# TomClabault/RayTracerCPP

Measured on AMD Instinct MI355X. Metric: Mrays/sec (primary+shadow) at 1920x1080, 1M-tri scene; max |dpixel|, higher is better.
Workload: dtype f32; 1 GPU; C4 sphere1m: 1,000,000 tris, 1920x1080, ssaa_factor 2 (3840x2160 rays), primary + shadow, octree 12/40; rays_per_frame=10029157, primary_rays=8294400, reflection_rays=0, band_rows=8, parallelism=image strips x1, frames_in_flight=3, world_size=1, bands=interleaved b % N

## Files before the change

### include/rt_mi355x.h

```cpp
#ifndef RT_MI355X_H
#define RT_MI355X_H

#include <stdint.h>

#ifdef __cplusplus
extern "C" {
#endif

#define RT_OK 0
#define RT_EINVAL (-1)
#define RT_EHIP (-2)
#define RT_ENOMEM (-3)
#define RT_ESTATE (-4)
#define RT_EUNSUPPORTED (-5)
#define RT_EIO (-6)

#define RT_SHADING_RT 0
#define RT_SHADING_ABS_NORMALS 1
#define RT_SHADING_PASTEL_NORMALS 2
#define RT_SHADING_BARYCENTRIC 3
#define RT_SHADING_VISUALIZE_AO 4

#define RT_TEX_AO 0
#define RT_TEX_DIFFUSE 1
// ... 91 lines not shown

int rt_set_devices(rt_renderer *r, const int32_t *ids, int32_t n);

int rt_change_render_size(rt_renderer *r, int32_t width, int32_t height);

int rt_set_triangles(rt_renderer *r, const float *tri9, const int32_t *mat, const float *uv6, int64_t n);

int rt_add_sphere(rt_renderer *r, float cx, float cy, float cz, float radius, int32_t mat);
int rt_add_plane(rt_renderer *r, float px, float py, float pz, float nx, float ny, float nz, int32_t mat);

int rt_clear_geometry(rt_renderer *r);

int rt_set_materials(rt_renderer *r, const float *mats16, int32_t n);
int rt_get_material_count(rt_renderer *r, int32_t *n);

int rt_change_camera_fov(rt_renderer *r, float fov);
int rt_change_camera_aspect_ratio(rt_renderer *r, float aspect);
int rt_set_light_position(rt_renderer *r, float x, float y, float z);

int rt_set_camera_transform(rt_renderer *r, const float m[16]);
int rt_apply_transformation_to_camera(rt_renderer *r, const float m[16]);

int rt_set_camera_matrices(rt_renderer *r, const float pos[3], const float proj_inv[16], const float cam_to_world[16]);
int rt_get_camera_matrices(rt_renderer *r, float pos[3], float proj_inv[16], float cam_to_world[16]);

int rt_set_camera_projection(rt_renderer *r, const float proj[16], const float world_to_cam[16]);

int rt_set_camera_lens(rt_renderer *r, float fov, float aspect);

int rt_set_object_transform(rt_renderer *r, const float m[16]);
int rt_reset_previous_transform(rt_renderer *r);
int rt_get_triangles(rt_renderer *r, float *tri9, int64_t *n);

int rt_set_texture(rt_renderer *r, int32_t slot, int32_t w, int32_t h, const float *rgba);

int rt_set_skybox(rt_renderer *r, const int32_t w[6], const int32_t h[6], const float *const faces[6]);

int rt_reconstruct_bvh_new(rt_renderer *r);
int rt_destroy_bvh(rt_renderer *r);

int rt_ray_trace(rt_renderer *r);

int rt_raster_trace(rt_renderer *r);

int rt_get_ssao_buffers(rt_renderer *r, float *z, float *n4, int32_t *ao);

int rt_post_process(rt_renderer *r);

int rt_get_image(rt_renderer *r, uint32_t *argb, int32_t *w, int32_t *h);

int rt_lock_image(rt_renderer *r);
int rt_unlock_image(rt_renderer *r);

int rt_render(rt_renderer *r, float *ms);

int rt_request_aux(rt_renderer *r, int32_t want_rgba, int32_t want_hit, int32_t want_shadow);
int rt_get_internal(rt_renderer *r, uint32_t *argb, float *rgba, int32_t *hit_id, float *hit_t, uint8_t *shadow);

int rt_get_stats(rt_renderer *r, rt_stats *out);

int rt_local_rows(rt_renderer *r, int32_t band_rows, int32_t rank, int32_t nranks, int32_t *rows_out);
int rt_render_bands_device(rt_renderer *r, int32_t band_rows, int32_t rank, int32_t nranks, uint32_t *d_out,
                           void *hip_stream);
int rt_render_band_list_device(rt_renderer *r, int32_t band_rows, const int32_t *bands, int32_t nbands,
                               uint32_t *d_out, void *hip_stream);
int rt_band_costs(rt_renderer *r, void *hip_stream, double *costs, int32_t nbands);

int rt_trace_rays(rt_renderer *r, const float *orig, const float *dir, int64_t n, int32_t *tri_id, float *t,
                  float *u, float *v, uint8_t *ret);

int rt_trace_rays_device(rt_renderer *r, const float *d_orig, const float *d_dir, int64_t n, int32_t *d_tri_id,
                         float *d_t, float *d_u, float *d_v, uint8_t *d_ret, int64_t *d_counts, void *hip_stream);
int rt_is_shadowed_device(rt_renderer *r, const float *d_point, const float *d_normal, int64_t n, const float *light,
                          uint8_t *d_shadowed, void *hip_stream);
int rt_get_device_ray_queries(rt_renderer *r, int64_t calls[2], int64_t rays[2]);

int rt_trace_ray(rt_renderer *r, const float *orig, const float *dir, int64_t n, int32_t current_recursion_depth,
                 float *rgba, int32_t *hit_src, float *t, uint8_t *intersection_found, uint8_t *shadowed);

int rt_kernel_times(rt_renderer *r, float *ms, int32_t n);
int rt_band_counters(rt_renderer *r, int64_t *shadow_rays, int64_t *reflection_rays);
int rt_tile_mask(rt_renderer *r, int32_t src, uint32_t *words, int64_t cap, int32_t info[5]);
int rt_tile_starts(rt_renderer *r, int32_t src, uint32_t *sets, int64_t cap, int32_t info[3]);

void rt_make_transform(int32_t kind, float x, float y, float z, float out[16]);
void rt_compose(const float a[16], const float b[16], float out[16]);
void rt_inverse(const float m[16], float out[16]);
void rt_perspective(float fov, float aspect, float znear, float zfar, float out[16]);
void rt_transform_points(const float m[16], const float *pts, int64_t n, float *out);

typedef struct rt_obj rt_obj;
rt_obj *rt_obj_open(const char *path, const float xform[16], int32_t mat_offset);
int rt_obj_counts(const rt_obj *o, int64_t *ntri, int32_t *nmat, int32_t *has_uv);
int rt_obj_fetch(const rt_obj *o, float *tri9, int32_t *mat, float *uv6, float *mats16);
void rt_obj_close(rt_obj *o);


#ifdef __cplusplus
}
#endif
#endif
```

### raytracercpp_amd/_lib.py

```python
from __future__ import annotations

import ctypes as C
import os

import numpy as np

HERE = os.path.dirname(os.path.abspath(__file__))
LIB_PATH = os.path.join(HERE, "librt_mi355x.so")
if os.environ.get("RT_LIB_PATH"):
    LIB_PATH = os.environ["RT_LIB_PATH"]

RT_OK = 0
ERRORS = {-1: "RT_EINVAL", -2: "RT_EHIP", -3: "RT_ENOMEM", -4: "RT_ESTATE", -5: "RT_EUNSUPPORTED", -6: "RT_EIO"}

_f32p = C.POINTER(C.c_float)
_i32p = C.POINTER(C.c_int32)
_u32p = C.POINTER(C.c_uint32)
_u8p = C.POINTER(C.c_uint8)
_i64p = C.POINTER(C.c_int64)


class RtSettings(C.Structure):
    _fields_ = [
        ("image_width", C.c_int32), ("image_height", C.c_int32),
# ... 35 lines not shown
                return [float(x) if n == "build_split_ms" else int(x) for x in v]
            return int(v)
        return {n: conv(n, t) for n, t in self._fields_}


class RtEntryProbe(C.Structure):
    _fields_ = [
        ("proj_inv", C.c_float * 16), ("cam_to_world", C.c_float * 16), ("rw", C.c_int32), ("rh", C.c_int32),
        ("k", C.c_int32), ("fan", C.c_int32), ("depth", C.c_int32), ("quick", C.c_int32),
        ("pixel", _i32p), ("sets", _u32p), ("info", C.c_int64 * 4), ("depth_hist", C.c_int64 * 16),
    ]


_H = C.c_void_p
SIGNATURES = {
    "rt_default_settings": (None, [C.POINTER(RtSettings)]),
    "rt_create": (_H, [C.c_int]),
    "rt_destroy": (None, [_H]),
    "rt_last_error": (C.c_char_p, []),
    "rt_get_settings": (C.c_int, [_H, C.POINTER(RtSettings)]),
    "rt_set_settings": (C.c_int, [_H, C.POINTER(RtSettings)]),
    "rt_change_render_size": (C.c_int, [_H, C.c_int32, C.c_int32]),
    "rt_set_exact": (C.c_int, [_H, C.c_int]),
    "rt_finish_accel": (C.c_int, [_H]),
    "rt_set_devices": (C.c_int, [_H, _i32p, C.c_int32]),
    "rt_set_triangles": (C.c_int, [_H, _f32p, _i32p, _f32p, C.c_int64]),
    "rt_add_sphere": (C.c_int, [_H, C.c_float, C.c_float, C.c_float, C.c_float, C.c_int32]),
    "rt_add_plane": (C.c_int, [_H] + [C.c_float] * 6 + [C.c_int32]),
    "rt_clear_geometry": (C.c_int, [_H]),
    "rt_set_materials": (C.c_int, [_H, _f32p, C.c_int32]),
    "rt_get_material_count": (C.c_int, [_H, _i32p]),
    "rt_change_camera_fov": (C.c_int, [_H, C.c_float]),
    "rt_change_camera_aspect_ratio": (C.c_int, [_H, C.c_float]),
    "rt_set_light_position": (C.c_int, [_H, C.c_float, C.c_float, C.c_float]),
    "rt_set_camera_transform": (C.c_int, [_H, _f32p]),
    "rt_apply_transformation_to_camera": (C.c_int, [_H, _f32p]),
    "rt_set_camera_matrices": (C.c_int, [_H, _f32p, _f32p, _f32p]),
    "rt_set_camera_projection": (C.c_int, [_H, _f32p, _f32p]),
    "rt_set_camera_lens": (C.c_int, [_H, C.c_float, C.c_float]),
    "rt_get_ssao_buffers": (C.c_int, [_H, _f32p, _f32p, _i32p]),
    "rt_get_camera_matrices": (C.c_int, [_H, _f32p, _f32p, _f32p]),
    "rt_set_object_transform": (C.c_int, [_H, _f32p]),
    "rt_reset_previous_transform": (C.c_int, [_H]),
    "rt_get_triangles": (C.c_int, [_H, _f32p, _i64p]),
    "rt_get_device_transforms": (C.c_int, [_H, _i64p]),
    "rt_transform_points_device": (C.c_int, [C.c_int32, _f32p, _f32p, C.c_int64, _f32p, _i32p, _f32p]),
    "rt_set_triangles_device": (C.c_int, [_H, C.c_void_p, C.c_int64, C.c_void_p, _i32p, _f32p, C.c_int64, C.c_void_p]),
    "rt_update_vertices_device": (C.c_int, [_H, C.c_void_p, C.c_int64, C.c_void_p, C.c_void_p]),
    "rt_get_device_ingests": (C.c_int, [_H, _i64p]),
    "rt_gather_triangles_device": (C.c_int, [C.c_int32, _f32p, C.c_int64, _i32p, C.c_int64, _f32p, _i32p, _f32p]),
    "rt_set_accel_deferred": (C.c_int, [_H, C.c_int]),
    "rt_get_accel_builds": (C.c_int, [_H, _i64p]),
    "rt_set_texture": (C.c_int, [_H, C.c_int32, C.c_int32, C.c_int32, _f32p]),
    "rt_set_skybox": (C.c_int, [_H, _i32p, _i32p, C.POINTER(_f32p)]),
    "rt_reconstruct_bvh_new": (C.c_int, [_H]),
    "rt_destroy_bvh": (C.c_int, [_H]),
    "rt_ray_trace": (C.c_int, [_H]),
    "rt_raster_trace": (C.c_int, [_H]),
    "rt_post_process": (C.c_int, [_H]),
    "rt_get_image": (C.c_int, [_H, _u32p, _i32p, _i32p]),
    "rt_render": (C.c_int, [_H, _f32p]),
    "rt_lock_image": (C.c_int, [_H]),
    "rt_unlock_image": (C.c_int, [_H]),
    "rt_request_aux": (C.c_int, [_H, C.c_int32, C.c_int32, C.c_int32]),
    "rt_get_internal": (C.c_int, [_H, _u32p, _f32p, _i32p, _f32p, _u8p]),
    "rt_get_stats": (C.c_int, [_H, C.POINTER(RtStats)]),
    "rt_local_rows": (C.c_int, [_H, C.c_int32, C.c_int32, C.c_int32, _i32p]),
    "rt_render_bands_device": (C.c_int, [_H, C.c_int32, C.c_int32, C.c_int32, C.c_void_p, C.c_void_p]),
    "rt_render_band_list_device": (C.c_int, [_H, C.c_int32, _i32p, C.c_int32, C.c_void_p, C.c_void_p]),
    "rt_band_costs": (C.c_int, [_H, C.c_void_p, C.POINTER(C.c_double), C.c_int32]),
    "rt_trace_rays": (C.c_int, [_H, _f32p, _f32p, C.c_int64, _i32p, _f32p, _f32p, _f32p, _u8p]),
    "rt_trace_rays_device": (C.c_int, [_H, C.c_void_p, C.c_void_p, C.c_int64, C.c_void_p, C.c_void_p, C.c_void_p,
                                       C.c_void_p, C.c_void_p, C.c_void_p, C.c_void_p]),
    "rt_is_shadowed_device": (C.c_int, [_H, C.c_void_p, C.c_void_p, C.c_int64, _f32p, C.c_void_p, C.c_void_p]),
    "rt_get_device_ray_queries": (C.c_int, [_H, _i64p, _i64p]),
    "rt_trace_ray": (C.c_int, [_H, _f32p, _f32p, C.c_int64, C.c_int32, _f32p, _i32p, _f32p, _u8p, _u8p]),
    "rt_wide_query": (C.c_int, [_H, _f32p, _f32p, C.c_int64, C.c_int32, _f32p, _f32p, _i32p, _i32p, _f32p, _f32p, _f32p,
                                _u8p]),
    "rt_risk_words": (C.c_int, [_H, C.c_int32, C.POINTER(C.c_uint64), C.c_int64, _i64p, _i64p]),
    "rt_kernel_times": (C.c_int, [_H, _f32p, C.c_int32]),
    "rt_band_counters": (C.c_int, [_H, _i64p, _i64p]),
    "rt_tile_mask": (C.c_int, [_H, C.c_int32, _u32p, C.c_int64, _i32p]),
    "rt_tile_starts": (C.c_int, [_H, C.c_int32, _u32p, C.c_int64, _i32p]),
    "rt_make_transform": (None, [C.c_int32, C.c_float, C.c_float, C.c_float, _f32p]),
    "rt_compose": (None, [_f32p, _f32p, _f32p]),
    "rt_inverse": (None, [_f32p, _f32p]),
    "rt_perspective": (None, [C.c_float, C.c_float, C.c_float, C.c_float, _f32p]),
    "rt_transform_points": (None, [_f32p, _f32p, C.c_int64, _f32p]),
    "rt_obj_open": (_H, [C.c_char_p, _f32p, C.c_int32]),
    "rt_obj_counts": (C.c_int, [_H, _i64p, _i32p, _i32p]),
    "rt_obj_fetch": (C.c_int, [_H, _f32p, _i32p, _f32p, _f32p]),
    "rt_obj_close": (None, [_H]),
    "rt_octree_digest": (C.c_int, [_f32p, C.c_int64, C.c_int32, C.c_int32, C.c_int32, C.POINTER(C.c_uint64), _i64p,
                                   _f32p]),
    "rt_octree_build_device": (C.c_int, [C.c_int32, _f32p, C.c_int64, C.c_int32, C.c_int32, C.POINTER(C.c_uint64),
                                         _i64p, _f32p]),
    "rt_set_device_build": (C.c_int, [_H, C.c_int]),
    "rt_get_device_builds": (C.c_int, [_H, _i64p]),
    "rt_get_device_wide_builds": (C.c_int, [_H, _i64p]),
    "rt_wbvh_quick_digest": (C.c_int, [_f32p, C.c_int64, C.c_int32, C.c_int32, C.POINTER(C.c_uint64), _i64p, _f32p]),
    "rt_wbvh_quick_build_device": (C.c_int, [C.c_int32, _f32p, C.c_int64, C.c_int32, C.c_int32, C.POINTER(C.c_uint64),
                                             _i64p, _i64p, _f32p]),
    "rt_debug_read": (C.c_int, [_H, C.POINTER(C.c_uint64), C.c_int64]),
    "rt_tile_costs": (C.c_int, [_H, C.POINTER(C.c_uint32), C.c_int64, _i32p, _i32p]),
    "rt_wbvh_query": (C.c_int, [_f32p, C.c_int64, C.c_int32, C.c_int32, _f32p, _f32p, C.c_int64, _i32p, _i32p, _f32p,
                                _f32p, _f32p, _i64p, _f32p]),
    "rt_wbvh_query_ex": (C.c_int, [_f32p, C.c_int64, C.c_int32, C.c_int32, _f32p, _f32p, C.c_int64, _f32p, _f32p,
                                   C.c_int32, _f32p, _f32p, _i32p, _i32p, _f32p, _f32p, _f32p, _i64p, _f32p, _i32p,
                                   C.c_int32, _i64p, C.POINTER(RtEntryProbe)]),
    "rt_ocone_check": (C.c_int, [_f32p, C.c_int64, C.c_int32, C.c_int32, C.c_int32, _f32p, _f32p, C.c_int64, _i32p,
                                 _i64p, C.POINTER(C.c_uint32), _i32p, _f32p, C.POINTER(C.c_uint32)]),
    "rt_ocone_read": (C.c_int, [_H, C.POINTER(C.c_uint32), C.c_int64, _i32p, _f32p]),
    "rt_risk_cap_check": (C.c_int, [_f32p, C.c_int64, C.c_int32, C.c_int32, _f32p, _f32p, C.c_int64, C.c_float, _i32p,
                                    _i64p]),
}

GEOMETRY_INPUT = ("rt_set_triangles_device", "rt_update_vertices_device", "rt_get_device_ingests",
                  "rt_gather_triangles_device", "rt_set_accel_deferred", "rt_get_accel_builds")
RAY_QUERIES = ("rt_trace_rays_device", "rt_is_shadowed_device", "rt_get_device_ray_queries")

_lib = None


def has(name):
    return hasattr(lib(), name)


def lib():
    global _lib
    if _lib is None:
        if not os.path.exists(LIB_PATH):
            raise RuntimeError(f"{LIB_PATH} is missing: the HIP library must be built "
                               "(python -c 'import __graft_entry__ as g; g.build()')")
        try:
            import torch
        except ImportError:
            pass
        L = C.CDLL(LIB_PATH)
        for name, (res, args) in SIGNATURES.items():
            if name in GEOMETRY_INPUT + RAY_QUERIES and os.environ.get("RT_LIB_PATH") and not hasattr(L, name):
                continue
            fn = getattr(L, name)
            fn.restype = res
            fn.argtypes = args
        _lib = L
    return _lib


class RtError(RuntimeError):
    def __init__(self, code, where):
        msg = lib().rt_last_error()
        super().__init__(f"{where}: {ERRORS.get(code, code)}: {msg.decode() if msg else ''}")
        self.code = code


def check(rc, where):
    if rc != RT_OK:
        raise RtError(rc, where)
    return rc


def ptr(a, t):
    if a is None:
        return C.cast(None, t)
    return a.ctypes.data_as(t)


def f32(a):
    return np.ascontiguousarray(a, dtype=np.float32)


_KINDS = {"translation": 0, "rx": 1, "ry": 2, "rz": 3, "scale": 4, "identity": 5}


def make_transform(kind, x=0.0, y=0.0, z=0.0):
    out = np.zeros(16, np.float32)
    lib().rt_make_transform(_KINDS[kind], x, y, z, ptr(out, _f32p))
    return out


def compose(a, b):
    a, b = f32(a), f32(b)
    out = np.zeros(16, np.float32)
    lib().rt_compose(ptr(a, _f32p), ptr(b, _f32p), ptr(out, _f32p))
    return out


def inverse(m):
    m = f32(m)
    out = np.zeros(16, np.float32)
    lib().rt_inverse(ptr(m, _f32p), ptr(out, _f32p))
    return out


def perspective(fov, aspect, znear=0.1, zfar=1000.0):
    out = np.zeros(16, np.float32)
    lib().rt_perspective(fov, aspect, znear, zfar, ptr(out, _f32p))
    return out


def camera_matrices(fov, aspect, znear=0.1, zfar=1000.0):
    p = perspective(fov, aspect, znear, zfar)
    return p, inverse(p)


def transform_points(m, pts):
    m = f32(m)
    pts = f32(pts).reshape(-1, 3)
    out = np.zeros_like(pts)
    lib().rt_transform_points(ptr(m, _f32p), ptr(pts, _f32p), pts.shape[0], ptr(out, _f32p))
    return out


def transform_points_device(m, pts, device=0):
    m = f32(m)
    pts = f32(pts).reshape(-1, 3)
    out = np.zeros_like(pts)
    flag = C.c_int32()
    ms = np.zeros(2, np.float32)
    check(lib().rt_transform_points_device(device, ptr(m, _f32p), ptr(pts, _f32p), pts.shape[0], ptr(out, _f32p),
                                           C.byref(flag), ptr(ms, _f32p)), "rt_transform_points_device")
    return out, int(flag.value), (float(ms[0]), float(ms[1]))

# ... 241 lines not shown
```

### raytracercpp_amd/csrc/capi.cpp

```cpp
#include <atomic>
#include <chrono>
#include <cmath>
#include <thread>
#include <cstring>
#include <new>
#include <string>

#include "../../include/rt_mi355x_diag.h"
#include "host_scene.hpp"
#include "launch.hpp"
#include "octree.hpp"
#include "octree_gpu.hpp"
#include "ocone.hpp"
#include "wbvh.hpp"
#include "wbvh_quick_gpu.hpp"
#include "renderer.hpp"

namespace {
thread_local std::string g_err;

int record(rt::Renderer* r, int rc)
{
    if (rc != RT_OK)
        g_err = r->error();
// ... 394 lines not shown
        if (n < 0)
            return bad("bad band layout");
        *rows_out = n;
        return RT_OK;
    });
}
int rt_render_bands_device(rt_renderer* r, int32_t band_rows, int32_t rank, int32_t nranks, uint32_t* d_out,
                           void* hip_stream)
{
    return guarded(R(r), [&] {
        return R(r)->render_bands_device(band_rows, rank, nranks, d_out, reinterpret_cast<hipStream_t>(hip_stream));
    });
}

int rt_render_band_list_device(rt_renderer* r, int32_t band_rows, const int32_t* bands, int32_t nbands, uint32_t* d_out,
                               void* hip_stream)
{
    return guarded(R(r), [&] {
        return R(r)->render_band_list_device(band_rows, bands, nbands, d_out, reinterpret_cast<hipStream_t>(hip_stream));
    });
}
int rt_band_costs(rt_renderer* r, void* hip_stream, double* costs, int32_t nbands)
{
    return guarded(R(r), [&] { return R(r)->band_costs(reinterpret_cast<hipStream_t>(hip_stream), costs, nbands); });
}

int rt_trace_rays(rt_renderer* r, const float* orig, const float* dir, int64_t n, int32_t* tri_id, float* t,
                  float* u, float* v, uint8_t* ret)
{
    return guarded(R(r), [&] { return R(r)->trace_rays(orig, dir, n, tri_id, t, u, v, ret); });
}
int rt_trace_rays_device(rt_renderer* r, const float* d_orig, const float* d_dir, int64_t n, int32_t* d_tri_id,
                         float* d_t, float* d_u, float* d_v, uint8_t* d_ret, int64_t* d_counts, void* hip_stream)
{
    return guarded(R(r), [&] {
        return R(r)->trace_rays_device(d_orig, d_dir, n, d_tri_id, d_t, d_u, d_v, d_ret, d_counts,
                                       reinterpret_cast<hipStream_t>(hip_stream));
    });
}
int rt_is_shadowed_device(rt_renderer* r, const float* d_point, const float* d_normal, int64_t n, const float* light,
                          uint8_t* d_shadowed, void* hip_stream)
{
    return guarded(R(r), [&] {
        return R(r)->is_shadowed_device(d_point, d_normal, n, light, d_shadowed, reinterpret_cast<hipStream_t>(hip_stream));
    });
}
int rt_get_device_ray_queries(rt_renderer* r, int64_t calls[2], int64_t rays[2])
{
    return guarded(R(r), [&] {
        if (!calls || !rays)
            return RT_EINVAL;
        R(r)->device_ray_queries(calls, rays);
        return RT_OK;
    });
}
int rt_wide_query(rt_renderer* r, const float* orig, const float* dir, int64_t n, int32_t kind, float* o_out,
                  float* d_out, int32_t* status, int32_t* tri_id, float* t, float* u, float* v, uint8_t* shadowed)
{
    return guarded(R(r), [&] { return R(r)->wide_query(orig, dir, n, kind, o_out, d_out, status, tri_id, t, u, v, shadowed); });
}
int rt_risk_words(rt_renderer* r, int32_t src, uint64_t* out, int64_t cap, int64_t* count, int64_t* violations)
{
    return guarded(R(r), [&] { return R(r)->risk_words(src, out, cap, count, violations); });
}
int rt_trace_ray(rt_renderer* r, const float* orig, const float* dir, int64_t n, int32_t current_recursion_depth,
                 float* rgba, int32_t* hit_src, float* t, uint8_t* intersection_found, uint8_t* shadowed)
{
    return guarded(R(r), [&] {
        return R(r)->trace_ray_colors(orig, dir, n, current_recursion_depth, rgba, hit_src, t, intersection_found,
                                      shadowed);
    });
}
int rt_kernel_times(rt_renderer* r, float* ms, int32_t n)
{
    return guarded(R(r), [&] { return ms ? R(r)->kernel_times(ms, n) : RT_EINVAL; });
}
int rt_tile_mask(rt_renderer* r, int32_t src, uint32_t* words, int64_t cap, int32_t info[5])
{
    return guarded(R(r), [&] { return info ? R(r)->tile_mask(src, words, cap, info) : RT_EINVAL; });
}
int rt_tile_starts(rt_renderer* r, int32_t src, uint32_t* sets, int64_t cap, int32_t info[3])
{
    return guarded(R(r), [&] { return info ? R(r)->tile_starts(src, sets, cap, info) : RT_EINVAL; });
}
int rt_band_counters(rt_renderer* r, int64_t* shadow_rays, int64_t* reflection_rays)
{
    return guarded(R(r), [&] {
        unsigned long long c[2] = {0, 0};
        int rc = R(r)->band_counters(c);
        if (shadow_rays) *shadow_rays = (int64_t)c[0];
        if (reflection_rays) *reflection_rays = (int64_t)c[1];
        return rc;
    });
}

void rt_make_transform(int32_t kind, float x, float y, float z, float out[16])
{
    switch (kind) {
    case 0: rt::mat::translation(x, y, z, out); break;
    case 1: rt::mat::rotation_x(x, out); break;
    case 2: rt::mat::rotation_y(x, out); break;
    case 3: rt::mat::rotation_z(x, out); break;
    case 4: rt::mat::scale(x, y, z, out); break;
    default: rt::mat::identity(out); break;
    }
}
void rt_compose(const float a[16], const float b[16], float out[16]) { rt::mat::compose(a, b, out); }
void rt_inverse(const float m[16], float out[16]) { rt::mat::inverse(m, out); }
void rt_perspective(float fov, float aspect, float znear, float zfar, float out[16])
{
    rt::mat::perspective(fov, aspect, znear, zfar, out);
}
void rt_transform_points(const float m[16], const float* pts, int64_t n, float* out)
{
    rt::mat::transform_points(m, pts, n, out);
}

struct rt_obj {
    rt::ObjData data;
};

rt_obj* rt_obj_open(const char* path, const float xform[16], int32_t mat_offset)
{
    try {
        float ident[16];
        rt::mat::identity(ident);
        rt_obj* o = new rt_obj;
        std::string err;
        if (!rt::load_obj(path, xform ? xform : ident, mat_offset, o->data, err)) {
            g_err = err;
            delete o;
            return nullptr;
        }
        return o;
    } catch (const std::exception& e) {
        g_err = e.what();
        return nullptr;
    }
}

int rt_obj_counts(const rt_obj* o, int64_t* ntri, int32_t* nmat, int32_t* has_uv)
{
    if (!o)
        return bad("null obj");
    if (ntri) *ntri = (int64_t)o->data.mat.size();
    if (nmat) *nmat = (int32_t)o->data.materials.size();
    if (has_uv) *has_uv = o->data.has_uv;
    return RT_OK;
}

int rt_obj_fetch(const rt_obj* o, float* tri9, int32_t* mat, float* uv6, float* mats16)
{
    if (!o)
        return bad("null obj");
    const rt::ObjData& d = o->data;
    if (tri9) std::memcpy(tri9, d.tri.data(), d.tri.size() * 4);
    if (mat) std::memcpy(mat, d.mat.data(), d.mat.size() * 4);
    if (uv6 && d.has_uv) std::memcpy(uv6, d.uv.data(), d.uv.size() * 4);
    if (mats16) {
        for (size_t i = 0; i < d.materials.size(); i++) {
            const rt::ObjMaterial& m = d.materials[i];
            float* f = mats16 + 16 * i;
            for (int c = 0; c < 3; c++) {
                f[0 + c] = m.ambient[c];
                f[3 + c] = m.diffuse[c];
                f[6 + c] = m.specular[c];
// ... 915 lines not shown
```

### raytracercpp_amd/csrc/kernels.hip

```cpp
#include <hip/hip_runtime.h>
#include <stdint.h>
#if defined(RT_COUNT) && RT_COUNT
__device__ unsigned long long g_wsteps[8];
__device__ __forceinline__ void w_step_hook(uint32_t cur, int leaf)
{
    const uint64_t act = __ballot(1);
    uint64_t left = act;
    unsigned distinct = 0;
    while (left) {
        const uint32_t f = (uint32_t)__builtin_amdgcn_readlane((int)cur, __ffsll((unsigned long long)left) - 1);
        left &= ~__ballot(cur == f);
        distinct++;
    }
    if ((int)__lane_id() == __ffsll((unsigned long long)act) - 1) {
        atomicAdd(&g_wsteps[2 * leaf], 1ull);
        if (distinct == 1)
            atomicAdd(&g_wsteps[2 * leaf + 1], 1ull);
        atomicAdd(&g_wsteps[4 + leaf], (unsigned long long)__popcll(act));
        atomicAdd(&g_wsteps[6 + leaf], (unsigned long long)distinct);
    }
}
#define W_STEP_HOOK(cur, leaf) w_step_hook(cur, leaf)
#endif
#include "kparams.hpp"
#include "rt_math.hpp"
#include "wbvh.hpp"
#include "launch.hpp"

namespace rt {

constexpr int WAVES_PER_BLOCK = 4;
constexpr int BLOCK = 64 * WAVES_PER_BLOCK;

#ifndef RT_OCC
#define RT_OCC 5
#endif
#ifndef RT_OCC_PLAIN
#define RT_OCC_PLAIN 3
#endif
#ifndef RT_OCC_OCT
#define RT_OCC_OCT 5
#endif
#ifndef RT_COUNT
#define RT_COUNT 0
#endif
#ifndef RT_PHASE_TIME
#define RT_PHASE_TIME 0
#endif

struct TRay {
    v3 o, d;
    float den[NPLANES], num[NPLANES];
    bool nan;
    float lo, hi;
};


struct Rec {
    int tri;
    float t, u, v;
    int mat;
    v3 normal, tangent;
};

__device__ __forceinline__ Rec rec_fresh()
{
    Rec r;
    r.tri = -1; r.t = -1.0f; r.u = 1.0f; r.v = 0.0f; r.mat = -1;
    r.normal = mk(0, 0, 0); r.tangent = mk(0, 0, 0);
    return r;
}

__device__ __forceinline__ TRay make_ray(const KParams& P, v3 o, v3 d)
{
    TRay R;
    R.o = o;
    R.d = d;
    bool nan = false;
#pragma unroll
    for (int i = 0; i < NPLANES; i++) {
        v3 n = mk(PLANE_N[i][0], PLANE_N[i][1], PLANE_N[i][2]);
        R.den[i] = dot(n, d);
        R.num[i] = dot(n, o);
        nan |= (R.den[i] != R.den[i]) || (R.num[i] != R.num[i]);
        if (R.den[i] == 0.0f)
            R.num[i] = __int_as_float(0x7fc00000);
    }
    R.nan = nan;
    R.lo = -INFINITY;
    R.hi = INFINITY;
    return R;
}

__device__ __forceinline__ v3 opaque(v3 v)
{
    asm volatile("" : "+v"(v.x), "+v"(v.y), "+v"(v.z));
    return v;
}

__device__ __forceinline__ bool ray_is_nan(v3 o, v3 d)
{
    bool nan = false;
#pragma unroll
    for (int i = 0; i < NPLANES; i++) {
        v3 n = mk(PLANE_N[i][0], PLANE_N[i][1], PLANE_N[i][2]);
        float den = dot(n, d), num = dot(n, o);
        nan |= (den != den) || (num != num);
    }
    return nan;
// ... 540 lines not shown
        face = d2.z < 0.0f ? 4 : 5;
        nf = (float)(0.5 / (double)da.z);
        u = d2.z < 0.0f ? -d2.x : d2.x;
        v = -d2.y;
    } else if (da.y >= da.x) {
        face = d2.y < 0.0f ? 3 : 2;
        nf = (float)(0.5 / (double)da.y);
        u = d2.x;
        v = d2.y < 0.0f ? -d2.z : d2.z;
    } else {
        face = d2.x < 0.0f ? 1 : 0;
        nf = (float)(0.5 / (double)da.x);
        u = d2.x < 0.0f ? d2.z : -d2.z;
        v = -d2.y;
    }
    u = (float)((double)(u * nf) + 0.5);
    v = (float)((double)(v * nf) + 0.5);
    return tex_bilinear(P.sky[face], u, v, alpha);
}

__device__ __forceinline__ const float* mat_of(const KParams& P, int id) { return P.mats + (size_t)MAT_STRIDE * id; }
__device__ __forceinline__ c3 mat_col(const float* m, int off) { return col(m[off], m[off + 1], m[off + 2]); }

__device__ __forceinline__ void get_tex_coords(const KParams& P, int tri, float u, float v, float& tu, float& tv)
{
    if (tri >= 0) {
        float u0 = -1, u1 = -1, u2 = -1, v0 = -1, v1 = -1, v2 = -1;
        if (P.tri_uv) {
            const float* uv = P.tri_uv + 6 * (size_t)tri;
            u0 = uv[0]; u1 = uv[1]; u2 = uv[2];
            v0 = uv[3]; v1 = uv[4]; v2 = uv[5];
        }
        tu = (1 - u - v) * u0 + u * u1 + v * u2;
        tv = (1 - u - v) * v0 + u * v1 + v * v2;
    } else {
        tu = u;
        tv = v;
    }
}

__device__ v3 normal_mapping(const KParams& P, const Rec& h, float u, float v)
{
    float tu, tv;
    get_tex_coords(P, h.tri, u, v, tu, tv);
    v3 T = h.tangent;
    v3 B = cross(T, h.normal);
    v3 N = h.normal;
    c3 nc = tex_floor(P.tex[TEX_NORMAL], tu, tv);
    v3 nm = mk(nc.r, nc.g, nc.b) * 2.0f - mk(1, 1, 1);
    v3 q = normalize(nm);
    v3 p = mk(T.x * q.x + B.x * q.y + N.x * q.z, T.y * q.x + B.y * q.y + N.y * q.z, T.z * q.x + B.z * q.y + N.z * q.z);
    return normalize(p);
}

__device__ void parallax_occlusion_mapping(const KParams& P, int tri, float u, float v, v3 view, float& nu, float& nv)
{
    float tu, tv;
    get_tex_coords(P, tri, u, v, tu, tv);
    const KTex& D = P.tex[TEX_DISPLACEMENT];
    int steps = P.parallax_mapping_steps;
    float current_depth;
    float depth_step = 1.0f / steps;
    float sampled = tex_floor(D, tu, tv).r;
    v3 search = -view * P.displacement_mapping_strength;
    float du = search.x / steps;
    float dv = search.y / steps;
    current_depth = 0.0f;
    float u2 = tu, v2 = tv;
    while (current_depth < sampled) {
        u2 += du;
        v2 += dv;
        sampled = tex_floor(D, u2, v2).r;
        current_depth += depth_step;
    }
    float pu = u2 - du, pv = v2 - dv;
    float after = sampled - current_depth;
    float before = tex_floor(D, pu, pv).r - (current_depth - depth_step);
    float w = after / (after - before);
    nu = (1 - w) * u2 + w * pu;
    nv = (1 - w) * v2 + w * pv;
}

#if RT_PHASE_TIME
__shared__ unsigned long long g_phase[WAVES_PER_BLOCK][8];
__device__ __forceinline__ void ph_mark(int k)
{
    const unsigned long long now = __builtin_amdgcn_s_memtime();
    const uint64_t act = __ballot(1);
    if ((int)__lane_id() == __ffsll((unsigned long long)act) - 1) {
        const int w = threadIdx.x >> 6;
        g_phase[w][k] += now - g_phase[w][7];
        g_phase[w][7] = now;
    }
}
#define PH_MARK(k) ph_mark(k)
#else
#define PH_MARK(k)
#endif

constexpr int LDS_SAVE_ENTRIES = 3;
__host__ __device__ __forceinline__ int lds_save_slot(const KParams& P) { return P.levels > W_STACK ? P.levels : W_STACK; }
#ifndef RT_W_STACK_PLAIN
#define RT_W_STACK_PLAIN 22
#endif
constexpr int W_STACK_PLAIN = RT_W_STACK_PLAIN;
static_assert(W_STACK_PLAIN >= W_STACK && W_STACK_PLAIN + LDS_SAVE_ENTRIES <= 26, "the plain kernel's LDS entries");
template <bool OCT>
__host__ __device__ __forceinline__ int lds_save_slot_plain(const KParams& P)
{
    const int w = OCT ? 0 : W_STACK_PLAIN;
    return P.levels > w ? P.levels : w;
}

template <int N = W_STACK>
struct WStackLdsN {
    static constexpr int CAP = N;
    uint2* base;
    __device__ __forceinline__ void put(int i, uint2 v) { base[i * BLOCK] = v; }
    __device__ __forceinline__ uint2 get(int i) const { return base[i * BLOCK]; }
    __device__ __forceinline__ uint2 get_lane(int delta, int i) const { return base[delta + i * BLOCK]; }
};
using WStackLds = WStackLdsN<W_STACK>;

#if RT_COUNT
__device__ void count_wave_steps(const KParams& P, int base, uint32_t steps)
{
    if (!P.counters)
        return;
    uint64_t act = __ballot(1), a = act;
    uint32_t mx = 0;
    while (a) {
        const int l = __ffsll((unsigned long long)a) - 1;
        a &= a - 1;
        mx = max(mx, (uint32_t)__builtin_amdgcn_readlane((int)steps, l));
    }
    if ((int)__lane_id() == __ffsll((unsigned long long)act) - 1) {
        atomicAdd(&P.counters[base], (unsigned long long)mx);
        atomicAdd(&P.counters[base + 2], 1ull);
    }
    atomicAdd(&P.counters[base + 1], (unsigned long long)steps);
}
#endif


struct WDeep {
    int st;
    WHit w;
};
__device__ __noinline__ WDeep wide_closest_deep(const WNode* wnodes, const GTri* wtris, v3 o, v3 d, float m, float hi,
                                                bool ties, float QS, const uint64_t* rk, int rsel, float rsub)
{
    WStackArr<W_DEEP_STACK> stk;
    WDeep r;
    const int st = wbvh_closest(wnodes, wtris, o, d, m, stk, r.w, nullptr, hi, ties, QS, rk, rsel, rsub);
    r.st = st == W_DEEP ? W_UNCERT : st;
    return r;
}

__device__ __forceinline__ float wide_margin(const KParams& P, v3 o)
{
    const float om = fmaxf(fabsf(o.x), fmaxf(fabsf(o.y), fabsf(o.z)));
    return 0x1p-16f * (om + P.scene_scale);
}

template <class Stk, int G>
__device__ __forceinline__ int wide_run(const KParams& P, v3 o, v3 d, uint2* lv, WHit& w, float hi, bool ties, float QS,
                                        const uint64_t* rk, int rsel, float rsub, uint32_t max_steps, bool nob, int count,
                                        const uint32_t* start = nullptr)
{
    const float m = wide_margin(P, o);
    Stk stk{lv};
#if RT_COUNT
    uint32_t work[4] = {0, 0, 0, 0};
    uint32_t* wk = count >= 0 ? work : nullptr;
#else
// ... 622 lines not shown
            if (F.rough > 0) {
                F.sc++;
                F.i++;
            } else {
                F.sc = 1;
                F.i = N;
            }
            f = depth - 1;
            state = S_NEXT;
        } else {
            Frame& F = fr[f];
            if (F.i < N) {
                v3 dir;
                next_key = child_key(F.key, (uint32_t)F.i);
                if (F.rough > 0) {
                    uint32_t rng = sample_state(F.key, (uint32_t)F.i);
                    float rx = rng_bilateral(rng);
                    float ry = rng_bilateral(rng);
                    float rz = rng_bilateral(rng);
                    v3 rdir = normalize(mk(rx, ry, rz));
                    if (dot(rdir, F.n) < 0)
                        rdir = -rdir;
                    dir = F.rough * rdir + (1 - F.rough) * F.perfect;
                } else
                    dir = F.perfect;
                nrefl++;
                ro = F.ro;
                rd = dir;
                depth = f + 1;
                state = S_TRACE;
            } else {
                const float* m = mat_of(P, F.mat);
                float sc = (float)F.sc, rf = m[12];
                c3 R = (F.total / col(sc, sc, sc)) * col(rf, rf, rf);
                ret = shade_finish(P, F.fc, m, R);
                depth = f;
                state = S_RET;
            }
        }
    }
    po.color = ret;
    return po;
}

__device__ __forceinline__ void write_ssao_buffers(const KParams& P, size_t o, bool found, v3 cam, v3 rd,
                                                   const Rec& fin)
{
    P.zbuf[o] = found ? -(cam.z + rd.z * fin.t) : INFINITY;
    P.nbuf[o] = found ? make_float4(fin.normal.x, fin.normal.y, fin.normal.z, 0.0f) : make_float4(0, 0, 0, 0);
}

__device__ __forceinline__ void tile_xy(const KParams& P, int tile, int& tx, int& ty)
{
    const int W = P.tiles_x;
    if (tile >= (1 << 24)) {
        tx = tile % W;
        ty = tile / W;
        return;
    }
    int q = (int)((float)tile * (1.0f / (float)W));
    int r = tile - q * W;
    if (r < 0) {
        q--;
        r += W;
    } else if (r >= W) {
        q++;
        r -= W;
    }
    tx = r;
    ty = q;
}

__device__ __forceinline__ int global_row(const KParams& P, int lr)
{
    if (P.nranks == 1)
        return lr;
    int band = lr / P.band_rows;
    const int g = P.band_map ? ldg(P.band_map + band) : band * P.nranks + P.rank;
    return g * P.band_rows + (lr - band * P.band_rows);
}

constexpr int BQ_BATCH = 4;

__device__ __forceinline__ int shard_tile(const KParams& P, int s, int t)
{
    const int r0 = (int)((long long)P.tiles_y * s / TILE_SHARDS), r1 = (int)((long long)P.tiles_y * (s + 1) / TILE_SHARDS);
    return t < (r1 - r0) * P.tiles_x ? r0 * P.tiles_x + t : -1;
}


struct BlockQueue {
    unsigned int word;
    int shard, empty;
    int base[4], sh[4];
    int heavy_done;
    int split_done;
    unsigned long long cost_sum;
    unsigned int cost_max;
    int waves_done;
};
__shared__ BlockQueue g_bq;

__device__ __forceinline__ void tile_queue_init()
{
    if (threadIdx.x == 0) {
        g_bq.word = 0u;
        g_bq.shard = (int)(blockIdx.x & (TILE_SHARDS - 1));
        g_bq.empty = 0;
        g_bq.heavy_done = 0;
        g_bq.split_done = 0;
        g_bq.cost_sum = 0;
        g_bq.cost_max = 0;
        g_bq.waves_done = 0;
    }
    __syncthreads();
}

__device__ __forceinline__ void tile_stats_add(uint32_t c, uint32_t cmax)
{
    __hip_atomic_fetch_add(&g_bq.cost_sum, (unsigned long long)c, __ATOMIC_RELAXED, __HIP_MEMORY_SCOPE_WORKGROUP);
    __hip_atomic_fetch_max(&g_bq.cost_max, cmax, __ATOMIC_RELAXED, __HIP_MEMORY_SCOPE_WORKGROUP);
}

__device__ __forceinline__ void tile_stats_flush(const KParams& P, int lane)
{
    if (!P.tile_stats || lane != 0)
        return;
    const int k = __hip_atomic_fetch_add(&g_bq.waves_done, 1, __ATOMIC_ACQ_REL, __HIP_MEMORY_SCOPE_WORKGROUP);
    if (k != (int)(blockDim.x >> 6) - 1)
        return;
    const unsigned long long s = __hip_atomic_load(&g_bq.cost_sum, __ATOMIC_ACQUIRE, __HIP_MEMORY_SCOPE_WORKGROUP);
    const unsigned int m = __hip_atomic_load(&g_bq.cost_max, __ATOMIC_ACQUIRE, __HIP_MEMORY_SCOPE_WORKGROUP);
    if (s) atomicAdd(P.tile_stats, s);
    if (m) atomicMax(P.tile_stats + 1, (unsigned long long)m);
}

__device__ __forceinline__ int tile_queue_next_shards(const KParams& P)
{
    const int lane = threadIdx.x & 63;
    for (;;) {
        unsigned int w = 0;
        if (lane == 0)
            w = __hip_atomic_fetch_add(&g_bq.word, 1u, __ATOMIC_ACQ_REL, __HIP_MEMORY_SCOPE_WORKGROUP);
        w = __builtin_amdgcn_readfirstlane(w);
        if (w & 0x80000000u)
            return -1;
        const unsigned int g = (w >> 24) & 0x7fu, c = (w >> 16) & 0xffu, i = w & 0xffffu;
        if (i < c) {
            const int slot = (int)(g & 3u);
            return shard_tile(P, g_bq.sh[slot], g_bq.base[slot] + (int)i);
        }
        if (i == c) {
            int shard = g_bq.shard, empty = g_bq.empty, b = 0, n = 0;
            while (empty < TILE_SHARDS) {
                int t = 0;
                if (lane == 0)
                    t = (int)atomicAdd(reinterpret_cast<unsigned int*>(&P.counters[NCOUNTERS + 16 * shard]),
                                       (unsigned)BQ_BATCH);
                b = __builtin_amdgcn_readfirstlane(t);
                n = 0;
                while (n < BQ_BATCH && shard_tile(P, shard, b + n) >= 0)
                    n++;
                if (n > 0)
                    break;
                empty++;
                shard = (shard + 1) & (TILE_SHARDS - 1);
            }
            const unsigned int g1 = (g + 1u) & 0x7fu;
            if (lane == 0) {
                g_bq.shard = shard;
                g_bq.empty = empty;
                g_bq.base[g1 & 3u] = b;
                g_bq.sh[g1 & 3u] = shard;
                __hip_atomic_store(&g_bq.word, n > 0 ? (g1 << 24) | ((unsigned)n << 16) | 1u : 0x80000000u,
                                   __ATOMIC_RELEASE, __HIP_MEMORY_SCOPE_WORKGROUP);
            }
            return n > 0 ? shard_tile(P, shard, b) : -1;
        }
        for (;;) {
            unsigned int v = 0;
            if (lane == 0)
                v = __hip_atomic_load(&g_bq.word, __ATOMIC_ACQUIRE, __HIP_MEMORY_SCOPE_WORKGROUP);
            v = __builtin_amdgcn_readfirstlane(v);
            if ((v & 0x80000000u) || ((v >> 24) & 0x7fu) != g)
                break;
            __builtin_amdgcn_s_sleep(2);
        }
    }
}

__device__ __forceinline__ int tile_queue_next(const KParams& P)
{
    const int lane = threadIdx.x & 63;
    if (P.heavy_list) {
        if (!__builtin_amdgcn_readfirstlane(__hip_atomic_load(&g_bq.heavy_done, __ATOMIC_RELAXED,
                                                             __HIP_MEMORY_SCOPE_WORKGROUP))) {
            int t = 0;
            if (lane == 0)
                t = atomicAdd(P.heavy_ctr + 1, 1);
            t = __builtin_amdgcn_readfirstlane(t);
            if (t < min(ldg(P.heavy_ctr), P.tiles_x * P.tiles_y / 16))
                return ldg(P.heavy_list + t);
            if (lane == 0)
                __hip_atomic_store(&g_bq.heavy_done, 1, __ATOMIC_RELAXED, __HIP_MEMORY_SCOPE_WORKGROUP);
        }
        for (;;) {
            const int tile = tile_queue_next_shards(P);
            if (tile < 0 || !((ldg(P.heavy_bits + (tile >> 5)) >> (tile & 31)) & 1u))
                return tile;
        }
    }
    return tile_queue_next_shards(P);
}

__device__ __forceinline__ void set_wave_prio(int level)
{
    switch (level) {
    case 3: __builtin_amdgcn_s_setprio(3); break;
    case 2: __builtin_amdgcn_s_setprio(2); break;
    case 1: __builtin_amdgcn_s_setprio(1); break;
    default: __builtin_amdgcn_s_setprio(0); break;
    }
}

template <int G = 1, int C0 = 8>
__device__ __forceinline__ void downscale_tile(const KParams& P, int lane, int lr, int px, uint32_t c, int C = C0)
{
    int r = (int)((c >> 16) & 0xffu), g = (int)((c >> 8) & 0xffu), b = (int)(c & 0xffu);
    const int f = 1 << P.ds_shift;
    for (int m = 1; m < f; m <<= 1) {
        r += __shfl_xor(r, G * m);
        g += __shfl_xor(g, G * m);
        b += __shfl_xor(b, G * m);
    }
    for (int m = C; m < C * f; m <<= 1) {
        r += __shfl_xor(r, G * m);
        g += __shfl_xor(g, G * m);
        b += __shfl_xor(b, G * m);
    }
    const int pl = lane / G;
    if ((lane & (G - 1)) == 0 && ((pl % C) & (f - 1)) == 0 && ((pl / C) & (f - 1)) == 0) {
        const int s2 = 2 * P.ds_shift;
        P.ds_out[(size_t)(lr >> P.ds_shift) * (size_t)(P.rw >> P.ds_shift) + (size_t)(px >> P.ds_shift)] =
            qrgb(r >> s2, g >> s2, b >> s2);
    }
}

__device__ __forceinline__ v3 camera_dir(const KParams& P, int px, int py, v3 cam)
{
    const float y_world = ((float)py + 0.5f) / P.rh * 2 - 1;
    const float x_world = ((float)px + 0.5f) / P.rw * 2 - 1;
    v3 vs;
    if (P.proj_mode != 0) {
        const float* m = P.proj_inv;
        const float x = x_world, y = y_world, z = -1.0f;
        const float xt = m[0] * x + m[1] * y + m[2] * z + m[3];
        const float yt = m[4] * x + m[5] * y + m[6] * z + m[7];
        const float zt = m[8] * x + m[9] * y + m[10] * z + m[11];
        const float w = P.proj_w;
        vs = P.proj_mode == 1 ? mk(xt, yt, zt) : mk(xt * w, yt * w, zt * w);
    } else
        vs = xform_point(P.proj_inv, mk(x_world, y_world, -1));
    v3 ws;
    if (P.c2w_affine && fabsf(vs.x) < INFINITY && fabsf(vs.y) < INFINITY && fabsf(vs.z) < INFINITY) {
        const float* m = P.cam_to_world;
        ws = mk(m[0] * vs.x + m[1] * vs.y + m[2] * vs.z + m[3], m[4] * vs.x + m[5] * vs.y + m[6] * vs.z + m[7],
                m[8] * vs.x + m[9] * vs.y + m[10] * vs.z + m[11]);
    } else
        ws = xform_point(P.cam_to_world, vs);
    return normalize(ws - cam);
}

__device__ __forceinline__ int tile_start_index(const KParams& P, int px, int py)
{
    return P.tile_start ? (py >> 3) * P.start_bw + (px >> 3) : -1;
}

template <int G>
__device__ __forceinline__ void trace_split_part(const KParams& P, uint2* lv, int t, int lane, unsigned& nshadow)
{
    static_assert(G > 1 && G <= 8 && (G & (G - 1)) == 0, "2, 4 or 8 lanes per pixel");
    const int cap = P.tiles_x * P.tiles_y / 16;
    const int np = P.split_parts;
    const int tq = ldg(P.heavy_list + cap + t / np), part = t % np;
    const int tile = tq & 0x0fffffff;
    set_wave_prio(tq >> 28);
    const uint64_t t0 = __builtin_amdgcn_s_memtime();
    int tx, ty;
    tile_xy(P, tile, tx, ty);
    const int npix = 64 / np;
    const int C = npix >= 16 ? 8 : npix / 2, R = npix / C;
    const int pl = lane / G;
    const int px = tx * 8 + (part % (8 / C)) * C + pl % C;
    const int lr = ty * 8 + (part / (8 / C)) * R + pl / C;
    const int py = lr < P.local_rows ? global_row(P, lr) : P.rh;
    if (pl < npix && px < P.rw && py < P.rh) {
        const v3 cam = mk(P.cam_pos[0], P.cam_pos[1], P.cam_pos[2]);
        const v3 rd = camera_dir(P, px, py, cam);
        unsigned ns = 0, nr = 0;
        PixelOut po = trace_pixel<false, true, G>(P, cam, rd, lv, 0u, ns, nr, tile_start_index(P, px, py));
        if ((lane & (G - 1)) == 0)
            nshadow += ns;
        const size_t o = (size_t)lr * P.rw + px;
        const uint32_t c = color_to_argb(po.color);
        if (P.ds_out) downscale_tile<G>(P, lane, lr, px, c, C);
        if ((lane & (G - 1)) == 0) {
            if (P.argb) P.argb[o] = c;
            if (P.rgba) P.rgba[o] = make_float4(po.color.r, po.color.g, po.color.b, po.alpha);
            if (P.hit_id) P.hit_id[o] = po.found ? po.src : -1;
            if (P.hit_t) P.hit_t[o] = po.fin.t;
            if (P.shadow) P.shadow[o] = (uint8_t)(po.found && po.shadowed);
        }
    }
    const uint64_t c = __builtin_amdgcn_s_memtime() - t0;
    if (lane == 0) {
        const uint32_t c32 = c > 0xFFFFFFFFull ? 0xFFFFFFFFu : (uint32_t)c;
        atomicAdd(P.tile_cost + tile, c32);
        tile_stats_add(c32, c32 > 0xFFFFFFFFu / G ? 0xFFFFFFFFu : c32 * G);
    }
}

__device__ __forceinline__ void tile_cost_store(const KParams& P, int tile, uint64_t t0, int lane)
{
    const uint64_t c = __builtin_amdgcn_s_memtime() - t0;
    if (lane == 0) {
        const uint32_t c32 = c > 0xFFFFFFFFull ? 0xFFFFFFFFu : (uint32_t)c;
        P.tile_cost[tile] = c32;
        tile_stats_add(c32, c32);
    }
}

__device__ __noinline__ void fill_masked_tile(const KParams& P, int lr, int px)
{
    const c3 bg = background();
    const uint32_t c = color_to_argb(bg);
    const size_t o = (size_t)lr * P.rw + px;
    if (P.argb) P.argb[o] = c;
    if (P.ds_out) {
        const int f = 1 << P.ds_shift;
        if ((px & (f - 1)) == 0 && (lr & (f - 1)) == 0)
            P.ds_out[(size_t)(lr >> P.ds_shift) * (size_t)(P.rw >> P.ds_shift) + (size_t)(px >> P.ds_shift)] =
                qrgb((int)((c >> 16) & 0xffu), (int)((c >> 8) & 0xffu), (int)(c & 0xffu));
    }
    if (P.rgba) P.rgba[o] = make_float4(bg.r, bg.g, bg.b, 1.0f);
    if (P.hit_id) P.hit_id[o] = -1;
    if (P.hit_t) P.hit_t[o] = rec_fresh().t;
    if (P.shadow) P.shadow[o] = (uint8_t)0;
#if RT_COUNT
    if (P.counters && (threadIdx.x & 63) == 0)
        atomicAdd(&P.counters[28], 1ull);
#endif
}

template <bool REFL, bool PLAIN = false, bool OCT = false>
__global__ __launch_bounds__(BLOCK, OCT ? RT_OCC_OCT : PLAIN ? RT_OCC_PLAIN : RT_OCC) void ray_trace_kernel(KParams P_arg)
{
    auto kp = __builtin_amdgcn_kernarg_segment_ptr();
    (void)P_arg;
    const KParams& P = *reinterpret_cast<const KParams*>((const void*)kp);
    uint2* lv = lane_stack();
    int lane = threadIdx.x & 63;
    unsigned nshadow = 0, nrefl = 0;
    tile_queue_init();
#if RT_PHASE_TIME
    if (PLAIN && lane == 0) {
        for (int k = 0; k < 7; k++)
            g_phase[threadIdx.x >> 6][k] = 0;
        g_phase[threadIdx.x >> 6][7] = __builtin_amdgcn_s_memtime();
    }
#endif
    for (;;) {
        auto kpl = kp;
        asm volatile("" : "+s"(kpl));
        const KParams& P = *reinterpret_cast<const KParams*>((const void*)kpl);
        const v3 cam = mk(P.cam_pos[0], P.cam_pos[1], P.cam_pos[2]);
        if (PLAIN && !REFL && !OCT && P.heavy_group == SPLIT_G &&
            !__builtin_amdgcn_readfirstlane(__hip_atomic_load(&g_bq.split_done, __ATOMIC_RELAXED, __HIP_MEMORY_SCOPE_WORKGROUP))) {
            int t = 0;
            if (lane == 0)
                t = atomicAdd(P.heavy_ctr + 2, 1);
            t = __builtin_amdgcn_readfirstlane(t);
            if (t < P.split_parts * min(ldg(P.heavy_ctr + 3), P.tiles_x * P.tiles_y / 16)) {
                trace_split_part<SPLIT_G>(P, lv, t, lane, nshadow);
                continue;
            }
            if (lane == 0)
                __hip_atomic_store(&g_bq.split_done, 1, __ATOMIC_RELAXED, __HIP_MEMORY_SCOPE_WORKGROUP);
        }
        const int tq = tile_queue_next(P);
        if (PLAIN) PH_MARK(6);
        if (tq < 0)
            break;
        const int tile = tq & 0x0fffffff;
        if (P.heavy_list)
            set_wave_prio(tq >> 28);
        const uint64_t tile_t0 = __builtin_amdgcn_s_memtime();
        int tx, ty;
        tile_xy(P, tile, tx, ty);
        int px = tx * 8 + (lane & 7);
        int lr = ty * 8 + (lane >> 3);
        int py = lr < P.local_rows ? global_row(P, lr) : P.rh;
        if (PLAIN) PH_MARK(0);
        if (px >= P.rw || py >= P.rh) {
            if (P.tile_cost && lane == 0)
                P.tile_cost[tile] = 0u;
            continue;
        }
        if (PLAIN && !REFL && !OCT && P.tile_mask) {
            const uint32_t mw = ldg(P.tile_mask + (size_t)(py >> 3) * (size_t)P.mask_wpr + (size_t)(px >> 8));
            if (!__ballot((mw >> ((px >> 3) & 31)) & 1u)) {
                fill_masked_tile(P, lr, px);
                if (P.tile_cost)
                    tile_cost_store(P, tile, tile_t0, lane);
                continue;
            }
        }
        const v3 rd = camera_dir(P, px, py, cam);
        if (PLAIN) PH_MARK(1);

        uint32_t rng = REFL ? pixel_seed((uint32_t)(py * P.rw + px), P.rng_seed) : 0u;
        PixelOut po = trace_pixel<REFL, PLAIN, 1, OCT>(P, cam, rd, lv, rng, nshadow, nrefl,
                                                        PLAIN && !REFL && !OCT ? tile_start_index(P, px, py) : -1);
        size_t o = (size_t)lr * P.rw + px;
        if (P.argb) P.argb[o] = color_to_argb(po.color);
        if (!REFL && P.ds_out) downscale_tile(P, lane, lr, px, color_to_argb(po.color));
        if (P.rgba) P.rgba[o] = make_float4(po.color.r, po.color.g, po.color.b, po.alpha);
        if (P.hit_id) P.hit_id[o] = po.found ? po.src : -1;
        if (P.hit_t) P.hit_t[o] = po.fin.t;
        if (P.shadow) P.shadow[o] = (uint8_t)(po.found && po.shadowed);
        if (!PLAIN && P.zbuf) write_ssao_buffers(P, o, po.found, cam, rd, po.fin);
        if (PLAIN) PH_MARK(5);
        if (P.tile_cost)
            tile_cost_store(P, tile, tile_t0, lane);
    }
    tile_stats_flush(P, lane);
#if RT_PHASE_TIME
    if (PLAIN) {
        PH_MARK(0);
        const int wid = (int)(blockIdx.x * WAVES_PER_BLOCK + (threadIdx.x >> 6));
        if (P.dbg && lane == 0 && wid < DBG_WAVES)
            for (int k = 0; k < 7; k++)
                P.dbg[DBG_WORDS * wid + k] = g_phase[threadIdx.x >> 6][k];
    }
#endif
    if (nshadow) atomicAdd(&P.counters[0], (unsigned long long)nshadow);
    if (nrefl) atomicAdd(&P.counters[1], (unsigned long long)nrefl);
}

__device__ __forceinline__ v3 ld3(const float* p) { return mk(p[0], p[1], p[2]); }
__device__ __forceinline__ void st3(float* p, v3 v) { p[0] = v.x; p[1] = v.y; p[2] = v.z; }
__device__ __forceinline__ void st3(float* p, c3 c) { p[0] = c.r; p[1] = c.g; p[2] = c.b; }
__device__ __forceinline__ c3 ldc(const float* p) { return col(p[0], p[1], p[2]); }

__device__ __forceinline__ void wave_count_add(unsigned long long* ctr, unsigned v)
{
    for (int off = 32; off > 0; off >>= 1)
        v += __shfl_xor(v, off);
    if ((threadIdx.x & 63) == 0 && v)
        atomicAdd(ctr, (unsigned long long)v);
}

__device__ __forceinline__ uint32_t wave_append(unsigned int* counter, bool lead = true)
{
    const uint64_t m = __ballot(lead);
    const int leader = __ffsll((unsigned long long)m) - 1;
    uint32_t base = 0;
    if ((int)(threadIdx.x & 63) == leader)
        base = atomicAdd(counter, (unsigned)__popcll(m));
    base = __shfl(base, leader);
    return base + __builtin_amdgcn_mbcnt_hi((uint32_t)(m >> 32), __builtin_amdgcn_mbcnt_lo((uint32_t)m, 0u));
}

__device__ __forceinline__ float frame_roughness(const KParams& P, const Rec& h, const float* m)
{
    if (P.enable_roughness_mapping) {
        float tu, tv;
        get_tex_coords(P, h.tri, h.u, h.v, tu, tv);
        return tex_floor(P.tex[TEX_ROUGHNESS], tu, tv).r;
    }
    return m[13];
}

__device__ __forceinline__ int frame_nsamp(const KParams& P, float rough)
{
    int N = P.rough_reflections_sample_count;
    return N <= 0 ? 0 : (rough > 0 ? N : 1);
}

__device__ __forceinline__ void make_frame(const KParams& P, FrameRec& F, v3 ip, v3 n, v3 rd, c3 fc, float rough,
                                           int mat, uint32_t key, int parent)
{
    st3(F.ro, ip + n * 0.01f);
    st3(F.perfect, rd - (2 * dot(rd, n)) * n);
    st3(F.n, n);
    st3(F.fc, fc);
    F.rough = rough;
    F.mat = mat;
    F.key = key;
    F.nsamp = frame_nsamp(P, rough);
    F.parent = parent;
}

__global__ __launch_bounds__(BLOCK, RT_OCC) void refl_level0_kernel(KParams P_arg, FrameRec* fr1, unsigned int* nfr1)
{
    const KParams& P = kernel_params();
    (void)P_arg;
    uint2* lv = lane_stack();
    int lane = threadIdx.x & 63;
    const int ntiles = P.tiles_x * P.tiles_y;
    v3 cam = mk(P.cam_pos[0], P.cam_pos[1], P.cam_pos[2]);
    unsigned nshadow = 0;
    for (;;) {
        int tile = 0;
        if (lane == 0)
            tile = (int)atomicAdd(reinterpret_cast<unsigned int*>(&P.counters[2]), 1u);
        tile = __builtin_amdgcn_readfirstlane(tile);
        if (tile >= ntiles)
            break;
        int tx, ty;
        tile_xy(P, tile, tx, ty);
        int px = tx * 8 + (lane & 7);
        int lr = ty * 8 + (lane >> 3);
        int py = lr < P.local_rows ? global_row(P, lr) : P.rh;
        if (px >= P.rw || py >= P.rh)
            continue;
        const v3 rd = camera_dir(P, px, py, cam);

        Rec fin = rec_fresh();
        int src = closest_hit(P, cam, rd, fin, lv);
// ... 1429 lines not shown
    if (blockIdx.x == 0) {
        for (int i = (int)threadIdx.x; i < ncounters; i += (int)blockDim.x)
            counters[i] = 0ull;
        if (threadIdx.x < 4)
            ctr_next[threadIdx.x] = 0;
        if (threadIdx.x < 2)
            stats_next[threadIdx.x] = 0ull;
    }
    const unsigned long long sum = stats_prev[0];
    const unsigned int mx = (unsigned int)min(stats_prev[1], 0xFFFFFFFFull);
    const unsigned long long mean = ntiles > 0 ? sum / (unsigned long long)ntiles : 0;
    const unsigned long long thr = max(4 * mean, (unsigned long long)(mx / 8));
    const unsigned long long thr2 = group > 1 && nwaves > 0 ? max(thr, (unsigned long long)((double)split * (double)sum / nwaves))
                                                            : ~0ull;
    const int cap = ntiles / 16;
    const int i = (int)(blockIdx.x * blockDim.x + threadIdx.x);
    const int lane = (int)(threadIdx.x & 63);
    const uint32_t c = i < ntiles ? cost[i] : 0u;
    const bool heavy = mx > 0 && c >= thr && c > 0;
    const bool two = heavy && c >= thr2;
    const uint64_t b1 = __ballot(heavy && !two), b2 = __ballot(two);
    int base1 = 0, base2 = 0;
    if (lane == 0) {
        if (b1) base1 = atomicAdd(ctr, __popcll(b1));
        if (b2) base2 = atomicAdd(ctr + 3, __popcll(b2));
    }
    base1 = __builtin_amdgcn_readfirstlane(base1);
    base2 = __builtin_amdgcn_readfirstlane(base2);
    const uint64_t below = (1ull << lane) - 1ull;
    const int k = two ? base2 + __popcll(b2 & below) : base1 + __popcll(b1 & below);
    const bool listed = heavy && k < cap;
    if (listed) {
        const int prio = ntiles >= (1 << 28) ? 0 : c >= mx / 2 ? 3 : c >= mx / 4 ? 2 : 1;
        list[two ? cap + k : k] = i | (prio << 28);
        if (two)
            cost[i] = 0u;
    }
    const uint64_t bl = __ballot(listed);
    if ((lane & 31) == 0 && i < ntiles)
        bits[i >> 5] = (uint32_t)(bl >> lane);
}

static int plain_blocks(const rt::KParams& P)
{
    const int tiles = P.tiles_x * P.tiles_y;
    const int blocks = (tiles + rt::WAVES_PER_BLOCK - 1) / rt::WAVES_PER_BLOCK;
    return P.max_blocks > 0 ? std::max(1, std::min(blocks, P.max_blocks / 8 * RT_OCC_PLAIN)) : blocks;
}

static int persistent_blocks(const rt::KParams& P)
{
    const int tiles = P.tiles_x * P.tiles_y;
    const int blocks = (tiles + rt::WAVES_PER_BLOCK - 1) / rt::WAVES_PER_BLOCK;
    return blocks > P.max_blocks && P.max_blocks > 0 ? P.max_blocks : blocks;
}

hipError_t rt_launch_heavy_prep(const rt::KParams* P, uint32_t* cost, int ntiles, int32_t* list, uint32_t* bits,
                                int32_t* ctr, int32_t* ctr_next, const unsigned long long* stats_prev,
                                unsigned long long* stats_next, float split, int group, hipStream_t stream)
{
    if (ntiles <= 0)
        return hipSuccess;
    hipLaunchKernelGGL(heavy_prep_kernel, dim3((ntiles + 63) / 64), dim3(64), 0, stream, cost, ntiles, list, bits,
                       ctr, ctr_next, stats_prev, stats_next, P->counters, rt::NCOUNTER_WORDS,
                       plain_blocks(*P) * rt::WAVES_PER_BLOCK, split, group);
    return hipGetLastError();
}

hipError_t rt_launch_ray_trace(const rt::KParams* P, hipStream_t stream)
{
    const int blocks = persistent_blocks(*P);
    if (blocks < 1)
        return hipSuccess;
    const bool plain = !P->has_reflection && P->plain && !P->zbuf && !P->nbuf;
    size_t lds = rt::lds_bytes(*P, plain);
    if (P->has_reflection)
        hipLaunchKernelGGL((rt::ray_trace_kernel<true, false>), dim3(blocks), dim3(rt::BLOCK), lds, stream, *P);
    else if (plain) {
        if (!P->wnodes) {
            hipLaunchKernelGGL((rt::ray_trace_kernel<false, true, true>), dim3(blocks), dim3(rt::BLOCK), lds, stream, *P);
            return hipGetLastError();
        }
        const int pblocks = plain_blocks(*P);
        hipLaunchKernelGGL((rt::ray_trace_kernel<false, true>), dim3(pblocks), dim3(rt::BLOCK), lds, stream, *P);
    } else
        hipLaunchKernelGGL((rt::ray_trace_kernel<false, false>), dim3(blocks), dim3(rt::BLOCK), lds, stream, *P);
    return hipGetLastError();
}

__global__ __launch_bounds__(256) void risk_box_init_kernel(float* B, size_t n)
{
    const size_t i = (size_t)blockIdx.x * 256 + threadIdx.x;
    if (i < 6 * n)
        B[i] = (i % 6) < 3 ? INFINITY : -INFINITY;
}

hipError_t rt_launch_risk_box_init(float* B, size_t nentries, hipStream_t stream)
{
    if (nentries > 0)
        hipLaunchKernelGGL(risk_box_init_kernel, dim3((unsigned)((6 * nentries + 255) / 256)), dim3(256), 0, stream, B,
                           nentries);
    return hipGetLastError();
}

__global__ __launch_bounds__(1024) void wide_cut_kernel(const rt::WNode* __restrict__ nodes, int nnodes, int budget,
                                                        int max_depth, float QS, uint32_t* buf)
{
    __shared__ int s_n, s_next, s_grew;
    uint32_t* cur = buf;
    uint32_t* nxt = buf + rt::W_CUT_MAX;
    const int tid = (int)threadIdx.x;
    if (tid == 0) {
        int n = 0;
        for (int j = 0; j < rt::W_WIDTH; j++)
            if (nodes[0].child[j] != rt::W_EMPTY)
                cur[n++] = (uint32_t)j;
        s_n = n;
    }
    __syncthreads();
    for (int depth = 1; depth < max_depth; depth++) {
        if (tid == 0) {
            s_next = 0;
            s_grew = 0;
        }
        __syncthreads();
        const int n = s_n;
        int total = 0, grew = 0;
        for (int i = tid; i < n; i += 1024) {
            uint32_t out[rt::W_WIDTH];
            const int k = rt::wbvh_cut_expand(nodes, nnodes, cur[i], QS, out);
            total += k;
            grew |= !(k == 1 && out[0] == cur[i]);
        }
        if (total)
            atomicAdd(&s_next, total);
        if (grew)
            atomicOr(&s_grew, 1);
        __syncthreads();
        const bool stop = !s_grew || s_next > budget;
        __syncthreads();
        if (stop)
            break;
        if (tid == 0)
            s_next = 0;
        __syncthreads();
        for (int i = tid; i < n; i += 1024) {
            uint32_t out[rt::W_WIDTH];
            const int k = rt::wbvh_cut_expand(nodes, nnodes, cur[i], QS, out);
            const int base = atomicAdd(&s_next, k);
            for (int q = 0; q < k; q++)
                nxt[base + q] = out[q];
        }
        __syncthreads();
        if (tid == 0)
            s_n = s_next;
        uint32_t* t = cur;
        cur = nxt;
        nxt = t;
        __syncthreads();
    }
    const int n = s_n;
    if (cur != buf)
        for (int i = tid; i < n; i += 1024)
            buf[i] = cur[i];
    if (tid == 0)
        buf[2 * rt::W_CUT_MAX] = (uint32_t)n;
}

__global__ __launch_bounds__(256) void wide_mask_kernel(const rt::WNode* __restrict__ nodes, int nnodes,
                                                        const uint32_t* __restrict__ parent, const uint32_t* __restrict__ cut,
                                                        rt::WMaskCam C, uint32_t* words)
{
    const uint32_t i = blockIdx.x * 256u + threadIdx.x;
    if (i >= cut[2 * rt::W_CUT_MAX] || i >= (uint32_t)rt::W_CUT_MAX)
        return;
    const uint32_t en = cut[i];
    if ((int)(en >> 2) >= nnodes)
        return;
    rt::WMaskRect R = rt::wbvh_mask_entry(nodes, nnodes, parent, en, C);
    R.x0 = max(R.x0, 0);
    R.y0 = max(R.y0, 0);
    R.x1 = min(R.x1, C.bw - 1);
    R.y1 = min(R.y1, C.bh - 1);
    if (R.x0 > R.x1)
        return;
    for (int y = R.y0; y <= R.y1; y++)
        for (int w = R.x0 >> 5; w <= R.x1 >> 5; w++) {
            uint32_t* p = words + (size_t)y * C.wpr + w;
            const uint32_t m = rt::wbvh_mask_word(R, w);
            if ((__hip_atomic_load(p, __ATOMIC_RELAXED, __HIP_MEMORY_SCOPE_AGENT) & m) != m)
                atomicOr(p, m);
        }
}

__global__ __launch_bounds__(256) void wide_entry_kernel(const rt::WNode* __restrict__ nodes, int nnodes, rt::WMaskCam C,
                                                         const uint32_t* __restrict__ words, int K, int fan, int max_depth,
                                                         uint4* out)
{
    const uint32_t i = blockIdx.x * 256u + threadIdx.x;
    if (i >= (uint32_t)(C.bw * C.bh))
        return;
    const int bx = (int)(i % (uint32_t)C.bw), by = (int)(i / (uint32_t)C.bw);
    uint4 r = make_uint4(0u, rt::W_EMPTY, rt::W_EMPTY, rt::W_EMPTY);
    if ((words[(size_t)by * C.wpr + (bx >> 5)] >> (bx & 31)) & 1u) {
        const rt::WEntrySet S = rt::wbvh_entry_block(nodes, nnodes, C, bx, by, K, fan, max_depth);
        r = make_uint4(S.link[0], S.link[1], S.link[2], S.link[3]);
    }
    out[i] = r;
}

hipError_t rt_launch_wide_entry(const rt::WNode* wnodes, int nnodes, const rt::WMaskCam* C, const uint32_t* words, int K,
                                int fan, int max_depth, uint4* out, hipStream_t stream)
{
    const int nb = C->bw * C->bh;
    if (nb <= 0)
        return hipSuccess;
    hipLaunchKernelGGL(wide_entry_kernel, dim3((nb + 255) / 256), dim3(256), 0, stream, wnodes, nnodes, *C, words, K, fan,
                       max_depth, out);
    return hipGetLastError();
}

hipError_t rt_launch_wide_cut(const rt::WNode* wnodes, int nnodes, int budget, int max_depth, uint32_t* buf, hipStream_t stream)
{
    budget = budget < rt::W_WIDTH ? rt::W_WIDTH : (budget > rt::W_CUT_MAX ? rt::W_CUT_MAX : budget);
    hipLaunchKernelGGL(wide_cut_kernel, dim3(1), dim3(1024), 0, stream, wnodes, nnodes, budget, max_depth, W_QS_CLOSEST, buf);
    return hipGetLastError();
}

hipError_t rt_launch_wide_mask(const rt::WNode* wnodes, int nnodes, const uint32_t* parent, const uint32_t* cut, int budget,
                               const rt::WMaskCam* C, uint32_t* words, hipStream_t stream)
{
    budget = budget < rt::W_WIDTH ? rt::W_WIDTH : (budget > rt::W_CUT_MAX ? rt::W_CUT_MAX : budget);
    hipError_t e = hipMemsetAsync(words, 0, (size_t)C->bh * C->wpr * 4, stream);
    if (e != hipSuccess)
        return e;
    hipLaunchKernelGGL(wide_mask_kernel, dim3((budget + 255) / 256), dim3(256), 0, stream, wnodes, nnodes, parent, cut,
                       *C, words);
    return hipGetLastError();
}

hipError_t rt_launch_wide_risk(const rt::GTri* wtris, const uint4* wmeta, const rt::GNode* onodes,
                               const rt::WNode* wnodes, const uint32_t* tri_leaf, const uint32_t* parent, uint32_t* K,
                               float* B, unsigned long long* risk, int n, int nnodes, const rt::WRiskArgs* A,
                               uint32_t* cap, const float* cap_dir, hipStream_t stream)
{
    rt::RiskCapDirs cd;
    for (int i = 0; i < 6; i++)
        cd.c[i / 3][i % 3] = cap_dir ? cap_dir[i] : 0.0f;
    if (n > 0)
        hipLaunchKernelGGL(rt::wide_risk_kernel, dim3((n + 255) / 256), dim3(256), 0, stream, wtris, wmeta, onodes,
                           tri_leaf, parent, K, B, n, *A, cap, cd);
    const int ne = 8 * nnodes;
    if (ne > 0)
        hipLaunchKernelGGL(rt::wide_risk_pack_kernel, dim3((ne + 255) / 256), dim3(256), 0, stream, wnodes, K, B, risk,
                           ne, *A);
    return hipGetLastError();
}

hipError_t rt_launch_wide_gather(const rt::GTri* tris, const int32_t* slot, const uint32_t* leaf_of_slot,
                                 const int32_t* tri_id, const int32_t* tri_mat, int n, rt::GTri* wtris, uint4* wmeta,
                                 hipStream_t stream)
{
    if (n <= 0)
        return hipSuccess;
    hipLaunchKernelGGL(rt::wide_gather_kernel, dim3((n + 255) / 256), dim3(256), 0, stream, tris, slot, leaf_of_slot,
                       tri_id, tri_mat, n, wtris, wmeta);
    return hipGetLastError();
}

namespace rt {
__global__ void ocone_fill_kernel(uint2* cells, size_t n)
{
    const size_t i = (size_t)blockIdx.x * 256 + threadIdx.x;
    if (i < n)
        cells[i] = make_uint2(0u, OC_NOSKIP << 16);
}

struct OConeArgs {
    float lo[3];
    int32_t dim[3];
    double h, r, slack, QS, cos_cap;
};

__global__ __launch_bounds__(256) void ocone_kernel(const OConeEnt* E, const GTri* tris, const uint32_t* todo, int n,
                                                    OConeArgs A, uint2* cells)
{
    const int i = blockIdx.x * 256 + threadIdx.x;
    if (i >= n)
        return;
    const uint32_t id = todo[i];
    double c[3];
    ocone_center(A.lo, A.dim, A.h, id, c);
    cells[id] = ocone_cell<OC_STACK>(E, tris, c, A.r, A.slack, A.QS, A.cos_cap);
}
}

hipError_t rt_launch_ocone(const rt::OConeEnt* E, const rt::GTri* tris, const uint32_t* todo, int n, const float lo[3],
                           const int32_t dim[3], double h, double r, double slack, double QS, double cos_cap,
                           uint2* cells, size_t ncells, hipStream_t stream)
{
    if (ncells == 0)
// ... 162 lines not shown
```

### raytracercpp_amd/csrc/kparams.hpp

```cpp
#pragma once

#include <stdint.h>

#include "octree.hpp"
#include "ocone.hpp"
#include "wbvh.hpp"

namespace rt {

#ifndef RT_SPLIT_G
#define RT_SPLIT_G 4
#endif
constexpr int SPLIT_G = RT_SPLIT_G;
constexpr int SPLIT_COLS = SPLIT_G == 8 ? 4 : 8;
constexpr int SPLIT_ROWS = 64 / SPLIT_G / SPLIT_COLS;
static_assert(SPLIT_G == 2 || SPLIT_G == 4 || SPLIT_G == 8, "2, 4 or 8 lanes per pixel");

constexpr int TEX_SLOTS = 6;
constexpr int MAT_STRIDE = 16;
constexpr int MAX_SHAPES = 64;
constexpr int NCOUNTERS = 32;
constexpr int TILE_SHARDS = 8;
constexpr int NCOUNTER_WORDS = NCOUNTERS + 16 * TILE_SHARDS;
constexpr int DBG_WAVES = 16384;
// ... 17 lines not shown
    const float* lslab;
    float scene_scale;
    const float* lsin;
    const WNode* wnodes;
    const GTri* wtris;
    const uint4* wmeta;
    const uint64_t* wrisk;
    float risk_G, risk_nl, risk_nu;
    const float* risk_cap;
    float cap_dir[2][3];
    float sb_lo[3], sb_hi[3];
    int32_t sb_valid;
    const uint32_t* tile_mask;
    int32_t mask_wpr;
    const uint4* tile_start;
    int32_t start_bw;
    OConeView ocone;
    int32_t nnodes;
    int32_t ntri_slots;
    int32_t levels;

    int32_t nshape;
    int32_t shape_kind[MAX_SHAPES];
    float shape[MAX_SHAPES][6];
    int32_t shape_mat[MAX_SHAPES];

    const float* mats;
    int32_t nmat;

    float cam_pos[3];
    float proj_inv[16];
    float cam_to_world[16];
    float light[3];
    int32_t proj_mode;
    float proj_w;
    int32_t c2w_affine;

    KTex tex[TEX_SLOTS];
    KTex sky[6];

    int32_t shading_method;
    int32_t compute_shadows;
    int32_t max_recursion_depth;
    int32_t enable_bvh;
    int32_t enable_ambient, enable_diffuse, enable_specular, enable_emissive;
    int32_t rough_reflections_sample_count;
    int32_t enable_ao_mapping, enable_diffuse_mapping, enable_normal_mapping, enable_displacement_mapping;
    float displacement_mapping_strength;
    int32_t parallax_mapping_steps;
    int32_t enable_roughness_mapping, enable_skysphere, enable_skybox;
    uint32_t rng_seed;
    int32_t has_reflection;
    float seg_scale;
    int32_t seg_oct;

    int32_t rw, rh;
    int32_t band_rows;
    int32_t nranks, rank;
    const int32_t* band_map;
    const int32_t* band_inv;
    int32_t local_rows;
    int32_t tiles_x, tiles_y;
    int32_t max_blocks;
    int32_t plain;
    uint32_t* tile_cost;
    unsigned long long* tile_stats;
    const int32_t* heavy_list;
    const uint32_t* heavy_bits;
    int32_t* heavy_ctr;
    int32_t heavy_group;
    int32_t split_parts;

    uint32_t* argb;
    float4* rgba;
    int32_t* hit_id;
    float* hit_t;
    uint8_t* shadow;
    unsigned long long* counters;
    unsigned long long* dbg;
    float* zbuf;
    float4* nbuf;
    uint32_t* ds_out;
    int32_t ds_shift;
};

struct SsaoArgs {
    const float* z;
    const float4* n;
    int32_t* ao;
    uint32_t* argb;
    int32_t w, h;
    int32_t simd_w;
    int32_t count;
    float radius, amount;
    float fovm;
    float tanv;
    float aspect;
    uint32_t seed;
    float proj[16];
};

struct FrameRec {
    float ro[3];
    float perfect[3];
    float n[3];
    float fc[3];
    float rough;
    int32_t mat;
    uint32_t key;
    int32_t nsamp;
    int32_t parent;
};

struct SampleRec {
    float d[3];
    int32_t kind;
    float fc[3];
    float ip[3];
    float nrm[3];
    int32_t mat;
    float crough;
    int32_t sh;
    int32_t child;
    int32_t ray;
};

struct RawHit {
    float t, u, v;
    int32_t k;
    float d[3];
    int32_t r;
};

struct ReflArgs {
    FrameRec* fr;
    SampleRec* sm;
    RawHit* hit;
    float* ret;
    const float* child_ret;
    FrameRec* child_fr;
    unsigned int* child_count;
    const int32_t* order;
    const FrameRec* frs;
    unsigned int* feed_parts;
    int32_t* list;
    unsigned int* list_count;
    int32_t c0, c1;
    int32_t level;
    int32_t stride;
    int32_t sample_major;
    float4* res;
    int32_t* defer;
    unsigned int* defer_count;
    int32_t max_steps;
    int32_t feed;
};

struct RasterPiece {
    float na[3], nb[3], nc[3];
    float wa[3], wb[3], wc[3];
    float inv_area;
    float za, zb, zc;
    int32_t x0, y0, x1, y1;
    int32_t tri;
    int32_t pad;
};
// ... 18 lines not shown
```

### raytracercpp_amd/csrc/launch.hpp

```cpp
#pragma once

#include <hip/hip_runtime.h>
#include <stdint.h>

#include "kparams.hpp"
#include "ocone.hpp"
#include "wbvh.hpp"

namespace rt {

enum class ReflStage {
    trace,
    long_,
    pass1,
    shadow,
    resolve,
};

enum class RasterStage {
    count,
    write,
    fill,
    fill_big,
};

}

#define RT_LAUNCH extern "C" __attribute__((visibility("hidden"))) hipError_t

RT_LAUNCH rt_launch_ray_trace(const rt::KParams* P, hipStream_t stream);
RT_LAUNCH rt_launch_heavy_prep(const rt::KParams* P, uint32_t* cost, int ntiles, int32_t* list, uint32_t* bits,
                               int32_t* ctr, int32_t* ctr_next, const unsigned long long* stats_prev,
                               unsigned long long* stats_next, float split, int group, hipStream_t stream);
RT_LAUNCH rt_launch_trace_rays(const rt::KParams* P, const float* o, const float* d, int n, int32_t* id, float* t,
                               float* u, float* v, uint8_t* ret, hipStream_t stream);
RT_LAUNCH rt_launch_wide_query(const rt::KParams* P, const float* o, const float* d, int n, int kind, float* o_out,
                               float* d_out, int32_t* status, int32_t* id, float* t, float* u, float* v, uint8_t* sh,
                               hipStream_t stream);
RT_LAUNCH rt_launch_closest_rays(const rt::KParams* P, const float* o, const float* d, int n, int32_t* id, float* t,
                                 float* u, float* v, uint8_t* ret, int64_t* counts, hipStream_t stream);
RT_LAUNCH rt_launch_shadow_points(const rt::KParams* P, const float* point, const float* normal, int n,
                                  const float light[3], uint8_t* shadowed, hipStream_t stream);
RT_LAUNCH rt_launch_trace_colors(const rt::KParams* P, bool refl, const float* o, const float* d, int n, float4* rgba,
                                 int32_t* src, float* t, uint8_t* found, uint8_t* shadow, hipStream_t stream);
RT_LAUNCH rt_launch_downscale(const uint32_t* in, int w, int h_rows, int f, uint32_t* out, hipStream_t stream);
RT_LAUNCH rt_launch_ssao(const rt::SsaoArgs* A, hipStream_t stream);

RT_LAUNCH rt_launch_wide_gather(const rt::GTri* tris, const int32_t* slot, const uint32_t* leaf_of_slot,
                                const int32_t* tri_id, const int32_t* tri_mat, int n, rt::GTri* wtris, uint4* wmeta,
                                hipStream_t stream);
RT_LAUNCH rt_launch_risk_box_init(float* B, size_t nentries, hipStream_t stream);
RT_LAUNCH rt_launch_wide_risk(const rt::GTri* wtris, const uint4* wmeta, const rt::GNode* onodes,
                              const rt::WNode* wnodes, const uint32_t* tri_leaf, const uint32_t* parent, uint32_t* K,
                              float* B, unsigned long long* risk, int n, int nnodes, const rt::WRiskArgs* A,
                              uint32_t* cap, const float* cap_dir, hipStream_t stream);
RT_LAUNCH rt_launch_wide_cut(const rt::WNode* wnodes, int nnodes, int budget, int max_depth, uint32_t* buf, hipStream_t stream);
RT_LAUNCH rt_launch_wide_mask(const rt::WNode* wnodes, int nnodes, const uint32_t* parent, const uint32_t* cut, int budget,
                              const rt::WMaskCam* C, uint32_t* words, hipStream_t stream);
RT_LAUNCH rt_launch_wide_entry(const rt::WNode* wnodes, int nnodes, const rt::WMaskCam* C, const uint32_t* words, int K,
                               int fan, int max_depth, uint4* out, hipStream_t stream);
RT_LAUNCH rt_launch_ocone(const rt::OConeEnt* E, const rt::GTri* tris, const uint32_t* todo, int n, const float lo[3],
                          const int32_t dim[3], double h, double r, double slack, double QS, double cos_cap,
                          uint2* cells, size_t ncells, hipStream_t stream);

RT_LAUNCH rt_launch_xform_points(const float m[16], float* pts, int64_t n, uint32_t* nonfinite, hipStream_t stream);
RT_LAUNCH rt_launch_gather_points(const float* verts, int64_t nv, const int32_t* idx, float* tri9, int64_t npts,
                                  uint32_t* flags, hipStream_t stream);

RT_LAUNCH rt_launch_refl_level0(const rt::KParams* P, rt::FrameRec* fr1, unsigned int* nfr1, hipStream_t stream);
RT_LAUNCH rt_launch_refl_stage(rt::ReflStage stage, const rt::KParams* P, const rt::ReflArgs* A, hipStream_t stream);
RT_LAUNCH rt_launch_refl_keys(const rt::KParams* P, const rt::FrameRec* fr, int n, uint32_t* keys, int32_t* idx,
                              hipStream_t stream);
RT_LAUNCH rt_launch_refl_sort_frames(const rt::FrameRec* fr, const int32_t* order, int n, rt::FrameRec* frs,
                                     hipStream_t stream);
RT_LAUNCH rt_launch_refl_shadow_keys(const rt::KParams* P, const rt::SampleRec* sm, const int32_t* list, int n,
                                     uint32_t* keys, hipStream_t stream);

RT_LAUNCH rt_launch_raster_stage(rt::RasterStage stage, const rt::KParams* P, const rt::RasterArgs* A, int npieces,
                                 hipStream_t stream);
RT_LAUNCH rt_launch_raster_shade(const rt::KParams* P, const rt::RasterArgs* A, rt::FrameRec* fr1, unsigned int* nfr1,
                                 hipStream_t stream);
```

### raytracercpp_amd/csrc/renderer.cpp

```cpp
#include "renderer.hpp"
#include "multidev.hpp"

#include <hipcub/hipcub.hpp>

#include <cstdlib>

#include <algorithm>
#include <chrono>
#include <cmath>
#include <cstring>
#include <thread>

#include "host_scene.hpp"
#include "launch.hpp"
#include "octree_gpu.hpp"
#include "wbvh_quick_gpu.hpp"

namespace rt {

DevBuf::~DevBuf() { release(); }

void DevBuf::release()
{
    if (p) {
// ... 17 lines not shown
    if (e != hipSuccess) {
        p = nullptr;
        return e;
    }
    bytes = n;
    return hipSuccess;
}

hipError_t WideDev::reserve(int64_t nodes, int64_t tris)
{
    nn = nodes;
    nt = tris;
    const size_t n = (size_t)nn, t = (size_t)nt;
    hipError_t e;
    if ((e = b_nodes.reserve(n * sizeof(WNode))) != hipSuccess || (e = b_tris.reserve(t * sizeof(GTri))) != hipSuccess ||
        (e = b_meta.reserve(t * 16)) != hipSuccess || (e = b_tmp.reserve(wide_tmp_bytes(n, t))) != hipSuccess)
        return e;
    return b_links.reserve(wide_links_bytes(n, t));
}

void WideDev::swap(WideDev& o)
{
    DevBuf* mine[5] = {&b_nodes, &b_tris, &b_meta, &b_tmp, &b_links};
    DevBuf* theirs[5] = {&o.b_nodes, &o.b_tris, &o.b_meta, &o.b_tmp, &o.b_links};
    for (int i = 0; i < 5; i++) mine[i]->swap(*theirs[i]);
    std::swap(nn, o.nn);
    std::swap(nt, o.nt);
}

static float ms_since(std::chrono::steady_clock::time_point t)
{
    return std::chrono::duration<float, std::milli>(std::chrono::steady_clock::now() - t).count();
}

Knobs Knobs::from_env()
{
    Knobs k;
    auto on = [](const char* name, bool dflt) {
        const char* v = getenv(name);
        return v ? v[0] != '0' : dflt;
    };
    auto flag = [](const char* name, bool dflt) {
        const char* v = getenv(name);
        return v ? atoi(v) != 0 : dflt;
    };
    auto num = [](const char* name, int dflt) {
        const char* v = getenv(name);
        return v ? atoi(v) : dflt;
    };
    auto real = [](const char* name, float dflt) {
        const char* v = getenv(name);
        return v ? (float)atof(v) : dflt;
    };
    k.wbvh = on("RT_WBVH", true);
    k.seg = on("RT_SEG", true);
    k.seg_oct = on("RT_SEG_OCTREE", false);
    k.cones = on("RT_CONES", true);
    k.lslab = on("RT_LSLAB", true);
    k.plain = on("RT_PLAIN", true);
    k.plain_octree = on("RT_PLAIN_OCTREE", true);
    k.quick_wbvh = on("RT_WBVH_QUICK_FIRST", true);
    k.fused_ssaa = on("RT_FUSED_SSAA", true);
    k.refl_engine = on("RT_REFL_ENGINE", true);
    k.debug_waves = getenv("RT_DEBUG_WAVES") != nullptr;
    k.exact = on("RT_EXACT", false);
    k.risk = on("RT_WBVH_RISK", true);
    k.heavy = on("RT_HEAVY_FIRST", true);
    if (getenv("RT_HEAVY_GROUP"))
        k.heavy_group = num("RT_HEAVY_GROUP", 0) > 1 ? SPLIT_G : 0;
    k.heavy_split = std::max(0.0f, real("RT_HEAVY_SPLIT", k.heavy_split));
    k.heavy_split_exp = std::max(0.0f, real("RT_HEAVY_SPLIT_EXP", k.heavy_split_exp));
    k.heavy_split_exp_overlap = std::max(0.0f, real("RT_HEAVY_SPLIT_EXP_OVERLAP", k.heavy_split_exp_overlap));
    if (getenv("RT_SPLIT_PARTS"))
        k.split_parts = num("RT_SPLIT_PARTS", 0) == 2 * SPLIT_G ? 2 * SPLIT_G : SPLIT_G;
    k.refl_defer = std::max(0, num("RT_REFL_DEFER", k.refl_defer));
    k.refl_feed = std::min(64, std::max(0, num("RT_REFL_FEED", k.refl_feed)));
    k.refl_sample_major = flag("RT_REFL_SAMPLE_MAJOR", k.refl_sample_major);
    k.refl_shadow_sort = flag("RT_REFL_SHADOW_SORT", k.refl_shadow_sort);
    k.refl_sorted_frames = flag("RT_REFL_SORTED_FRAMES", k.refl_sorted_frames);
    k.risk_cap = flag("RT_RISK_CAP", k.risk_cap);
    k.scene_bound = flag("RT_SCENE_BOUND", k.scene_bound);
    k.tile_mask = flag("RT_TILE_MASK", k.tile_mask);
    k.tile_start = flag("RT_TILE_START", k.tile_start);
    k.cut_budget = std::min((int)W_CUT_MAX, std::max((int)W_WIDTH, num("RT_TILE_MASK_CUT", k.cut_budget)));
    k.ocone = flag("RT_OCONE", k.ocone);
    k.ocone_dim = std::min(1024, std::max(1, num("RT_OCONE_DIM", k.ocone_dim)));
    k.inject_fail = num("RT_INJECT_FRAME_FAIL", 0);
    k.async_accel = on("RT_ASYNC_ACCEL", true);
    k.gpu_build = flag("RT_GPU_BUILD", k.gpu_build);
    k.gpu_xform = on("RT_GPU_XFORM", true);
    k.accel_hold = flag("RT_ACCEL_HOLD", k.accel_hold);
    k.accel_defer = flag("RT_ACCEL_DEFER", k.accel_defer);
    const int chunk = num("RT_REFL_CHUNK_LOG2", k.refl_chunk_log2);
    if (chunk >= 10 && chunk <= 27)
        k.refl_chunk_log2 = chunk;
    return k;
}

Renderer::Renderer(int device) : knobs_(Knobs::from_env()), device_(device)
{
    rt_default_settings(&s_);
    mat::identity(c2w_);
    mat::identity(w2c_);
    mat::identity(prev_object_);
    int rw, rh;
    render_size(rw, rh);
    img_w_ = rw;
    img_h_ = rh;
    aspect_ = (float)rw / rh;
    update_camera_projection();
}

int Renderer::init(std::string& err)
{
    hipError_t e = hipSetDevice(device_);
    if (e == hipSuccess)
        e = hipStreamCreateWithFlags(&stream_, hipStreamNonBlocking);
    if (e == hipSuccess)
        e = hipStreamCreateWithFlags(&accel_stream_, hipStreamNonBlocking);
    if (e == hipSuccess)
        e = hipStreamCreateWithFlags(&fence_stream_, hipStreamNonBlocking);
    if (e == hipSuccess)
        e = hipDeviceGetAttribute(&num_cus_, hipDeviceAttributeMultiprocessorCount, device_);
    for (int i = 0; i < 4 && e == hipSuccess; i++)
        e = hipEventCreate(&ev_[i]);
    geo_.init(device_, stream_);
    if (e == hipSuccess)
        e = risk_fence_.create();
    if (e == hipSuccess)
        e = cut_fence_.create();
    if (e == hipSuccess)
        e = query_fence_.create();
    if (e != hipSuccess) {
        err = std::string("HIP init failed: ") + hipGetErrorString(e);
        return RT_EHIP;
    }
    return RT_OK;
}

Renderer::~Renderer()
{
    if (accel_thread_.joinable())
        accel_thread_.join();
    hipSetDevice(device_);
    sync_slots();
    if (accel_stream_) hipStreamDestroy(accel_stream_);
    for (auto& e : ev_)
        if (e) hipEventDestroy(e);
    risk_fence_.destroy();
    cut_fence_.destroy();
    query_fence_.destroy();
    for (auto& e : ring_)
        if (e) hipEventDestroy(e);
    for (auto& b : band_slot_)
        b.fence.destroy();
    if (fence_stream_) hipStreamDestroy(fence_stream_);
    if (stream_) hipStreamDestroy(stream_);
    for (hipEvent_t ev : display_ev_)
        if (ev) hipEventDestroy(ev);
    if (display_stream_) hipStreamDestroy(display_stream_);
    if (display_host_) hipHostFree(display_host_);
    for (void* q : display_old_)
        hipHostFree(q);
}

int Renderer::fail(int code, const std::string& msg)
// ... 1410 lines not shown
    rt_settings keep = s_;
    s_.hybrid_rasterization_tracing = 1;
    int rc = trace_frame();
    s_.hybrid_rasterization_tracing = keep.hybrid_rasterization_tracing;
    return rc;
}

int Renderer::trace_frame()
{
    if (validate() != RT_OK)
        return fail(RT_EINVAL, "invalid scene: material index out of range or enabled texture map missing");
    if (check_frame() != RT_OK)
        return fail(RT_EUNSUPPORTED, "reflective materials with max_recursion_depth > 15, a raster frame with "
                                     "reflections and no BVH, or more than 2^27 triangles to rasterise");
    int rc = ensure_device_scene();
    if (rc != RT_OK)
        return rc;
    KParams P;
    fill_params(P);
    last_seg_ = P.seg_scale;
    size_t npx = (size_t)P.rw * P.rh;
    hipError_t e;
    if ((e = d_counters_.reserve(NCOUNTER_WORDS * 8)) != hipSuccess)
        return hip_fail(e, "hipMalloc (counters)");
    const int prev_w = img_w_, prev_h = img_h_;
    const bool prev_internal = img_is_internal_, prev_rendered = rendered_;
    if ((rc = begin_internal_image(P.rw, P.rh)) != RT_OK)
        return rc;
    struct Restore {
        Renderer* r;
        int w, h;
        bool internal, rendered, armed = true;
        ~Restore()
        {
            if (!armed)
                return;
            std::lock_guard<std::recursive_mutex> g(r->image_mu_);
            r->img_w_ = w;
            r->img_h_ = h;
            r->img_is_internal_ = internal;
            r->rendered_ = rendered && !internal;
        }
    } restore{this, prev_w, prev_h, prev_internal, prev_rendered};
    if (knobs_.inject_fail > 0 && ++frames_started_ == knobs_.inject_fail)
        return fail(RT_EHIP, "injected frame failure (RT_INJECT_FRAME_FAIL)");
    if (want_rgba_ && (e = d_rgba_.reserve(npx * 16)) != hipSuccess) return hip_fail(e, "hipMalloc (rgba)");
    if (want_hit_ && ((e = d_hit_id_.reserve(npx * 4)) != hipSuccess || (e = d_hit_t_.reserve(npx * 4)) != hipSuccess))
        return hip_fail(e, "hipMalloc (hit)");
    if (want_shadow_ && (e = d_shadow_.reserve(npx)) != hipSuccess) return hip_fail(e, "hipMalloc (shadow)");
    if (s_.enable_ssao && ((e = d_zbuf_.reserve(npx * 4)) != hipSuccess || (e = d_nbuf_.reserve(npx * 16)) != hipSuccess))
        return hip_fail(e, "hipMalloc (z / normal buffers)");
    P.zbuf = s_.enable_ssao ? d_zbuf_.as<float>() : nullptr;
    P.nbuf = s_.enable_ssao ? d_nbuf_.as<float4>() : nullptr;
    P.band_rows = P.rh;
    P.nranks = 1;
    P.rank = 0;
    P.local_rows = P.rh;
    P.tiles_x = (P.rw + 7) / 8;
    P.tiles_y = (P.rh + 7) / 8;
    P.argb = d_internal_.as<uint32_t>();
    P.rgba = want_rgba_ ? d_rgba_.as<float4>() : nullptr;
    P.hit_id = want_hit_ ? d_hit_id_.as<int32_t>() : nullptr;
    P.hit_t = want_hit_ ? d_hit_t_.as<float>() : nullptr;
    P.shadow = want_shadow_ ? d_shadow_.as<uint8_t>() : nullptr;
    P.counters = d_counters_.as<unsigned long long>();
    if (knobs_.debug_waves) {
        if ((e = d_dbg_.reserve((size_t)DBG_WAVES * DBG_WORDS * 8)) != hipSuccess ||
            (e = hipMemsetAsync(d_dbg_.p, 0, (size_t)DBG_WAVES * DBG_WORDS * 8, stream_)) != hipSuccess)
            return hip_fail(e, "debug buffer");
        P.dbg = d_dbg_.as<unsigned long long>();
    }
    if (wait_slots(stream_) != RT_OK)
        return RT_EHIP;
    if ((rc = prepare_risk(P, stream_)) != RT_OK || (rc = prepare_mask(P, stream_, mask_main_)) != RT_OK)
        return rc;
    bool zeroed = false;
    if ((rc = prepare_heavy(P, tc_main_, stream_, 0, &zeroed)) != RT_OK)
        return rc;
    if (!zeroed && (e = hipMemsetAsync(d_counters_.p, 0, NCOUNTER_WORDS * 8, stream_)) != hipSuccess)
        return hip_fail(e, "hipMemsetAsync");
    hipEventRecord(ev_[0], stream_);
    if ((rc = launch_frame(P, stream_)) != RT_OK) return rc;
    hipEventRecord(ev_[1], stream_);
    unsigned long long cnt[NCOUNTERS] = {};
    if ((e = hipMemcpyAsync(cnt, d_counters_.p, sizeof(cnt), hipMemcpyDeviceToHost, stream_)) != hipSuccess)
        return hip_fail(e, "counters");
    if ((e = hipStreamSynchronize(stream_)) != hipSuccess) return hip_fail(e, "ray_trace_kernel");
    hipEventElapsedTime(&kernel_ms_, ev_[0], ev_[1]);
    last_primary_ = (int64_t)npx;
    take_counters(cnt);
    aux_valid_ = true;
    ssao_ready_ = s_.enable_ssao;
    post_ms_ = 0;
    restore.armed = false;
    return RT_OK;
}

int Renderer::post_process()
{
    if (!rendered_)
        return fail(RT_ESTATE, "post_process before ray_trace");
    if (!img_is_internal_)
        return RT_OK;
    hipError_t e = hipSetDevice(device_);
    if (e != hipSuccess) return hip_fail(e, "hipSetDevice");
    post_ms_ = 0;
    if (s_.enable_ssao) {
        if (!ssao_ready_)
            return fail(RT_ESTATE, "post_process: enable_ssao but the last frame was rendered without it");
        int rc = launch_ssao();
        if (rc != RT_OK)
            return rc;
    }
    if (!s_.enable_ssaa)
        return RT_OK;
    int f = s_.ssaa_factor;
    if (img_w_ % f != 0 || img_h_ % f != 0)
        return RT_OK;
    int dw = img_w_ / f, dh = img_h_ / f;
    {
        std::lock_guard<std::recursive_mutex> g(image_mu_);
        if ((e = d_image_.reserve((size_t)dw * dh * 4)) != hipSuccess) return hip_fail(e, "hipMalloc (ssaa)");
    }
    hipEventRecord(ev_[2], stream_);
    if ((e = rt_launch_downscale(d_internal_.as<uint32_t>(), img_w_, img_h_, f, d_image_.as<uint32_t>(), stream_)) !=
        hipSuccess)
        return hip_fail(e, "downscale launch");
    hipEventRecord(ev_[3], stream_);
    if ((e = hipStreamSynchronize(stream_)) != hipSuccess) return hip_fail(e, "downscale");
    float ms = 0;
    hipEventElapsedTime(&ms, ev_[2], ev_[3]);
    post_ms_ += ms;
    std::lock_guard<std::recursive_mutex> g(image_mu_);
    img_w_ = dw;
    img_h_ = dh;
    img_is_internal_ = false;
    return RT_OK;
}

int Renderer::launch_ssao()
{
    hipError_t e;
    size_t npx = (size_t)img_w_ * img_h_;
    if ((e = d_ao_.reserve(npx * 4)) != hipSuccess) return hip_fail(e, "hipMalloc (ssao)");
    SsaoArgs A;
    std::memset(&A, 0, sizeof(A));
    A.z = d_zbuf_.as<float>();
    A.n = d_nbuf_.as<float4>();
    A.ao = d_ao_.as<int32_t>();
    A.argb = d_internal_.as<uint32_t>();
    A.w = img_w_;
    A.h = img_h_;
    A.simd_w = img_w_ - img_w_ % 8;
    A.count = s_.ssao_sample_count;
    A.radius = s_.ssao_radius;
    A.amount = s_.ssao_amount;
    const double pi = 3.14159265358979323846;
    A.fovm = (float)std::tan(fov_ / 2 / 180 * pi);
    A.tanv = std::tan(((float)pi / 180) * (fov_ / 2));
    A.aspect = aspect_;
    A.seed = s_.rng_seed;
    std::memcpy(A.proj, proj_, sizeof(A.proj));
    hipEventRecord(ev_[2], stream_);
    if ((e = rt_launch_ssao(&A, stream_)) != hipSuccess) return hip_fail(e, "ssao launch");
    hipEventRecord(ev_[3], stream_);
    if ((e = hipStreamSynchronize(stream_)) != hipSuccess) return hip_fail(e, "ssao");
// ... 289 lines not shown
        return fail(RT_EUNSUPPORTED, "reflective materials with max_recursion_depth > 15, a raster frame with "
                                     "reflections and no BVH, or more than 2^27 triangles to rasterise");
    int rc = ensure_device_scene();
    if (rc != RT_OK)
        return rc;
    if (!stream)
        stream = stream_;
    KParams P;
    fill_params(P);
    last_seg_ = P.seg_scale;
    hipError_t e;
    int si = -1;
    for (int i = 0; i < band_nslots_; i++)
        if (band_slot_[i].stream == stream) si = i;
    if (si < 0) {
        if (band_nslots_ < BAND_SLOTS) {
            si = band_nslots_++;
            if ((e = band_slot_[si].fence.create()) != hipSuccess)
                return hip_fail(e, "hipEventCreate");
        } else {
            si = 0;
            for (int i = 1; i < BAND_SLOTS; i++)
                if (band_slot_[i].used < band_slot_[si].used) si = i;
            if ((e = band_slot_[si].fence.sync()) != hipSuccess)
                return hip_fail(e, "render_bands_device: recycling a stream slot");
        }
        band_slot_[si].stream = stream;
    }
    band_slot_[si].used = ++band_uses_;
    const bool slot_only = !P.has_reflection && !s_.hybrid_rasterization_tracing;
    if (!slot_only && wait_slots(stream) != RT_OK)
        return RT_EHIP;
    BandSlot& S = band_slot_[si];
    band_last_ = si;
    int f = s_.enable_ssaa ? s_.ssaa_factor : 1;
    P.band_rows = band_rows * f;
    P.nranks = nranks;
    P.rank = rank;
    P.local_rows = lrows * f;
    uint64_t layout_key = 0;
    if (bands) {
        const int nb = (s_.image_height + band_rows - 1) / band_rows;
        std::vector<int32_t> host(bands, bands + nbands);
        host.resize((size_t)nbands + nb, -1);
        for (int i = 0; i < nbands; i++)
            host[(size_t)nbands + bands[i]] = i;
        if (host != S.map_host || nb != S.map_nb) {
            if ((e = S.fence.sync()) != hipSuccess)
                return hip_fail(e, "render_band_list_device: waiting for the slot's last launch");
            if ((e = S.map.reserve(host.size() * 4)) != hipSuccess ||
                (e = hipMemcpy(S.map.p, host.data(), host.size() * 4, hipMemcpyHostToDevice)) != hipSuccess)
                return hip_fail(e, "band list upload");
            S.map_host.swap(host);
            S.map_nb = nb;
        }
        P.band_map = S.map.as<int32_t>();
        P.band_inv = P.band_map + nbands;
        layout_key = 1469598103934665603ull;
        for (int32_t b : S.map_host)
            layout_key = (layout_key ^ (uint64_t)(uint32_t)b) * 1099511628211ull;
    }
    P.tiles_x = (P.rw + 7) / 8;
    P.tiles_y = (P.local_rows + 7) / 8;
    if ((e = S.counters.reserve(NCOUNTER_WORDS * 8)) != hipSuccess) return hip_fail(e, "hipMalloc (counters)");
    const bool fused = (f == 2 || f == 4 || f == 8) && slot_only && knobs_.fused_ssaa && P.rw % 8 == 0 &&
                       P.local_rows % 8 == 0;
    uint32_t* target = d_out;
    if (f > 1 && !fused) {
        if ((e = S.tmp.reserve((size_t)P.rw * P.local_rows * 4)) != hipSuccess)
            return hip_fail(e, "hipMalloc (band)");
        target = S.tmp.as<uint32_t>();
    }
    P.argb = fused ? nullptr : target;
    if (fused) {
        P.ds_out = d_out;
        P.ds_shift = f == 2 ? 1 : (f == 4 ? 2 : 3);
    }
    P.counters = S.counters.as<unsigned long long>();
    if (ring_.empty()) {
        ring_.resize(2 * EV_RING, nullptr);
        for (auto& ev : ring_)
            if ((e = hipEventCreate(&ev)) != hipSuccess) return hip_fail(e, "hipEventCreate");
    }
    if ((rc = prepare_risk(P, stream)) != RT_OK || (rc = prepare_mask(P, stream, S.mask)) != RT_OK)
        return rc;
    bool zeroed = false;
    bool overlapped = false;
    for (int i = 0; i < band_nslots_ && !overlapped; i++)
        overlapped = i != si && band_slot_[i].fence.busy();
    if ((rc = prepare_heavy(P, S.tc, stream, layout_key, &zeroed, overlapped)) != RT_OK)
        return rc;
    if (!zeroed && (e = hipMemsetAsync(S.counters.p, 0, NCOUNTER_WORDS * 8, stream)) != hipSuccess)
        return hip_fail(e, "hipMemsetAsync");
    S.tc.band_rows = band_rows;
    S.tc.ssaa = f;
    S.tc.bands.resize(lrows / band_rows);
    for (int i = 0; i < (int)S.tc.bands.size(); i++)
        S.tc.bands[i] = bands ? bands[i] : i * nranks + rank;
    hipEventRecord(ring_[2 * ring_next_], stream);
    if ((rc = launch_frame(P, stream)) != RT_OK) return rc;
    hipEventRecord(ring_[2 * ring_next_ + 1], stream);
    ring_next_ = (ring_next_ + 1) % EV_RING;
    if (ring_count_ < EV_RING) ring_count_++;
    if (f > 1 && !fused && (e = rt_launch_downscale(target, P.rw, P.local_rows, f, d_out, stream)) != hipSuccess)
        return hip_fail(e, "downscale launch");
    if ((e = S.fence.record(stream, fence_stream_)) != hipSuccess)
        return hip_fail(e, "hipEventRecord");
    return RT_OK;
}

int Renderer::prepare_risk(KParams& P, hipStream_t stream)
{
    P.wrisk = nullptr;
    P.risk_G = 0.0f;
    P.risk_nl = 0.0f;
    P.risk_nu = 0.0f;
    P.risk_cap = nullptr;
    P.sb_valid = 0;
    if (P.wnodes && knobs_.scene_bound && wide_.nn > 0) {
        if (!sb_root_valid_) {
            if (!wb_on_device_ && !lead_ && !wb_.nodes.empty())
                sb_root_ = wb_.nodes[0];
            else {
                const hipError_t e = hipMemcpy(&sb_root_, wide_.nodes(), sizeof(WNode), hipMemcpyDeviceToHost);
                if (e != hipSuccess)
                    return hip_fail(e, "download (the wide BVH's root)");
            }
            sb_root_valid_ = true;
        }
        const WSceneBound B = wbvh_scene_bound(sb_root_, P.cam_pos, P.light, P.scene_scale, W_QS_CLOSEST);
        std::memcpy(P.sb_lo, B.lo, sizeof P.sb_lo);
        std::memcpy(P.sb_hi, B.hi, sizeof P.sb_hi);
        P.sb_valid = B.valid;
    }
    if (!P.wnodes || !knobs_.risk || wide_.nn <= 0 || !d_wrisk_.p || !wide_.b_links.p)
        return RT_OK;
    const WRiskView R = wide_risk_view(d_wrisk_.p, (size_t)wide_.nn);
    float cap_dir[2][3];
    for (int sel = 0; sel < 2; sel++) {
        const float* X = sel == 0 ? P.cam_pos : P.light;
        double v[3], l = 0;
        for (int a = 0; a < 3; a++) {
            v[a] = 0.5 * ((double)oct_root_.dn[a] + (double)oct_root_.df[a]) - (double)X[a];
            l += v[a] * v[a];
        }
        l = std::sqrt(l);
        for (int a = 0; a < 3; a++)
            cap_dir[sel][a] = l > 0 && l < INFINITY ? (float)(v[a] / l) : (a == 0 ? 1.0f : 0.0f);
    }
    hipError_t e;
    if (!risk_valid_ || std::memcmp(risk_cam_, P.cam_pos, sizeof risk_cam_) ||
        std::memcmp(risk_light_, P.light, sizeof risk_light_)) {
        if (wait_slots(stream) != RT_OK)
            return RT_EHIP;
        const float lo[3] = {oct_root_.dn[0], oct_root_.dn[1], oct_root_.dn[2]};
        const float hi[3] = {oct_root_.df[0], oct_root_.df[1], oct_root_.df[2]};
        const WRiskArgs A = wbvh_risk_args(lo, hi, P.scene_scale, P.cam_pos, P.light, W_QS_CLOSEST, W_QS_SHADOW);
        risk_valid_ = false;
        std::memcpy(risk_cap_dir_, cap_dir, sizeof risk_cap_dir_);
        if ((e = hipMemsetD32Async(reinterpret_cast<hipDeviceptr_t>(R.keys), 0x7F800000, R.entries, stream)) != hipSuccess ||
            (e = hipMemsetD32Async(reinterpret_cast<hipDeviceptr_t>(R.caps), 0x7F800000, 2, stream)) != hipSuccess ||
            (e = rt_launch_risk_box_init(R.boxes, R.entries, stream)) != hipSuccess ||
            (e = rt_launch_wide_risk(P.wtris, P.wmeta, P.nodes, P.wnodes, wide_.tri_leaf(), wide_.parent(), R.keys, R.boxes,
                                     R.words, (int)wide_.nt, (int)wide_.nn, &A, R.caps, &risk_cap_dir_[0][0], stream)) !=
                hipSuccess ||
            (e = risk_fence_.record(stream, fence_stream_)) != hipSuccess)
            return hip_fail(e, "wide_risk_kernel");
        risk_valid_ = true;
        std::memcpy(risk_cam_, P.cam_pos, sizeof risk_cam_);
        std::memcpy(risk_light_, P.light, sizeof risk_light_);
        risk_G_ = A.ray_G;
        risk_nl_ = A.ray_nl;
        risk_nu_ = A.ray_nu;
    } else if ((e = risk_fence_.wait_on(stream)) != hipSuccess)
        return hip_fail(e, "hipStreamWaitEvent (risk bits)");
    P.wrisk = reinterpret_cast<const uint64_t*>(R.words);
    P.risk_G = risk_G_;
    P.risk_nl = risk_nl_;
    P.risk_nu = risk_nu_;
    if (knobs_.risk_cap) {
        P.risk_cap = reinterpret_cast<const float*>(R.caps);
        std::memcpy(P.cap_dir, risk_cap_dir_, sizeof P.cap_dir);
    }
    return RT_OK;
}

int Renderer::prepare_mask(KParams& P, hipStream_t stream, MaskSlot& M)
{
    P.tile_mask = nullptr;
    P.mask_wpr = 0;
    P.tile_start = nullptr;
    P.start_bw = 0;
    mask_last_ = nullptr;
    starts_last_ = false;
    mask_seen_ = true;
    if (!knobs_.tile_mask || !P.wnodes || !P.plain || P.has_reflection || P.zbuf || P.nbuf || wide_.nn <= 0 || !wide_.b_links.p ||
        s_.hybrid_rasterization_tracing)
        return RT_OK;
    const WMaskCam C = wbvh_mask_cam(P.proj_inv, P.cam_to_world, P.proj_mode, P.proj_w, P.c2w_affine, P.cam_pos, P.light,
                                     P.scene_scale, W_QS_CLOSEST, P.rw, P.rh);
    if (!C.valid)
        return RT_OK;
    hipError_t e;
    if (!cut_valid_) {
        if (wait_slots(stream) != RT_OK)
            return RT_EHIP;
        if ((e = d_cut_.reserve((size_t)(2 * W_CUT_MAX + 1) * 4)) != hipSuccess)
            return hip_fail(e, "hipMalloc (tile mask cut)");
        if ((e = rt_launch_wide_cut(P.wnodes, (int)wide_.nn, knobs_.cut_budget, W_CUT_DEPTH, d_cut_.as<uint32_t>(), stream)) !=
                hipSuccess ||
            (e = cut_fence_.record(stream, fence_stream_)) != hipSuccess)
            return hip_fail(e, "wide_cut_kernel");
        cut_valid_ = true;
        cut_gen_++;
    }
    if (M.cut_gen != cut_gen_ || std::memcmp(&C, &M.cam, sizeof C)) {
        M.cut_gen = 0;
        if ((e = M.words.reserve((size_t)C.bh * C.wpr * 4)) != hipSuccess)
            return hip_fail(e, "hipMalloc (tile mask)");
        if ((e = cut_fence_.wait_on(stream)) != hipSuccess ||
            (e = rt_launch_wide_mask(P.wnodes, (int)wide_.nn, wide_.parent(), d_cut_.as<uint32_t>(),
                                     knobs_.cut_budget, &C, M.words.as<uint32_t>(), stream)) != hipSuccess)
            return hip_fail(e, "wide_mask_kernel");
        M.cut_gen = cut_gen_;
        std::memcpy(&M.cam, &C, sizeof C);
        M.starts_valid = false;
        M.launches = 0;
    }
    M.launches++;
    if (knobs_.tile_start && !M.starts_valid && M.launches >= 2) {
        if ((e = M.starts.reserve((size_t)C.bh * C.bw * sizeof(uint4))) != hipSuccess)
            return hip_fail(e, "hipMalloc (entry sets)");
        if ((e = rt_launch_wide_entry(P.wnodes, (int)wide_.nn, &C, M.words.as<uint32_t>(), W_ENTRY_K, W_ENTRY_FAN,
                                      W_CUT_DEPTH, M.starts.as<uint4>(), stream)) != hipSuccess)
            return hip_fail(e, "wide_entry_kernel");
        M.starts_valid = true;
    }
    P.tile_mask = M.words.as<uint32_t>();
    P.mask_wpr = C.wpr;
    if (M.starts_valid) {
        P.tile_start = M.starts.as<uint4>();
        P.start_bw = C.bw;
        starts_last_ = true;
    }
    mask_last_ = &M;
    return RT_OK;
}

int Renderer::prepare_heavy(KParams& P, TileCost& T, hipStream_t stream, uint64_t layout_key, bool* zeroed,
                            bool overlapped)
{
    if (zeroed)
        *zeroed = false;
    P.tile_cost = nullptr;
    P.heavy_list = nullptr;
    P.heavy_bits = nullptr;
    P.heavy_ctr = nullptr;
    P.heavy_group = 0;
    if (!knobs_.heavy || P.has_reflection || s_.hybrid_rasterization_tracing)
        return RT_OK;
    const int ntiles = P.tiles_x * P.tiles_y;
    if (ntiles <= 0)
        return RT_OK;
    const size_t nb = ((size_t)ntiles + 31) / 32;
    hipError_t e;
    const size_t stats_off = ((size_t)ntiles * 4 + nb * 4 + 7) / 8 * 8;
    if ((e = T.cost.reserve((size_t)ntiles * 4)) != hipSuccess ||
        (e = T.heavy.reserve(stats_off + 4 * 8 + 2 * 16)) != hipSuccess)
        return hip_fail(e, "hipMalloc (tile costs)");
    unsigned long long* stats = reinterpret_cast<unsigned long long*>(static_cast<char*>(T.heavy.p) + stats_off);
    int32_t* ctrs = reinterpret_cast<int32_t*>(stats + 4);
    uint64_t key = 1469598103934665603ull;
    for (int64_t v : {(int64_t)P.rw, (int64_t)P.rh, (int64_t)P.local_rows, (int64_t)P.tiles_x, (int64_t)P.tiles_y,
                      (int64_t)P.band_rows, (int64_t)P.rank, (int64_t)P.nranks, (int64_t)T.cost.bytes,
                      (int64_t)layout_key})
        key = (key ^ (uint64_t)v) * 1099511628211ull;
    if (key != T.key && ((e = hipMemsetAsync(T.cost.p, 0, (size_t)ntiles * 4, stream)) != hipSuccess ||
                         (e = hipMemsetAsync(stats, 0, 4 * 8 + 2 * 16, stream)) != hipSuccess))
        return hip_fail(e, "hipMemsetAsync (tile costs)");
    T.key = key;
    T.parity ^= 1u;
    T.ntiles = ntiles;
    T.tiles_x = P.tiles_x;
    T.tiles_y = P.tiles_y;
    int32_t* list = T.heavy.as<int32_t>();
    uint32_t* bits = reinterpret_cast<uint32_t*>(list + ntiles);
    int32_t* ctr = ctrs + 4 * T.parity;
    const int G = knobs_.heavy_group;
    const bool split = G > 1 && !P.has_reflection && P.plain && !P.zbuf && !P.nbuf && P.wnodes && P.nnodes > 0 &&
                       (!P.ds_out || ((1 << P.ds_shift) <= SPLIT_ROWS && (1 << P.ds_shift) <= SPLIT_COLS));
    unsigned long long* stats_next = stats + 2 * T.parity;
    const double share = (double)ntiles / (double)((int64_t)((P.rw + 7) / 8) * ((P.rh + 7) / 8));
    const float split_bar = knobs_.heavy_split *
                            (float)std::pow(std::min(1.0, std::max(share, 1e-6)),
                                            -(double)(overlapped ? knobs_.heavy_split_exp_overlap : knobs_.heavy_split_exp));
    if ((e = rt_launch_heavy_prep(&P, T.cost.as<uint32_t>(), ntiles, list, bits, ctr, ctrs + 4 * (T.parity ^ 1u),
                                  stats + 2 * (T.parity ^ 1u), stats_next, split_bar, split ? G : 0, stream)) != hipSuccess)
        return hip_fail(e, "heavy_prep_kernel");
    P.tile_cost = T.cost.as<uint32_t>();
    P.tile_stats = stats_next;
    last_tc_ = &T;
    P.heavy_list = list;
    P.heavy_bits = bits;
    P.heavy_ctr = ctr;
    P.heavy_group = split ? G : 0;
    P.split_parts = knobs_.split_parts > 0 ? knobs_.split_parts : G;
    if (zeroed)
        *zeroed = true;
    return RT_OK;
}

int Renderer::wait_slots(hipStream_t stream)
{
    for (int i = 0; i < band_nslots_; i++) {
        BandSlot& b = band_slot_[i];
        if (b.stream == stream)
            continue;
        hipError_t e = b.fence.wait_on(stream);
        if (e != hipSuccess)
            return hip_fail(e, "hipStreamWaitEvent (frames in flight)");
    }
    hipError_t e = query_fence_.wait_on(stream);
    if (e != hipSuccess)
        return hip_fail(e, "hipStreamWaitEvent (ray queries in flight)");
    return RT_OK;
}

int Renderer::sync_slots()
// ... 344 lines not shown
    info[1] = bh;
    info[2] = wpr;
    info[3] = on ? 1 : 0;
    info[4] = 0;
    const size_t nw = (size_t)bh * wpr;
    if (!out)
        return RT_OK;
    if (cap < (int64_t)nw)
        return fail(RT_EINVAL, "tile_mask: the buffer is too small");
    if (!on) {
        const WMaskRect all = {0, 0, bw - 1, bh - 1};
        for (int y = 0; y < bh; y++)
            for (int w = 0; w < wpr; w++)
                out[(size_t)y * wpr + w] = wbvh_mask_word(all, w);
        return RT_OK;
    }
    hipError_t e = hipDeviceSynchronize();
    uint32_t ncut = 0;
    if (e == hipSuccess)
        e = hipMemcpy(&ncut, d_cut_.as<uint32_t>() + 2 * W_CUT_MAX, 4, hipMemcpyDeviceToHost);
    if (e == hipSuccess && src == 0)
        e = hipMemcpy(out, mask_last_->words.p, nw * 4, hipMemcpyDeviceToHost);
    if (e != hipSuccess)
        return hip_fail(e, "tile_mask");
    info[4] = (int32_t)ncut;
    if (src == 1) {
        std::vector<WNode> nodes((size_t)wide_.nn);
        if ((e = hipMemcpy(nodes.data(), wide_.nodes(), nodes.size() * sizeof(WNode), hipMemcpyDeviceToHost)) != hipSuccess)
            return hip_fail(e, "download (wide BVH nodes)");
        std::vector<uint32_t> cut, words, parent(nodes.size());
        if ((e = hipMemcpy(parent.data(), wide_.parent(), parent.size() * 4, hipMemcpyDeviceToHost)) != hipSuccess)
            return hip_fail(e, "download (wide BVH parents)");
        wbvh_cut_host(nodes.data(), (int64_t)nodes.size(), knobs_.cut_budget, W_CUT_DEPTH, W_QS_CLOSEST, cut);
        wbvh_mask_host(nodes.data(), (int64_t)nodes.size(), parent.data(), cut, mask_last_->cam, words);
        if (cut.size() != ncut)
            return fail(RT_ESTATE, "tile_mask: the host's cut differs from the device's in size");
        std::memcpy(out, words.data(), nw * 4);
    }
    return RT_OK;
}

int Renderer::tile_starts(int src, uint32_t* out, int64_t cap, int32_t info[3])
{
    hipSetDevice(device_);
    if (!mask_seen_)
        return fail(RT_ESTATE, "tile_starts: no frame launch yet");
    if (src != 0 && src != 1)
        return fail(RT_EINVAL, "tile_starts: src is 0 (device) or 1 (host)");
    int rw, rh;
    render_size(rw, rh);
    const bool on = mask_last_ != nullptr && starts_last_;
    const int bw = mask_last_ ? mask_last_->cam.bw : (rw + 7) / 8, bh = mask_last_ ? mask_last_->cam.bh : (rh + 7) / 8;
    info[0] = bw;
    info[1] = bh;
    info[2] = on ? 1 : 0;
    const size_t nw = (size_t)bw * bh * W_ENTRY_MAX;
    if (!out)
        return RT_OK;
    if (cap < (int64_t)nw)
        return fail(RT_EINVAL, "tile_starts: the buffer is too small");
    if (!on) {
        for (size_t i = 0; i < nw; i++)
            out[i] = i % W_ENTRY_MAX ? W_EMPTY : 0u;
        return RT_OK;
    }
    hipError_t e = hipDeviceSynchronize();
    if (e == hipSuccess && src == 0)
        e = hipMemcpy(out, mask_last_->starts.p, nw * 4, hipMemcpyDeviceToHost);
    if (e != hipSuccess)
        return hip_fail(e, "tile_starts");
    if (src == 1) {
        const WMaskCam& C = mask_last_->cam;
        std::vector<WNode> nodes((size_t)wide_.nn);
        std::vector<uint32_t> words((size_t)C.bh * C.wpr), sets;
        if ((e = hipMemcpy(nodes.data(), wide_.nodes(), nodes.size() * sizeof(WNode), hipMemcpyDeviceToHost)) != hipSuccess ||
            (e = hipMemcpy(words.data(), mask_last_->words.p, words.size() * 4, hipMemcpyDeviceToHost)) != hipSuccess)
            return hip_fail(e, "download (wide BVH nodes, mask words)");
        wbvh_entry_host(nodes.data(), (int64_t)nodes.size(), C, words.data(), W_ENTRY_K, W_ENTRY_FAN, W_CUT_DEPTH, sets);
        std::memcpy(out, sets.data(), nw * 4);
    }
    return RT_OK;
}

void Renderer::take_counters(const unsigned long long* cnt)
{
    last_shadow_ = (int64_t)cnt[0];
    last_refl_ = (int64_t)cnt[1];
    for (int i = 0; i < 4; i++) last_work_[i] = (int64_t)cnt[4 + i];
    for (int i = 0; i < 3; i++) last_work_[4 + i] = (int64_t)cnt[10 + i];
    last_work_[7] = (int64_t)cnt[14];
    for (int i = 0; i < 6; i++) last_uncert_[i] = (int64_t)cnt[16 + i];
    for (int i = 0; i < 6; i++) last_wave_[i] = (int64_t)cnt[22 + i];
}

float render(Renderer& renderer, int* rc)
{
    auto t0 = std::chrono::steady_clock::now();
    int r;
    if (renderer.multi_active() && !renderer.render_settings().enable_ssao) {
        r = renderer.render_multi();
    } else {
        r = renderer.render_settings().hybrid_rasterization_tracing ? renderer.raster_trace() : renderer.ray_trace();
        if (r == RT_OK)
            r = renderer.post_process();
    }
    if (rc)
        *rc = r;
    return std::chrono::duration<float, std::milli>(std::chrono::steady_clock::now() - t0).count();
}

}
```

### raytracercpp_amd/csrc/renderer.hpp

```cpp
#pragma once

#include <stdint.h>

#include <array>
#include <atomic>
#include <memory>
#include <mutex>
#include <string>
#include <thread>
#include <vector>

#include "../../include/rt_mi355x.h"
#include "devbuf.hpp"
#include "kparams.hpp"
#include "ocone.hpp"
#include "octree.hpp"
#include "tri_geometry.hpp"
#include "wbvh.hpp"
#include "wide_layout.hpp"

namespace rt {

struct OctreeGpuScratch;
struct OctreeDevInfo;
struct WQuickGpuScratch;

struct WideDev {
    DevBuf b_nodes, b_tris, b_meta, b_tmp, b_links;
    int64_t nn = 0, nt = 0;
    WNode* nodes() const { return b_nodes.as<WNode>(); }
    GTri* tris() const { return b_tris.as<GTri>(); }
    uint4* meta() const { return b_meta.as<uint4>(); }
    int32_t* slot() const { return at<int32_t>(b_tmp, wide_tmp_slot_off((size_t)nn, (size_t)nt)); }
    uint32_t* leaf_of_slot() const { return at<uint32_t>(b_tmp, wide_tmp_leaf_of_slot_off((size_t)nn, (size_t)nt)); }
    uint32_t* tri_leaf() const { return at<uint32_t>(b_links, wide_links_tri_leaf_off((size_t)nn, (size_t)nt)); }
    uint32_t* parent() const { return at<uint32_t>(b_links, wide_links_parent_off((size_t)nn, (size_t)nt)); }
    hipError_t reserve(int64_t nodes, int64_t tris);
    void clear() { nn = nt = 0; }
    void swap(WideDev& o);

private:
    template <class T> static T* at(const DevBuf& b, size_t off) { return reinterpret_cast<T*>(b.as<char>() + off); }
};

struct Fence {
    hipError_t create()
    {
        hipError_t e = hipEventCreateWithFlags(&done_, hipEventDisableTiming);
        return e == hipSuccess ? hipEventCreateWithFlags(&mark_, hipEventDisableTiming) : e;
    }
    void destroy()
    {
        if (done_) hipEventDestroy(done_);
        if (mark_) hipEventDestroy(mark_);
        done_ = mark_ = nullptr;
        live_ = false;
    }
    hipError_t record(hipStream_t stream, hipStream_t fence_stream)
    {
        hipError_t e;
        if ((e = hipEventRecord(mark_, stream)) == hipSuccess && (e = hipStreamWaitEvent(fence_stream, mark_, 0)) == hipSuccess &&
            (e = hipEventRecord(done_, fence_stream)) == hipSuccess)
            live_ = true;
        return e;
    }
    hipError_t wait_on(hipStream_t stream) const { return live_ ? hipStreamWaitEvent(stream, done_, 0) : hipSuccess; }
    hipError_t sync() const { return live_ ? hipEventSynchronize(done_) : hipSuccess; }
    bool live() const { return live_; }
    bool busy() const { return live_ && hipEventQuery(done_) == hipErrorNotReady; }

private:
    hipEvent_t mark_ = nullptr, done_ = nullptr;
    bool live_ = false;
};

struct HostTex {
    int w = 0, h = 0;
    std::vector<float> rgba;
};

struct Knobs {
    bool wbvh = true;
    bool seg = true;
    bool seg_oct = false;
    bool cones = true;
    bool lslab = true;
    bool plain = true;
    bool quick_wbvh = true;
    bool plain_octree = true;
    bool fused_ssaa = true;
    bool refl_engine = true;
    int refl_chunk_log2 = 27;
    bool debug_waves = false;
    bool exact = false;
    bool risk = true;
    bool heavy = true;
    int heavy_group = SPLIT_G;
    int split_parts = 0;
    float heavy_split_exp = 0.5f;
    float heavy_split_exp_overlap = 0.7f;
    float heavy_split = 0.5f;
    int refl_defer = 32;
    int refl_feed = 24;
    bool refl_sample_major = true;
    bool refl_shadow_sort = true;
    bool refl_sorted_frames = true;
    bool risk_cap = true;
    bool scene_bound = true;
    bool tile_mask = true;
    bool tile_start = true;
    int cut_budget = W_CUT_BUDGET;
    bool ocone = true;
    int ocone_dim = 128;
    int inject_fail = 0;
    bool gpu_build = false;
    bool gpu_xform = true;
    bool async_accel = true;
    bool accel_hold = false;
    bool accel_defer = false;
    static Knobs from_env();
};

class Renderer {
public:
    explicit Renderer(int device);
    ~Renderer();
    int init(std::string& err);

    const rt_settings& render_settings() const { return s_; }
    int set_settings(const rt_settings& s);
    int set_exact(bool on);
    void set_device_build(bool on) { knobs_.gpu_build = on; }
    int64_t device_builds() const { return device_builds_; }
    int64_t device_wide_builds() const { return device_wide_builds_; }
    int64_t device_transforms() const { return geo_.transforms(); }
    int64_t device_ingests() const { return geo_.ingests(); }
    int64_t accel_builds() const { return accel_builds_; }
    void set_accel_deferred(bool on) { knobs_.accel_defer = on; }
    int set_triangles_device(const float* d_verts, int64_t nv, const int32_t* d_idx, const int32_t* mat,
                             const float* uv6, int64_t n, hipStream_t stream);
    int update_vertices_device(const float* d_verts, int64_t nv, const int32_t* d_idx, hipStream_t stream);
    int finish_accel();
    bool exact() const { return knobs_.exact; }
    int change_render_size(int w, int h);
    int set_triangles(const float* tri9, const int32_t* mat, const float* uv6, int64_t n);
    int add_sphere(float cx, float cy, float cz, float r, int mat);
    int add_plane(float px, float py, float pz, float nx, float ny, float nz, int mat);
    int clear_geometry();
    int set_materials(const float* mats16, int n);
    int material_count() const { return (int)(mats_.size() / MAT_STRIDE); }
    int change_camera_fov(float fov);
    int change_camera_aspect_ratio(float aspect);
    int set_light_position(float x, float y, float z);
    int set_camera_transform(const float m[16]);
    int apply_transformation_to_camera(const float m[16]);
    int set_camera_matrices(const float pos[3], const float proj_inv[16], const float c2w[16]);
    void get_camera_matrices(float pos[3], float proj_inv[16], float c2w[16]) const;
    int set_camera_projection(const float proj[16], const float w2c[16]);
    int set_camera_lens(float fov, float aspect);
    int set_object_transform(const float m[16]);
    int reset_previous_transform();
    int get_triangles(float* tri9, int64_t* n);
    int set_texture(int slot, int w, int h, const float* rgba);
    int set_skybox(const int32_t w[6], const int32_t h[6], const float* const faces[6]);
    int reconstruct_bvh_new();
    int destroy_bvh();
    int ray_trace();
    int raster_trace();
    int post_process();
    int get_image(uint32_t* argb, int32_t* w, int32_t* h);
    void lock_image() { image_mu_.lock(); }
    void unlock_image() { image_mu_.unlock(); }
    std::string display_error()
    {
        std::lock_guard<std::recursive_mutex> g(image_mu_);
        return display_err_;
    }
    int get_ssao_buffers(float* z, float* n4, int32_t* ao);
    int request_aux(bool rgba, bool hit, bool shadow);
    int get_internal(uint32_t* argb, float* rgba, int32_t* hit_id, float* hit_t, uint8_t* shadow);
    int get_stats(rt_stats* out) const;

    int local_rows(int band_rows, int rank, int nranks) const;
    int render_bands_device(int band_rows, int rank, int nranks, uint32_t* d_out, hipStream_t stream);
    int render_band_list_device(int band_rows, const int32_t* bands, int nbands, uint32_t* d_out, hipStream_t stream);
    int band_costs(hipStream_t stream, double* costs, int nbands);
    int kernel_times(float* ms, int n);
    int band_counters(unsigned long long out[2]);
    int tile_mask(int src, uint32_t* out, int64_t cap, int32_t info[5]);
    int tile_starts(int src, uint32_t* out, int64_t cap, int32_t info[3]);
    int debug_read(uint64_t* out, int64_t n);
    int tile_costs(uint32_t* out, int64_t n, int32_t* tiles_x, int32_t* tiles_y);
    int origin_cones(uint32_t* out, int64_t n, int32_t dims[3], float lo_ih[4]);
    int set_devices(const int* ids, int n);
    bool multi_active() const { return multi_ != nullptr; }
    int render_multi();

    int trace_rays(const float* orig, const float* dir, int64_t n, int32_t* id, float* t, float* u, float* v,
                   uint8_t* ret);
    int trace_rays_device(const float* d_orig, const float* d_dir, int64_t n, int32_t* d_id, float* d_t, float* d_u,
                          float* d_v, uint8_t* d_ret, int64_t* d_counts, hipStream_t stream);
    int is_shadowed_device(const float* d_point, const float* d_normal, int64_t n, const float* light,
                           uint8_t* d_shadowed, hipStream_t stream);
    void device_ray_queries(int64_t calls[2], int64_t rays[2]) const;
    int wide_query(const float* orig, const float* dir, int64_t n, int kind, float* o_out, float* d_out,
                   int32_t* status, int32_t* id, float* t, float* u, float* v, uint8_t* shadow);
    int risk_words(int src, uint64_t* out, int64_t cap, int64_t* count, int64_t* violations);
    int trace_ray_colors(const float* orig, const float* dir, int64_t n, int depth, float* rgba, int32_t* src,
                         float* t, uint8_t* found, uint8_t* shadow);

    const std::string& error() const { return err_; }

private:
    int fail(int code, const std::string& msg);
    int hip_fail(hipError_t e, const char* what);
    void render_size(int& w, int& h) const;
    void update_camera_projection();
    int ensure_device_scene();
    int rebuild_geometry();
    int build_octree(int64_t n, bool& dev_built);
    int upload_octree_tables(bool dev_built, hipError_t& e);
    int build_quick_wide(bool dev_built, hipError_t& e);
    int upload_materials();
    int upload_textures();
    int validate() const;
    void fill_params(KParams& P) const;
    int launch_trace(const KParams& P, hipStream_t stream);
    int launch_raster(const KParams& P, hipStream_t stream);
    int launch_frame(const KParams& P, hipStream_t stream)
    {
        return s_.hybrid_rasterization_tracing ? launch_raster(P, stream) : launch_trace(P, stream);
    }
    int check_frame() const;
    int launch_ssao();
    int trace_frame();
    int refl_level(const KParams& P, int level, int nframes, hipStream_t stream);
    int refl_level1_begin(const KParams& P, hipStream_t stream);
    int refl_level1_finish(const KParams& P, hipStream_t stream, const char* what, bool run_empty);
    int wait_slots(hipStream_t stream);
    int sync_slots();
    Fence query_fence_;
    int64_t query_calls_[2] = {}, query_rays_[2] = {};
    int begin_ray_query(const char* what, const void* const* ptrs, int nptrs, int n_required, int64_t n,
                        hipStream_t stream, KParams& P);
    int end_ray_query(int kind, int64_t n, hipStream_t stream);

    Knobs knobs_;
    int device_;
    uint64_t geom_ver_ = 0, mats_ver_ = 0, tex_ver_ = 0;
    uint64_t mir_geom_ = ~0ull, mir_mats_ = ~0ull, mir_tex_ = ~0ull;
    std::thread accel_thread_;
    std::atomic<int> accel_state_{0};
    std::atomic<bool> oc_done_{false};
    bool tree_pending_ = false;
    float oc_ms_ = 0.0f;
    std::string accel_err_;
    hipStream_t accel_stream_ = nullptr;
    hipStream_t fence_stream_ = nullptr;
    float accel_ms_[3] = {};
    bool cones_ready_ = false, wide_ready_ = false, lslab_ready_ = false;
    int wide_tree_ = 0;
    uint64_t accel_ver_ = 0;
    int install_wide(int tree);
    void drop_accel();
    void start_accel();
    int poll_accel(bool wait, bool release = false);
    int mirror_from(Renderer& lead);
    const Renderer* lead_ = nullptr;
    uint64_t mir_accel_ = ~0ull;
    int adopt_from_lead();
    int64_t host_builds_ = 0;
    int64_t device_builds_ = 0;
    std::unique_ptr<OctreeGpuScratch> oct_gpu_;
    DevBuf d_oct_info_;
    int build_octree_device(int64_t n, bool& built);
    int64_t device_wide_builds_ = 0;
    std::unique_ptr<OctreeDevInfo> oct_dev_info_;
    std::unique_ptr<WQuickGpuScratch> wq_gpu_;
    bool wb_on_device_ = false;
    WStats wb_dev_stats_;
    int build_wide_device(bool& built);
    int host_wide();
    TriGeometry geo_;
    void touch_geometry() { geom_dirty_ = true, ++geom_ver_; }
    int host_tris(const std::vector<float>*& tri);
    int ingest_positions(const float* d_verts, int64_t nv, const int32_t* d_idx, int64_t n, hipStream_t stream);
    bool unrefined_ = false;
    int64_t accel_builds_ = 0;
    struct MultiDev;
    std::unique_ptr<MultiDev> multi_;
    int num_cus_ = 256;
    hipStream_t stream_ = nullptr;
    hipEvent_t ev_[4] = {nullptr, nullptr, nullptr, nullptr};
    std::string err_;

    rt_settings s_;

    std::vector<int32_t> shape_kind_;
    std::vector<float> shape_;
    std::vector<int32_t> shape_mat_;
    std::vector<float> mats_;
    float cam_pos_[3] = {0, 0, 0};
    float fov_ = 45.0f, near_ = 0.1f, far_ = 1000.0f, aspect_ = 1.0f;
    float proj_[16], proj_inv_[16], c2w_[16], w2c_[16];
    float light_[3] = {3, 3, 2};
    float prev_object_[16];
    HostTex tex_[TEX_SLOTS];
    HostTex sky_[6];
    bool has_bvh_ = false;

    FlatOctree oct_;
    int64_t oct_nn_ = 0, oct_nt_ = 0;
    int oct_levels_ = 0;
    GNode oct_root_{};
    OctreeStats oct_stats_{};
    bool has_uv_dev_ = false;
    bool geom_dirty_ = true, mats_dirty_ = true, tex_dirty_ = true;
    DevBuf d_nodes_, d_tris_, d_tri_id_, d_tri_mat_, d_tri_uv_, d_mats_;
    DevBuf d_tex_[TEX_SLOTS], d_sky_[6];
    DevBuf d_internal_, d_image_, d_rgba_, d_hit_id_, d_hit_t_, d_shadow_, d_counters_;
    DevBuf d_zbuf_, d_nbuf_, d_ao_;
    std::vector<float> cones_;
    DevBuf d_cones_;
    std::vector<float> lslab_;
    DevBuf d_lslab_;
    std::vector<float> lsin_;
    DevBuf d_lsin_;
    WBvh wb_;
    WideDev wide_;
    WBvh wb_next_;
    WideDev wide_next_;
    OConeGrid ocg_, ocg_next_;
    DevBuf d_ocone_, d_ocone2_, d_oc_ent_, d_oc_todo_;
    bool ocone_ready_ = false;
    float risk_cap_dir_[2][3] = {};
    hipError_t upload_wide(const WBvh& w, WideDev& d, hipStream_t stream);
    int reserve_risk(size_t nodes);
    DevBuf d_wrisk_;
    bool risk_valid_ = false;
    WNode sb_root_{};
    bool sb_root_valid_ = false;
    float risk_cam_[3] = {0, 0, 0}, risk_light_[3] = {0, 0, 0};
    float risk_G_ = 0.0f, risk_nl_ = 0.0f, risk_nu_ = 0.0f;
    Fence risk_fence_;
    int prepare_risk(KParams& P, hipStream_t stream);
    struct MaskSlot {
        DevBuf words;
        DevBuf starts;
        bool starts_valid = false;
        uint32_t launches = 0;
        WMaskCam cam{};
        uint64_t cut_gen = 0;
    };
    DevBuf d_cut_;
    bool cut_valid_ = false, mask_seen_ = false;
    uint64_t cut_gen_ = 0;
    MaskSlot mask_main_;
    MaskSlot* mask_last_ = nullptr;
    bool starts_last_ = false;
    Fence cut_fence_;
    int prepare_mask(KParams& P, hipStream_t stream, MaskSlot& M);
    DevBuf d_dbg_;
    bool ssao_ready_ = false;
    DevBuf d_rcount_, d_roff_, d_pieces_, d_piece_uv_, d_zkey_, d_big_, d_scan_tmp_;
    bool want_rgba_ = false, want_hit_ = false, want_shadow_ = false;
    bool aux_valid_ = false;
    std::recursive_mutex image_mu_;
    hipStream_t display_stream_ = nullptr;
    hipEvent_t display_ev_[8] = {};
    void* display_host_ = nullptr;
    size_t display_bytes_ = 0;
    std::vector<void*> display_old_;
    int frames_started_ = 0;
    std::string display_err_;
    int begin_internal_image(int rw, int rh);
    int img_w_ = 0, img_h_ = 0;
    bool img_is_internal_ = false;
    bool rendered_ = false;

    struct ReflLevel {
        DevBuf fr, ret, sm, hit, cnt, list, sort, sort_tmp, res, frs, slist;
    };
    static constexpr int REFL_LEVELS = 18;
    ReflLevel refl_[REFL_LEVELS];

    struct TileCost {
        DevBuf cost, heavy;
        uint64_t key = 0;
        int ntiles = 0, tiles_x = 0, tiles_y = 0;
        uint32_t parity = 0;
        int band_rows = 0, ssaa = 1;
        std::vector<int32_t> bands;
    };
    int prepare_heavy(KParams& P, TileCost& T, hipStream_t stream, uint64_t layout_key = 0, bool* zeroed = nullptr,
                      bool overlapped = false);
    int render_bands_impl(int band_rows, int rank, int nranks, const int32_t* bands, int nbands, uint32_t* d_out,
                          hipStream_t stream);
    const TileCost* last_tc_ = nullptr;
    TileCost tc_main_;
    struct BandSlot {
        hipStream_t stream = nullptr;
        DevBuf counters, tmp;
        TileCost tc;
        Fence fence;
        DevBuf map;
        std::vector<int32_t> map_host;
        int map_nb = 0;
        uint64_t used = 0;
        MaskSlot mask;
    };
    static constexpr int BAND_SLOTS = 8;
    BandSlot band_slot_[BAND_SLOTS];
    int band_nslots_ = 0, band_last_ = -1;
    uint64_t band_uses_ = 0;
    static constexpr int EV_RING = 256;
    std::vector<hipEvent_t> ring_;
    int ring_next_ = 0, ring_count_ = 0;

    int64_t last_primary_ = 0, last_shadow_ = 0, last_refl_ = 0;
    float last_seg_ = 0;
    int64_t last_work_[8] = {};
    int64_t last_wave_[6] = {};
    int64_t last_uncert_[6] = {};
    void take_counters(const unsigned long long* cnt);
    float kernel_ms_ = 0, post_ms_ = 0, build_ms_ = 0;
    float build_split_ms_[4] = {};
};

float render(Renderer& renderer, int* rc = nullptr);

}
```

### raytracercpp_amd/renderer.py

```python
from __future__ import annotations

import ctypes as C
import time
from typing import Optional, Sequence

import numpy as np

from . import _lib
from ._lib import RtSettings, RtStats, check, f32, ptr
from .scene import RenderSettings, SceneData, SHAPE_SPHERE, TEX_AO, TEX_DIFFUSE, TEX_NORMAL, TEX_DISPLACEMENT, \
    TEX_ROUGHNESS, TEX_SKYSPHERE

_f32p = C.POINTER(C.c_float)
_i32p = C.POINTER(C.c_int32)
_u32p = C.POINTER(C.c_uint32)
_u8p = C.POINTER(C.c_uint8)


def _to_c(st: RenderSettings) -> RtSettings:
    c = RtSettings()
    _lib.lib().rt_default_settings(C.byref(c))
    for name, typ in RtSettings._fields_:
        if hasattr(st, name):
            v = getattr(st, name)
# ... 354 lines not shown
    def is_shadowed_device(self, points, normals, light=None, out=None, stream=None):
        import torch
        pp, np_, n = _lib.device_ray_args(points, normals, self.device, ("points", "normals"))
        if n > 1 << 30:
            raise ValueError(f"is_shadowed_device: {n} pairs, at most 2^30 are taken")
        stream = self._ray_stream(stream)
        if out is None:
            with torch.cuda.stream(stream):
                out = torch.empty(n, dtype=torch.uint8, device=points.device)
        sp = _lib.device_ray_out(out, "out", torch.uint8, n, self.device)
        lp = None if light is None else f32(light).reshape(3)
        self._call("rt_is_shadowed_device", C.c_void_p(pp), C.c_void_p(np_), n, ptr(lp, _f32p), C.c_void_p(sp),
                   self._stream_ptr(stream, self.device))
        return out

    def device_ray_queries(self):
        calls, rays = np.zeros(2, np.int64), np.zeros(2, np.int64)
        i64p = C.POINTER(C.c_int64)
        self._call("rt_get_device_ray_queries", ptr(calls, i64p), ptr(rays, i64p))
        return (int(calls[0]), int(calls[1])), (int(rays[0]), int(rays[1]))

    def wide_query(self, orig, dirs, kind=1):
        o = f32(orig).reshape(-1, 3)
        d = f32(dirs).reshape(-1, 3)
        if d.shape != o.shape:
            raise ValueError(f"wide_query: {o.shape[0]} origins but {d.shape[0]} directions")
        n = o.shape[0]
        out = dict(o=np.zeros((n, 3), np.float32), d=np.zeros((n, 3), np.float32), status=np.zeros(n, np.int32),
                   id=np.zeros(n, np.int32), t=np.zeros(n, np.float32), u=np.zeros(n, np.float32),
                   v=np.zeros(n, np.float32), shadowed=np.zeros(n, np.uint8))
        self._call("rt_wide_query", ptr(o, _f32p), ptr(d, _f32p), n, int(kind), ptr(out["o"], _f32p),
                   ptr(out["d"], _f32p), ptr(out["status"], _i32p), ptr(out["id"], _i32p), ptr(out["t"], _f32p),
                   ptr(out["u"], _f32p), ptr(out["v"], _f32p), ptr(out["shadowed"], _u8p))
        return out

    def risk_words(self, src=0):
        n, bad = C.c_int64(), C.c_int64()
        self._call("rt_risk_words", int(src), None, 0, C.byref(n), None)
        out = np.zeros(n.value, np.uint64)
        self._call("rt_risk_words", int(src), out.ctypes.data_as(C.POINTER(C.c_uint64)), out.size, C.byref(n),
                   C.byref(bad))
        return out, bad.value

    def trace_ray(self, orig, dirs, current_recursion_depth=0):
        o = f32(orig).reshape(-1, 3)
        d = f32(dirs).reshape(-1, 3)
        if d.shape != o.shape:
            raise ValueError(f"trace_ray: {o.shape[0]} origins but {d.shape[0]} directions")
        n = o.shape[0]
        rgba = np.zeros((n, 4), np.float32)
        src = np.zeros(n, np.int32)
        t = np.zeros(n, np.float32)
        found = np.zeros(n, np.uint8)
        shadowed = np.zeros(n, np.uint8)
        self._call("rt_trace_ray", ptr(o, _f32p), ptr(d, _f32p), n, int(current_recursion_depth), ptr(rgba, _f32p),
                   ptr(src, _i32p), ptr(t, _f32p), ptr(found, _u8p), ptr(shadowed, _u8p))
        return rgba, src, t, found, shadowed

    def kernel_times(self, n):
        ms = np.zeros(n, np.float32)
        self._call("rt_kernel_times", ptr(ms, _f32p), int(n))
        return ms

    def band_counters(self):
        a, b = C.c_int64(), C.c_int64()
        self._call("rt_band_counters", C.byref(a), C.byref(b))
        return a.value, b.value

    def tile_mask(self, src=0):
        info = np.zeros(5, np.int32)
        self._call("rt_tile_mask", int(src), None, 0, ptr(info, _i32p))
        bw, bh, wpr = int(info[0]), int(info[1]), int(info[2])
        words = np.zeros(bh * wpr, np.uint32)
        self._call("rt_tile_mask", int(src), ptr(words, _u32p), words.size, ptr(info, _i32p))
        bits = (words.reshape(bh, wpr)[:, :, None] >> np.arange(32, dtype=np.uint32)) & 1
        return bits.reshape(bh, wpr * 32)[:, :bw].astype(bool), {"on": bool(info[3]), "cut": int(info[4])}

    def tile_starts(self, src=0):
        info = np.zeros(3, np.int32)
        self._call("rt_tile_starts", int(src), None, 0, ptr(info, _i32p))
        sets = np.zeros((int(info[1]), int(info[0]), 4), np.uint32)
        self._call("rt_tile_starts", int(src), ptr(sets, _u32p), sets.size, ptr(info, _i32p))
        return sets, bool(info[2])

    def load_scene(self, sc: SceneData, st: RenderSettings):
        self.set_render_settings(st)
        self.change_render_size(st.image_width, st.image_height)
        self.set_camera_matrices(sc.cam_pos, sc.proj_inv, sc.cam_to_world)
        if sc.proj is not None and sc.world_to_cam is not None:
            self.set_camera_projection(sc.proj, sc.world_to_cam)
        self.set_camera_lens(*sc.lens(st))
        self.set_light_position(sc.light)
        self.set_materials(sc.materials)
        self.clear_geometry()
        for k in range(len(sc.shape_kind)):
            s = sc.shape[k]
            if sc.shape_kind[k] == SHAPE_SPHERE:
                self.add_sphere(s[:3], s[3], int(sc.shape_mat[k]))
            else:
                self.add_plane(s[:3], s[3:6], int(sc.shape_mat[k]))
        self.set_triangles(sc.tri, sc.tri_mat, sc.tri_uv)
        for slot in range(6):
            self._set_tex(slot, sc.textures.get(slot) if sc.textures else None)
        if sc.skybox is not None:
            self.set_skybox(sc.skybox)


def render(renderer: Renderer) -> float:
    ms = C.c_float()
    check(_lib.lib().rt_render(renderer._h, C.byref(ms)), "rt_render")
    return float(ms.value)
```

Baseline: 10370 Mrays/s.

## Compact covered and clear tile lists so trace waves skip background tiles

Adds a device pass that classifies each 8x8 tile against the coverage mask and stream-compacts the results into a covered list and a clear list. A new list-driven trace kernel draws its work only from covered tiles, and clear tiles are filled with the background colour in a separate cheap path. This removes per-tile mask checks and the wave dispatch spent on empty screen regions, at the cost of two extra small kernels per frame. A probe/heuristic decides when the lists are used.

```diff
diff --git a/include/rt_mi355x.h b/include/rt_mi355x.h
--- a/include/rt_mi355x.h
+++ b/include/rt_mi355x.h
@@ -197,6 +197,7 @@
 int rt_band_counters(rt_renderer *r, int64_t *shadow_rays, int64_t *reflection_rays);
 int rt_tile_mask(rt_renderer *r, int32_t src, uint32_t *words, int64_t cap, int32_t info[5]);
 int rt_tile_starts(rt_renderer *r, int32_t src, uint32_t *sets, int64_t cap, int32_t info[3]);
+int rt_tile_lists(rt_renderer *r, int32_t src, int32_t *tiles, int64_t cap, int32_t info[5]);
 
 void rt_make_transform(int32_t kind, float x, float y, float z, float out[16]);
 void rt_compose(const float a[16], const float b[16], float out[16]);
diff --git a/raytracercpp_amd/_lib.py b/raytracercpp_amd/_lib.py
--- a/raytracercpp_amd/_lib.py
+++ b/raytracercpp_amd/_lib.py
@@ -141,6 +141,7 @@
     "rt_band_counters": (C.c_int, [_H, _i64p, _i64p]),
     "rt_tile_mask": (C.c_int, [_H, C.c_int32, _u32p, C.c_int64, _i32p]),
     "rt_tile_starts": (C.c_int, [_H, C.c_int32, _u32p, C.c_int64, _i32p]),
+    "rt_tile_lists": (C.c_int, [_H, C.c_int32, _i32p, C.c_int64, _i32p]),
     "rt_make_transform": (None, [C.c_int32, C.c_float, C.c_float, C.c_float, _f32p]),
     "rt_compose": (None, [_f32p, _f32p, _f32p]),
     "rt_inverse": (None, [_f32p, _f32p]),
@@ -177,6 +178,7 @@
 GEOMETRY_INPUT = ("rt_set_triangles_device", "rt_update_vertices_device", "rt_get_device_ingests",
                   "rt_gather_triangles_device", "rt_set_accel_deferred", "rt_get_accel_builds")
 RAY_QUERIES = ("rt_trace_rays_device", "rt_is_shadowed_device", "rt_get_device_ray_queries")
+TILE_LISTS = ("rt_tile_lists",)
 
 _lib = None
 
@@ -197,7 +199,7 @@
             pass
         L = C.CDLL(LIB_PATH)
         for name, (res, args) in SIGNATURES.items():
-            if name in GEOMETRY_INPUT + RAY_QUERIES and os.environ.get("RT_LIB_PATH") and not hasattr(L, name):
+            if name in GEOMETRY_INPUT + RAY_QUERIES + TILE_LISTS and os.environ.get("RT_LIB_PATH") and not hasattr(L, name):
                 continue
             fn = getattr(L, name)
             fn.restype = res
diff --git a/raytracercpp_amd/csrc/capi.cpp b/raytracercpp_amd/csrc/capi.cpp
--- a/raytracercpp_amd/csrc/capi.cpp
+++ b/raytracercpp_amd/csrc/capi.cpp
@@ -500,6 +500,10 @@
 int rt_tile_starts(rt_renderer* r, int32_t src, uint32_t* sets, int64_t cap, int32_t info[3])
 {
     return guarded(R(r), [&] { return info ? R(r)->tile_starts(src, sets, cap, info) : RT_EINVAL; });
+}
+int rt_tile_lists(rt_renderer* r, int32_t src, int32_t* tiles, int64_t cap, int32_t info[5])
+{
+    return guarded(R(r), [&] { return info ? R(r)->tile_lists(src, tiles, cap, info) : RT_EINVAL; });
 }
 int rt_band_counters(rt_renderer* r, int64_t* shadow_rays, int64_t* reflection_rays)
 {
diff --git a/raytracercpp_amd/csrc/kernels.hip b/raytracercpp_amd/csrc/kernels.hip
--- a/raytracercpp_amd/csrc/kernels.hip
+++ b/raytracercpp_amd/csrc/kernels.hip
@@ -25,6 +25,7 @@
 #include "kparams.hpp"
 #include "rt_math.hpp"
 #include "wbvh.hpp"
+#include "tile_lists.hpp"
 #include "launch.hpp"
 
 namespace rt {
@@ -731,15 +732,17 @@
 }
 
 #if RT_PHASE_TIME
-__shared__ unsigned long long g_phase[WAVES_PER_BLOCK][8];
+constexpr int PH_PHASES = 8;
+static_assert(PH_PHASES <= DBG_WORDS, "a wave's record holds its phases");
+__shared__ unsigned long long g_phase[WAVES_PER_BLOCK][PH_PHASES + 1];
 __device__ __forceinline__ void ph_mark(int k)
 {
     const unsigned long long now = __builtin_amdgcn_s_memtime();
     const uint64_t act = __ballot(1);
     if ((int)__lane_id() == __ffsll((unsigned long long)act) - 1) {
         const int w = threadIdx.x >> 6;
-        g_phase[w][k] += now - g_phase[w][7];
-        g_phase[w][7] = now;
+        g_phase[w][k] += now - g_phase[w][PH_PHASES];
+        g_phase[w][PH_PHASES] = now;
     }
 }
 #define PH_MARK(k) ph_mark(k)
@@ -1528,12 +1531,37 @@
 
 constexpr int BQ_BATCH = 4;
 
+__device__ __forceinline__ const int32_t* tile_lists_of(const KParams& P)
+{
+    return reinterpret_cast<const int32_t*>(P.tile_mask) + P.list_off;
+}
+
+template <bool LIST>
+__device__ __forceinline__ bool shard_has(const KParams& P, int s, int t);
+
+template <bool LIST = false>
 __device__ __forceinline__ int shard_tile(const KParams& P, int s, int t)
 {
+    if (LIST && P.list_off) {
+        const int32_t* tl = tile_lists_of(P);
+        int r0, r1;
+        tile_shard_range(ldg(tl), s, TILE_SHARDS, r0, r1);
+        return t < r1 - r0 ? ldg(tl + TL_HEAD + r0 + t) : -1;
+    }
     const int r0 = (int)((long long)P.tiles_y * s / TILE_SHARDS), r1 = (int)((long long)P.tiles_y * (s + 1) / TILE_SHARDS);
     return t < (r1 - r0) * P.tiles_x ? r0 * P.tiles_x + t : -1;
 }
 
+template <bool LIST>
+__device__ __forceinline__ bool shard_has(const KParams& P, int s, int t)
+{
+    if (LIST && P.list_off) {
+        int r0, r1;
+        tile_shard_range(ldg(tile_lists_of(P)), s, TILE_SHARDS, r0, r1);
+        return t < r1 - r0;
+    }
+    return shard_tile(P, s, t) >= 0;
+}
 
 struct BlockQueue {
     unsigned int word;
@@ -1581,6 +1609,7 @@
     if (m) atomicMax(P.tile_stats + 1, (unsigned long long)m);
 }
 
+template <bool LIST = false>
 __device__ __forceinline__ int tile_queue_next_shards(const KParams& P)
 {
     const int lane = threadIdx.x & 63;
@@ -1594,7 +1623,7 @@
         const unsigned int g = (w >> 24) & 0x7fu, c = (w >> 16) & 0xffu, i = w & 0xffffu;
         if (i < c) {
             const int slot = (int)(g & 3u);
-            return shard_tile(P, g_bq.sh[slot], g_bq.base[slot] + (int)i);
+            return shard_tile<LIST>(P, g_bq.sh[slot], g_bq.base[slot] + (int)i);
         }
         if (i == c) {
             int shard = g_bq.shard, empty = g_bq.empty, b = 0, n = 0;
@@ -1605,7 +1634,7 @@
                                        (unsigned)BQ_BATCH);
                 b = __builtin_amdgcn_readfirstlane(t);
                 n = 0;
-                while (n < BQ_BATCH && shard_tile(P, shard, b + n) >= 0)
+                while (n < BQ_BATCH && shard_has<LIST>(P, shard, b + n))
                     n++;
                 if (n > 0)
                     break;
@@ -1621,7 +1650,7 @@
                 __hip_atomic_store(&g_bq.word, n > 0 ? (g1 << 24) | ((unsigned)n << 16) | 1u : 0x80000000u,
                                    __ATOMIC_RELEASE, __HIP_MEMORY_SCOPE_WORKGROUP);
             }
-            return n > 0 ? shard_tile(P, shard, b) : -1;
+            return n > 0 ? shard_tile<LIST>(P, shard, b) : -1;
         }
         for (;;) {
             unsigned int v = 0;
@@ -1635,6 +1664,7 @@
     }
 }
 
+template <bool LIST = false>
 __device__ __forceinline__ int tile_queue_next(const KParams& P)
 {
     const int lane = threadIdx.x & 63;
@@ -1651,12 +1681,12 @@
                 __hip_atomic_store(&g_bq.heavy_done, 1, __ATOMIC_RELAXED, __HIP_MEMORY_SCOPE_WORKGROUP);
         }
         for (;;) {
-            const int tile = tile_queue_next_shards(P);
+            const int tile = tile_queue_next_shards<LIST>(P);
             if (tile < 0 || !((ldg(P.heavy_bits + (tile >> 5)) >> (tile & 31)) & 1u))
                 return tile;
         }
     }
-    return tile_queue_next_shards(P);
+    return tile_queue_next_shards<LIST>(P);
 }
 
 __device__ __forceinline__ void set_wave_prio(int level)
@@ -1798,99 +1828,72 @@
 #endif
 }
 
+__device__ __noinline__ void fill_clear_tiles(const KParams& P)
+{
+    const int lane = threadIdx.x & 63;
+    const int32_t* tl = tile_lists_of(P);
+    const int nclear = ldg(tl + 1);
+    const int32_t* clear = tl + TL_HEAD + P.tiles_x * P.tiles_y;
+    const long long w = (long long)blockIdx.x * WAVES_PER_BLOCK + (threadIdx.x >> 6), W = (long long)gridDim.x * WAVES_PER_BLOCK;
+    const bool packed = P.ds_out && !P.argb && !P.rgba && !P.hit_id && !P.hit_t && !P.shadow;
+    const int sh = packed ? P.ds_shift : 0;
+    const int q = packed ? 64 >> (2 * sh) : 64;
+    const int T = 64 / q;
+    const int k = lane / q, j = lane % q;
+    const uint32_t c = color_to_argb(background());
+    const uint32_t word = qrgb((int)((c >> 16) & 0xffu), (int)((c >> 8) & 0xffu), (int)(c & 0xffu));
+    for (long long e0 = w * T; e0 < nclear; e0 += W * T) {
+        const uint64_t t0 = P.tile_cost ? __builtin_amdgcn_s_memtime() : 0ull;
+        int tile = -1;
+        if (e0 + k < nclear) {
+            tile = ldg(clear + (e0 + k));
+            if (P.heavy_bits && ((ldg(P.heavy_bits + (tile >> 5)) >> (tile & 31)) & 1u))
+                tile = -1;
+        }
+        if (tile >= 0) {
+            int tx, ty;
+            tile_xy(P, tile, tx, ty);
+            const int side = 8 >> sh;
+            const int px = tx * 8 + ((j % side) << sh);
+            const int lr = ty * 8 + ((j / side) << sh);
+            const int py = lr < P.local_rows ? global_row(P, lr) : P.rh;
+            if (px < P.rw && py < P.rh) {
+                if (packed)
+                    P.ds_out[(size_t)(lr >> sh) * (size_t)(P.rw >> sh) + (size_t)(px >> sh)] = word;
+                else
+                    fill_masked_tile(P, lr, px);
+            }
+        }
+        const uint64_t firsts = __ballot(tile >= 0 && j == 0);
+        const int n = __popcll(firsts);
+        if (n == 0)
+            continue;
+#if RT_COUNT
+        if (packed && P.counters && lane == __ffsll((unsigned long long)firsts) - 1)
+            atomicAdd(&P.counters[28], (unsigned long long)n);
+#endif
+        if (P.tile_cost) {
+            const uint64_t cy = (__builtin_amdgcn_s_memtime() - t0) / (uint64_t)n;
+            const uint32_t c32 = cy > 0xFFFFFFFFull ? 0xFFFFFFFFu : cy < 1 ? 1u : (uint32_t)cy;
+            if (tile >= 0 && j == 0) {
+                P.tile_cost[tile] = c32;
+                tile_stats_add(c32, c32);
+            }
+        }
+    }
+}
+
 template <bool REFL, bool PLAIN = false, bool OCT = false>
 __global__ __launch_bounds__(BLOCK, OCT ? RT_OCC_OCT : PLAIN ? RT_OCC_PLAIN : RT_OCC) void ray_trace_kernel(KParams P_arg)
 {
-    auto kp = __builtin_amdgcn_kernarg_segment_ptr();
-    (void)P_arg;
-    const KParams& P = *reinterpret_cast<const KParams*>((const void*)kp);
-    uint2* lv = lane_stack();
-    int lane = threadIdx.x & 63;
-    unsigned nshadow = 0, nrefl = 0;
-    tile_queue_init();
-#if RT_PHASE_TIME
-    if (PLAIN && lane == 0) {
-        for (int k = 0; k < 7; k++)
-            g_phase[threadIdx.x >> 6][k] = 0;
-        g_phase[threadIdx.x >> 6][7] = __builtin_amdgcn_s_memtime();
-    }
-#endif
-    for (;;) {
-        auto kpl = kp;
-        asm volatile("" : "+s"(kpl));
-        const KParams& P = *reinterpret_cast<const KParams*>((const void*)kpl);
-        const v3 cam = mk(P.cam_pos[0], P.cam_pos[1], P.cam_pos[2]);
-        if (PLAIN && !REFL && !OCT && P.heavy_group == SPLIT_G &&
-            !__builtin_amdgcn_readfirstlane(__hip_atomic_load(&g_bq.split_done, __ATOMIC_RELAXED, __HIP_MEMORY_SCOPE_WORKGROUP))) {
-            int t = 0;
-            if (lane == 0)
-                t = atomicAdd(P.heavy_ctr + 2, 1);
-            t = __builtin_amdgcn_readfirstlane(t);
-            if (t < P.split_parts * min(ldg(P.heavy_ctr + 3), P.tiles_x * P.tiles_y / 16)) {
-                trace_split_part<SPLIT_G>(P, lv, t, lane, nshadow);
-                continue;
-            }
-            if (lane == 0)
-                __hip_atomic_store(&g_bq.split_done, 1, __ATOMIC_RELAXED, __HIP_MEMORY_SCOPE_WORKGROUP);
-        }
-        const int tq = tile_queue_next(P);
-        if (PLAIN) PH_MARK(6);
-        if (tq < 0)
-            break;
-        const int tile = tq & 0x0fffffff;
-        if (P.heavy_list)
-            set_wave_prio(tq >> 28);
-        const uint64_t tile_t0 = __builtin_amdgcn_s_memtime();
-        int tx, ty;
-        tile_xy(P, tile, tx, ty);
-        int px = tx * 8 + (lane & 7);
-        int lr = ty * 8 + (lane >> 3);
-        int py = lr < P.local_rows ? global_row(P, lr) : P.rh;
-        if (PLAIN) PH_MARK(0);
-        if (px >= P.rw || py >= P.rh) {
-            if (P.tile_cost && lane == 0)
-                P.tile_cost[tile] = 0u;
-            continue;
-        }
-        if (PLAIN && !REFL && !OCT && P.tile_mask) {
-            const uint32_t mw = ldg(P.tile_mask + (size_t)(py >> 3) * (size_t)P.mask_wpr + (size_t)(px >> 8));
-            if (!__ballot((mw >> ((px >> 3) & 31)) & 1u)) {
-                fill_masked_tile(P, lr, px);
-                if (P.tile_cost)
-                    tile_cost_store(P, tile, tile_t0, lane);
-                continue;
-            }
-        }
-        const v3 rd = camera_dir(P, px, py, cam);
-        if (PLAIN) PH_MARK(1);
-
-        uint32_t rng = REFL ? pixel_seed((uint32_t)(py * P.rw + px), P.rng_seed) : 0u;
-        PixelOut po = trace_pixel<REFL, PLAIN, 1, OCT>(P, cam, rd, lv, rng, nshadow, nrefl,
-                                                        PLAIN && !REFL && !OCT ? tile_start_index(P, px, py) : -1);
-        size_t o = (size_t)lr * P.rw + px;
-        if (P.argb) P.argb[o] = color_to_argb(po.color);
-        if (!REFL && P.ds_out) downscale_tile(P, lane, lr, px, color_to_argb(po.color));
-        if (P.rgba) P.rgba[o] = make_float4(po.color.r, po.color.g, po.color.b, po.alpha);
-        if (P.hit_id) P.hit_id[o] = po.found ? po.src : -1;
-        if (P.hit_t) P.hit_t[o] = po.fin.t;
-        if (P.shadow) P.shadow[o] = (uint8_t)(po.found && po.shadowed);
-        if (!PLAIN && P.zbuf) write_ssao_buffers(P, o, po.found, cam, rd, po.fin);
-        if (PLAIN) PH_MARK(5);
-        if (P.tile_cost)
-            tile_cost_store(P, tile, tile_t0, lane);
-    }
-    tile_stats_flush(P, lane);
-#if RT_PHASE_TIME
-    if (PLAIN) {
-        PH_MARK(0);
-        const int wid = (int)(blockIdx.x * WAVES_PER_BLOCK + (threadIdx.x >> 6));
-        if (P.dbg && lane == 0 && wid < DBG_WAVES)
-            for (int k = 0; k < 7; k++)
-                P.dbg[DBG_WORDS * wid + k] = g_phase[threadIdx.x >> 6][k];
-    }
-#endif
-    if (nshadow) atomicAdd(&P.counters[0], (unsigned long long)nshadow);
-    if (nrefl) atomicAdd(&P.counters[1], (unsigned long long)nrefl);
+    constexpr bool LIST = false;
+#include "ray_trace_body.hpp"
+}
+
+__global__ __launch_bounds__(BLOCK, RT_OCC_PLAIN) void ray_trace_list_kernel(KParams P_arg)
+{
+    constexpr bool REFL = false, PLAIN = true, OCT = false, LIST = true;
+#include "ray_trace_body.hpp"
 }
 
 __device__ __forceinline__ v3 ld3(const float* p) { return mk(p[0], p[1], p[2]); }
@@ -3486,7 +3489,10 @@
             return hipGetLastError();
         }
         const int pblocks = plain_blocks(*P);
-        hipLaunchKernelGGL((rt::ray_trace_kernel<false, true>), dim3(pblocks), dim3(rt::BLOCK), lds, stream, *P);
+        if (P->list_off)
+            hipLaunchKernelGGL(rt::ray_trace_list_kernel, dim3(pblocks), dim3(rt::BLOCK), lds, stream, *P);
+        else
+            hipLaunchKernelGGL((rt::ray_trace_kernel<false, true>), dim3(pblocks), dim3(rt::BLOCK), lds, stream, *P);
     } else
         hipLaunchKernelGGL((rt::ray_trace_kernel<false, false>), dim3(blocks), dim3(rt::BLOCK), lds, stream, *P);
     return hipGetLastError();
@@ -3621,6 +3627,71 @@
         return hipSuccess;
     hipLaunchKernelGGL(wide_entry_kernel, dim3((nb + 255) / 256), dim3(256), 0, stream, wnodes, nnodes, *C, words, K, fan,
                        max_depth, out);
+    return hipGetLastError();
+}
+
+__global__ __launch_bounds__(256) void tile_class_kernel(rt::TileLayout L, int ntiles, unsigned long long* cls)
+{
+    const int i = (int)(blockIdx.x * 256u + threadIdx.x);
+    const int c = i < ntiles ? rt::tile_class(L, i) : (int)rt::TILE_OFF;
+    const uint64_t cov = __ballot(c == rt::TILE_COVERED), clr = __ballot(c == rt::TILE_CLEAR);
+    if ((threadIdx.x & 63) == 0 && i < ntiles) {
+        cls[2 * (i >> 6)] = cov;
+        cls[2 * (i >> 6) + 1] = clr;
+    }
+}
+
+__global__ __launch_bounds__(256) void tile_list_kernel(const unsigned long long* __restrict__ cls, int ntiles, int32_t* lists)
+{
+    __shared__ int s_cov[4], s_clr[4];
+    const int lane = (int)(threadIdx.x & 63), wv = (int)(threadIdx.x >> 6);
+    const int word0 = (int)blockIdx.x * 4, nwords = (ntiles + 63) / 64;
+    int a = 0, b = 0;
+    for (int k = (int)threadIdx.x; k < word0; k += 256) {
+        a += __popcll(cls[2 * k]);
+        b += __popcll(cls[2 * k + 1]);
+    }
+    for (int m = 32; m; m >>= 1) {
+        a += __shfl_xor(a, m);
+        b += __shfl_xor(b, m);
+    }
+    if (lane == 0) {
+        s_cov[wv] = a;
+        s_clr[wv] = b;
+    }
+    __syncthreads();
+    const int k = word0 + wv;
+    if (k >= nwords)
+        return;
+    int base_cov = s_cov[0] + s_cov[1] + s_cov[2] + s_cov[3], base_clr = s_clr[0] + s_clr[1] + s_clr[2] + s_clr[3];
+    for (int j = word0; j < k; j++) {
+        base_cov += __popcll(cls[2 * j]);
+        base_clr += __popcll(cls[2 * j + 1]);
+    }
+    const uint64_t cov = cls[2 * k], clr = cls[2 * k + 1];
+    const uint64_t below = (1ull << lane) - 1ull;
+    const int i = 64 * k + lane;
+    int32_t* covered = lists + rt::TL_HEAD;
+    int32_t* clear = covered + ntiles;
+    if ((cov >> lane) & 1ull)
+        covered[base_cov + __popcll(cov & below)] = i;
+    if ((clr >> lane) & 1ull)
+        clear[base_clr + __popcll(clr & below)] = i;
+    if (k == nwords - 1 && lane == 0) {
+        lists[0] = base_cov + __popcll(cov);
+        lists[1] = base_clr + __popcll(clr);
+    }
+}
+
+hipError_t rt_launch_tile_lists(const rt::TileLayout* L, int32_t* lists, hipStream_t stream)
+{
+    const int ntiles = L->tiles_x * L->tiles_y;
+    if (ntiles <= 0)
+        return hipSuccess;
+    unsigned long long* cls = reinterpret_cast<unsigned long long*>(lists + rt::tile_lists_class_word(ntiles));
+    const dim3 grid((unsigned)((ntiles + 255) / 256));
+    hipLaunchKernelGGL(tile_class_kernel, grid, dim3(256), 0, stream, *L, ntiles, cls);
+    hipLaunchKernelGGL(tile_list_kernel, grid, dim3(256), 0, stream, cls, ntiles, lists);
     return hipGetLastError();
 }
 
diff --git a/raytracercpp_amd/csrc/kparams.hpp b/raytracercpp_amd/csrc/kparams.hpp
--- a/raytracercpp_amd/csrc/kparams.hpp
+++ b/raytracercpp_amd/csrc/kparams.hpp
@@ -123,6 +123,7 @@
     float4* nbuf;
     uint32_t* ds_out;
     int32_t ds_shift;
+    int32_t list_off;
 };
 
 struct SsaoArgs {
diff --git a/raytracercpp_amd/csrc/launch.hpp b/raytracercpp_amd/csrc/launch.hpp
--- a/raytracercpp_amd/csrc/launch.hpp
+++ b/raytracercpp_amd/csrc/launch.hpp
@@ -5,6 +5,7 @@
 
 #include "kparams.hpp"
 #include "ocone.hpp"
+#include "tile_lists.hpp"
 #include "wbvh.hpp"
 
 namespace rt {
@@ -59,6 +60,7 @@
                               const rt::WMaskCam* C, uint32_t* words, hipStream_t stream);
 RT_LAUNCH rt_launch_wide_entry(const rt::WNode* wnodes, int nnodes, const rt::WMaskCam* C, const uint32_t* words, int K,
                                int fan, int max_depth, uint4* out, hipStream_t stream);
+RT_LAUNCH rt_launch_tile_lists(const rt::TileLayout* L, int32_t* lists, hipStream_t stream);
 RT_LAUNCH rt_launch_ocone(const rt::OConeEnt* E, const rt::GTri* tris, const uint32_t* todo, int n, const float lo[3],
                           const int32_t dim[3], double h, double r, double slack, double QS, double cos_cap,
                           uint2* cells, size_t ncells, hipStream_t stream);
diff --git a/raytracercpp_amd/csrc/ray_trace_body.hpp b/raytracercpp_amd/csrc/ray_trace_body.hpp
--- /dev/null
+++ b/raytracercpp_amd/csrc/ray_trace_body.hpp
@@ -0,0 +1,94 @@
+    auto kp = __builtin_amdgcn_kernarg_segment_ptr();
+    const KParams& P = *reinterpret_cast<const KParams*>((const void*)kp);
+    uint2* lv = lane_stack();
+    int lane = threadIdx.x & 63;
+    unsigned nshadow = 0, nrefl = 0;
+    tile_queue_init();
+#if RT_PHASE_TIME
+    if (PLAIN && lane == 0) {
+        for (int k = 0; k < PH_PHASES; k++)
+            g_phase[threadIdx.x >> 6][k] = 0;
+        g_phase[threadIdx.x >> 6][PH_PHASES] = __builtin_amdgcn_s_memtime();
+    }
+#endif
+    for (;;) {
+        auto kpl = kp;
+        asm volatile("" : "+s"(kpl));
+        const KParams& P = *reinterpret_cast<const KParams*>((const void*)kpl);
+        const v3 cam = mk(P.cam_pos[0], P.cam_pos[1], P.cam_pos[2]);
+        if (PLAIN && !REFL && !OCT && P.heavy_group == SPLIT_G &&
+            !__builtin_amdgcn_readfirstlane(__hip_atomic_load(&g_bq.split_done, __ATOMIC_RELAXED, __HIP_MEMORY_SCOPE_WORKGROUP))) {
+            int t = 0;
+            if (lane == 0)
+                t = atomicAdd(P.heavy_ctr + 2, 1);
+            t = __builtin_amdgcn_readfirstlane(t);
+            if (t < P.split_parts * min(ldg(P.heavy_ctr + 3), P.tiles_x * P.tiles_y / 16)) {
+                trace_split_part<SPLIT_G>(P, lv, t, lane, nshadow);
+                continue;
+            }
+            if (lane == 0)
+                __hip_atomic_store(&g_bq.split_done, 1, __ATOMIC_RELAXED, __HIP_MEMORY_SCOPE_WORKGROUP);
+        }
+        const int tq = tile_queue_next<LIST>(P);
+        if (PLAIN) PH_MARK(6);
+        if (tq < 0)
+            break;
+        const int tile = tq & 0x0fffffff;
+        if (P.heavy_list)
+            set_wave_prio(tq >> 28);
+        const uint64_t tile_t0 = __builtin_amdgcn_s_memtime();
+        int tx, ty;
+        tile_xy(P, tile, tx, ty);
+        int px = tx * 8 + (lane & 7);
+        int lr = ty * 8 + (lane >> 3);
+        int py = lr < P.local_rows ? global_row(P, lr) : P.rh;
+        if (PLAIN) PH_MARK(0);
+        if (px >= P.rw || py >= P.rh) {
+            if (P.tile_cost && lane == 0)
+                P.tile_cost[tile] = 0u;
+            continue;
+        }
+        if (PLAIN && !REFL && !OCT && P.tile_mask) {
+            const uint32_t mw = ldg(P.tile_mask + (size_t)(py >> 3) * (size_t)P.mask_wpr + (size_t)(px >> 8));
+            if (!__ballot((mw >> ((px >> 3) & 31)) & 1u)) {
+                fill_masked_tile(P, lr, px);
+                if (P.tile_cost)
+                    tile_cost_store(P, tile, tile_t0, lane);
+                PH_MARK(7);
+                continue;
+            }
+        }
+        const v3 rd = camera_dir(P, px, py, cam);
+        if (PLAIN) PH_MARK(1);
+
+        uint32_t rng = REFL ? pixel_seed((uint32_t)(py * P.rw + px), P.rng_seed) : 0u;
+        PixelOut po = trace_pixel<REFL, PLAIN, 1, OCT>(P, cam, rd, lv, rng, nshadow, nrefl,
+                                                        PLAIN && !REFL && !OCT ? tile_start_index(P, px, py) : -1);
+        size_t o = (size_t)lr * P.rw + px;
+        if (P.argb) P.argb[o] = color_to_argb(po.color);
+        if (!REFL && P.ds_out) downscale_tile(P, lane, lr, px, color_to_argb(po.color));
+        if (P.rgba) P.rgba[o] = make_float4(po.color.r, po.color.g, po.color.b, po.alpha);
+        if (P.hit_id) P.hit_id[o] = po.found ? po.src : -1;
+        if (P.hit_t) P.hit_t[o] = po.fin.t;
+        if (P.shadow) P.shadow[o] = (uint8_t)(po.found && po.shadowed);
+        if (!PLAIN && P.zbuf) write_ssao_buffers(P, o, po.found, cam, rd, po.fin);
+        if (PLAIN) PH_MARK(5);
+        if (P.tile_cost)
+            tile_cost_store(P, tile, tile_t0, lane);
+    }
+    if (LIST && P.list_off) {
+        fill_clear_tiles(P);
+        PH_MARK(7);
+    }
+    tile_stats_flush(P, lane);
+#if RT_PHASE_TIME
+    if (PLAIN) {
+        PH_MARK(0);
+        const int wid = (int)(blockIdx.x * WAVES_PER_BLOCK + (threadIdx.x >> 6));
+        if (P.dbg && lane == 0 && wid < DBG_WAVES)
+            for (int k = 0; k < PH_PHASES; k++)
+                P.dbg[DBG_WORDS * wid + k] = g_phase[threadIdx.x >> 6][k];
+    }
+#endif
+    if (nshadow) atomicAdd(&P.counters[0], (unsigned long long)nshadow);
+    if (nrefl) atomicAdd(&P.counters[1], (unsigned long long)nrefl);
diff --git a/raytracercpp_amd/csrc/renderer.cpp b/raytracercpp_amd/csrc/renderer.cpp
--- a/raytracercpp_amd/csrc/renderer.cpp
+++ b/raytracercpp_amd/csrc/renderer.cpp
@@ -123,6 +123,7 @@
     k.scene_bound = flag("RT_SCENE_BOUND", k.scene_bound);
     k.tile_mask = flag("RT_TILE_MASK", k.tile_mask);
     k.tile_start = flag("RT_TILE_START", k.tile_start);
+    k.tile_list = flag("RT_TILE_LIST", k.tile_list);
     k.cut_budget = std::min((int)W_CUT_MAX, std::max((int)W_WIDTH, num("RT_TILE_MASK_CUT", k.cut_budget)));
     k.ocone = flag("RT_OCONE", k.ocone);
     k.ocone_dim = std::min(1024, std::max(1, num("RT_OCONE_DIM", k.ocone_dim)));
@@ -1699,6 +1700,7 @@
     hipEventRecord(ev_[0], stream_);
     if ((rc = launch_frame(P, stream_)) != RT_OK) return rc;
     hipEventRecord(ev_[1], stream_);
+    if ((rc = probe_lists(P, stream_)) != RT_OK) return rc;
     unsigned long long cnt[NCOUNTERS] = {};
     if ((e = hipMemcpyAsync(cnt, d_counters_.p, sizeof(cnt), hipMemcpyDeviceToHost, stream_)) != hipSuccess)
         return hip_fail(e, "counters");
@@ -2154,7 +2156,7 @@
         for (auto& ev : ring_)
             if ((e = hipEventCreate(&ev)) != hipSuccess) return hip_fail(e, "hipEventCreate");
     }
-    if ((rc = prepare_risk(P, stream)) != RT_OK || (rc = prepare_mask(P, stream, S.mask)) != RT_OK)
+    if ((rc = prepare_risk(P, stream)) != RT_OK || (rc = prepare_mask(P, stream, S.mask, layout_key)) != RT_OK)
         return rc;
     bool zeroed = false;
     bool overlapped = false;
@@ -2172,6 +2174,7 @@
     hipEventRecord(ring_[2 * ring_next_], stream);
     if ((rc = launch_frame(P, stream)) != RT_OK) return rc;
     hipEventRecord(ring_[2 * ring_next_ + 1], stream);
+    if ((rc = probe_lists(P, stream)) != RT_OK) return rc;
     ring_next_ = (ring_next_ + 1) % EV_RING;
     if (ring_count_ < EV_RING) ring_count_++;
     if (f > 1 && !fused && (e = rt_launch_downscale(target, P.rw, P.local_rows, f, d_out, stream)) != hipSuccess)
@@ -2257,14 +2260,16 @@
     return RT_OK;
 }
 
-int Renderer::prepare_mask(KParams& P, hipStream_t stream, MaskSlot& M)
+int Renderer::prepare_mask(KParams& P, hipStream_t stream, MaskSlot& M, uint64_t layout_key)
 {
     P.tile_mask = nullptr;
     P.mask_wpr = 0;
     P.tile_start = nullptr;
     P.start_bw = 0;
+    P.list_off = 0;
     mask_last_ = nullptr;
     starts_last_ = false;
+    lists_last_ = false;
     mask_seen_ = true;
     if (!knobs_.tile_mask || !P.wnodes || !P.plain || P.has_reflection || P.zbuf || P.nbuf || wide_.nn <= 0 || !wide_.b_links.p ||
         s_.hybrid_rasterization_tracing)
@@ -2286,9 +2291,16 @@
         cut_valid_ = true;
         cut_gen_++;
     }
+    const int ntiles = P.tiles_x * P.tiles_y;
+    const size_t list_off = ((size_t)C.bh * C.wpr + 3) / 4 * 4;
+    const bool lists = knobs_.tile_list && ntiles > 0 && list_off + tile_lists_words(ntiles) <= (size_t)INT32_MAX;
+    const size_t need = lists ? (list_off + tile_lists_words(ntiles)) * 4 : (size_t)C.bh * C.wpr * 4;
+    if (need > M.words.bytes)
+        M.cut_gen = 0;
     if (M.cut_gen != cut_gen_ || std::memcmp(&C, &M.cam, sizeof C)) {
         M.cut_gen = 0;
-        if ((e = M.words.reserve((size_t)C.bh * C.wpr * 4)) != hipSuccess)
+        M.lists_valid = false;
+        if ((e = M.words.reserve(need)) != hipSuccess)
             return hip_fail(e, "hipMalloc (tile mask)");
         if ((e = cut_fence_.wait_on(stream)) != hipSuccess ||
             (e = rt_launch_wide_mask(P.wnodes, (int)wide_.nn, wide_.parent(), d_cut_.as<uint32_t>(),
@@ -2310,12 +2322,63 @@
     }
     P.tile_mask = M.words.as<uint32_t>();
     P.mask_wpr = C.wpr;
+    if (M.use_gen != cut_gen_) {
+        M.use_gen = cut_gen_;
+        M.list_use = -1;
+        M.list_launches = 0;
+        M.probe_pending = false;
+    }
+    if (M.probe_pending && hipEventQuery(M.probe.ev) == hipSuccess) {
+        M.probe_pending = false;
+        const unsigned long long sum = M.probe.host[0];
+        const int32_t nclear = reinterpret_cast<const int32_t*>(M.probe.host + 2)[1];
+        if (sum > 0 && nclear >= 0)
+            M.list_use = (unsigned long long)nclear * LIST_TICKET_CYCLES * LIST_MIN_SHARE_INV >= sum ? 1 : 0;
+    }
+    lists_slot_ = nullptr;
+    if (lists && M.list_use != 0) {
+        uint64_t key = 1469598103934665603ull;
+        for (int64_t v : {(int64_t)P.rw, (int64_t)P.rh, (int64_t)P.local_rows, (int64_t)P.band_rows, (int64_t)P.rank,
+                          (int64_t)P.nranks, (int64_t)layout_key})
+            key = (key ^ (uint64_t)v) * 1099511628211ull;
+        if (!M.lists_valid || key != M.list_key || M.L.band_map != P.band_map) {
+            M.lists_valid = false;
+            M.L = TileLayout{P.rw, P.rh, P.local_rows, P.band_rows, P.rank, P.nranks, P.tiles_x, P.tiles_y,
+                             P.band_map, M.words.as<uint32_t>(), C.wpr};
+            if ((e = rt_launch_tile_lists(&M.L, M.words.as<int32_t>() + list_off, stream)) != hipSuccess)
+                return hip_fail(e, "tile_list_kernel");
+            M.lists_valid = true;
+            M.list_key = key;
+            M.list_off = (int32_t)list_off;
+        }
+        P.list_off = M.list_off;
+        lists_last_ = true;
+        lists_slot_ = &M;
+    }
     if (M.starts_valid) {
         P.tile_start = M.starts.as<uint4>();
         P.start_bw = C.bw;
         starts_last_ = true;
     }
     mask_last_ = &M;
+    return RT_OK;
+}
+
+int Renderer::probe_lists(const KParams& P, hipStream_t stream)
+{
+    MaskSlot* M = lists_slot_;
+    lists_slot_ = nullptr;
+    if (!M || !P.list_off || !P.tile_stats || M->list_use >= 0 || M->probe_pending || ++M->list_launches < 2)
+        return RT_OK;
+    hipError_t e = hipSuccess;
+    if (!M->probe.host && ((e = hipHostMalloc(reinterpret_cast<void**>(&M->probe.host), 32)) != hipSuccess ||
+                           (e = hipEventCreateWithFlags(&M->probe.ev, hipEventDisableTiming)) != hipSuccess))
+        return hip_fail(e, "hipHostMalloc (list probe)");
+    if ((e = hipMemcpyAsync(M->probe.host, P.tile_stats, 16, hipMemcpyDeviceToHost, stream)) != hipSuccess ||
+        (e = hipMemcpyAsync(M->probe.host + 2, P.tile_mask + P.list_off, 8, hipMemcpyDeviceToHost, stream)) != hipSuccess ||
+        (e = hipEventRecord(M->probe.ev, stream)) != hipSuccess)
+        return hip_fail(e, "list probe");
+    M->probe_pending = true;
     return RT_OK;
 }
 
@@ -2826,6 +2889,62 @@
     return RT_OK;
 }
 
+int Renderer::tile_lists(int src, int32_t* out, int64_t cap, int32_t info[5])
+{
+    hipSetDevice(device_);
+    if (!mask_seen_)
+        return fail(RT_ESTATE, "tile_lists: no frame launch yet");
+    if (src != 0 && src != 1)
+        return fail(RT_EINVAL, "tile_lists: src is 0 (device) or 1 (host)");
+    const bool on = mask_last_ != nullptr && lists_last_;
+    for (int i = 0; i < 5; i++)
+        info[i] = 0;
+    if (!on)
+        return RT_OK;
+    const MaskSlot& M = *mask_last_;
+    const int ntiles = M.L.tiles_x * M.L.tiles_y;
+    info[0] = M.L.tiles_x;
+    info[1] = M.L.tiles_y;
+    info[4] = 1;
+    hipError_t e = hipDeviceSynchronize();
+    std::vector<int32_t> covered, clear;
+    if (src == 0) {
+        std::vector<int32_t> all(TL_HEAD + 2 * (size_t)ntiles);
+        if (e == hipSuccess)
+            e = hipMemcpy(all.data(), M.words.as<int32_t>() + M.list_off, all.size() * 4, hipMemcpyDeviceToHost);
+        if (e != hipSuccess)
+            return hip_fail(e, "tile_lists");
+        if (all[0] < 0 || all[1] < 0 || (int64_t)all[0] + all[1] > ntiles)
+            return fail(RT_ESTATE, "tile_lists: the device's counts exceed the launch's tiles");
+        covered.assign(all.begin() + TL_HEAD, all.begin() + TL_HEAD + all[0]);
+        clear.assign(all.begin() + TL_HEAD + ntiles, all.begin() + TL_HEAD + ntiles + all[1]);
+    } else {
+        std::vector<uint32_t> words((size_t)M.cam.bh * M.cam.wpr);
+        std::vector<int32_t> map;
+        TileLayout L = M.L;
+        if (e == hipSuccess)
+            e = hipMemcpy(words.data(), M.words.p, words.size() * 4, hipMemcpyDeviceToHost);
+        if (e == hipSuccess && L.band_map) {
+            map.resize((size_t)((L.local_rows + L.band_rows - 1) / L.band_rows));
+            e = hipMemcpy(map.data(), L.band_map, map.size() * 4, hipMemcpyDeviceToHost);
+            L.band_map = map.data();
+        }
+        if (e != hipSuccess)
+            return hip_fail(e, "tile_lists");
+        L.mask = words.data();
+        tile_lists_host(L, covered, clear);
+    }
+    info[2] = (int32_t)covered.size();
+    info[3] = (int32_t)clear.size();
+    if (!out)
+        return RT_OK;
+    if (cap < (int64_t)(covered.size() + clear.size()))
+        return fail(RT_EINVAL, "tile_lists: the buffer is too small");
+    std::copy(covered.begin(), covered.end(), out);
+    std::copy(clear.begin(), clear.end(), out + covered.size());
+    return RT_OK;
+}
+
 void Renderer::take_counters(const unsigned long long* cnt)
 {
     last_shadow_ = (int64_t)cnt[0];
diff --git a/raytracercpp_amd/csrc/renderer.hpp b/raytracercpp_amd/csrc/renderer.hpp
--- a/raytracercpp_amd/csrc/renderer.hpp
+++ b/raytracercpp_amd/csrc/renderer.hpp
@@ -15,6 +15,7 @@
 #include "kparams.hpp"
 #include "ocone.hpp"
 #include "octree.hpp"
+#include "tile_lists.hpp"
 #include "tri_geometry.hpp"
 #include "wbvh.hpp"
 #include "wide_layout.hpp"
@@ -109,6 +110,7 @@
     bool scene_bound = true;
     bool tile_mask = true;
     bool tile_start = true;
+    bool tile_list = true;
     int cut_budget = W_CUT_BUDGET;
     bool ocone = true;
     int ocone_dim = 128;
@@ -188,6 +190,7 @@
     int kernel_times(float* ms, int n);
     int band_counters(unsigned long long out[2]);
     int tile_mask(int src, uint32_t* out, int64_t cap, int32_t info[5]);
+    int tile_lists(int src, int32_t* out, int64_t cap, int32_t info[5]);
     int tile_starts(int src, uint32_t* out, int64_t cap, int32_t info[3]);
     int debug_read(uint64_t* out, int64_t n);
     int tile_costs(uint32_t* out, int64_t n, int32_t* tiles_x, int32_t* tiles_y);
@@ -351,15 +354,37 @@
         uint32_t launches = 0;
         WMaskCam cam{};
         uint64_t cut_gen = 0;
+        bool lists_valid = false;
+        uint64_t list_key = 0;
+        int32_t list_off = 0;
+        TileLayout L{};
+        int list_use = -1;
+        uint64_t use_gen = 0;
+        uint32_t list_launches = 0;
+        bool probe_pending = false;
+        struct Probe {
+            unsigned long long* host = nullptr;
+            hipEvent_t ev = nullptr;
+            ~Probe()
+            {
+                if (host) hipHostFree(host);
+                if (ev) hipEventDestroy(ev);
+            }
+        } probe;
     };
+    static constexpr unsigned long long LIST_TICKET_CYCLES = 10000;
+    static constexpr unsigned long long LIST_MIN_SHARE_INV = 50;
+    int probe_lists(const KParams& P, hipStream_t stream);
+    MaskSlot* lists_slot_ = nullptr;
     DevBuf d_cut_;
     bool cut_valid_ = false, mask_seen_ = false;
     uint64_t cut_gen_ = 0;
     MaskSlot mask_main_;
     MaskSlot* mask_last_ = nullptr;
+    bool lists_last_ = false;
     bool starts_last_ = false;
     Fence cut_fence_;
-    int prepare_mask(KParams& P, hipStream_t stream, MaskSlot& M);
+    int prepare_mask(KParams& P, hipStream_t stream, MaskSlot& M, uint64_t layout_key = 0);
     DevBuf d_dbg_;
     bool ssao_ready_ = false;
     DevBuf d_rcount_, d_roff_, d_pieces_, d_piece_uv_, d_zkey_, d_big_, d_scan_tmp_;
diff --git a/raytracercpp_amd/csrc/tile_lists.hpp b/raytracercpp_amd/csrc/tile_lists.hpp
--- /dev/null
+++ b/raytracercpp_amd/csrc/tile_lists.hpp
@@ -0,0 +1,79 @@
+#pragma once
+
+#include <stdint.h>
+
+#include <vector>
+
+#include "rt_math.hpp"
+
+namespace rt {
+
+struct TileLayout {
+    int32_t rw, rh;
+    int32_t local_rows;
+    int32_t band_rows;
+    int32_t rank, nranks;
+    int32_t tiles_x, tiles_y;
+    const int32_t* band_map;
+    const uint32_t* mask;
+    int32_t mask_wpr;
+};
+
+enum TileClass { TILE_OFF = 0, TILE_CLEAR = 1, TILE_COVERED = 2 };
+
+RT_HD int tl_global_row(const TileLayout& L, int lr)
+{
+    if (L.nranks == 1)
+        return lr;
+    const int band = lr / L.band_rows;
+    const int g = L.band_map ? L.band_map[band] : band * L.nranks + L.rank;
+    return g * L.band_rows + (lr - band * L.band_rows);
+}
+
+RT_HD int tile_lane_class(const TileLayout& L, int tile, int lane)
+{
+    const int tx = tile % L.tiles_x, ty = tile / L.tiles_x;
+    const int px = tx * 8 + (lane & 7);
+    const int lr = ty * 8 + (lane >> 3);
+    const int py = lr < L.local_rows ? tl_global_row(L, lr) : L.rh;
+    if (px >= L.rw || py >= L.rh)
+        return TILE_OFF;
+    const uint32_t mw = L.mask[(size_t)(py >> 3) * (size_t)L.mask_wpr + (size_t)(px >> 8)];
+    return (mw >> ((px >> 3) & 31)) & 1u ? TILE_COVERED : TILE_CLEAR;
+}
+
+RT_HD int tile_class(const TileLayout& L, int tile)
+{
+    int c = TILE_OFF;
+    for (int row = 0; row < 8; row++) {
+        const int k = tile_lane_class(L, tile, 8 * row);
+        c = k > c ? k : c;
+    }
+    return c;
+}
+
+RT_HD void tile_shard_range(int n, int s, int shards, int& r0, int& r1)
+{
+    r0 = (int)((long long)n * s / shards);
+    r1 = (int)((long long)n * (s + 1) / shards);
+}
+
+constexpr int TL_HEAD = 4;
+RT_HD size_t tile_lists_class_word(int ntiles) { return (size_t)TL_HEAD + 2 * (size_t)ntiles; }
+RT_HD size_t tile_lists_words(int ntiles) { return tile_lists_class_word(ntiles) + 4 * (((size_t)ntiles + 63) / 64); }
+
+inline void tile_lists_host(const TileLayout& L, std::vector<int32_t>& covered, std::vector<int32_t>& clear)
+{
+    covered.clear();
+    clear.clear();
+    const int ntiles = L.tiles_x * L.tiles_y;
+    for (int t = 0; t < ntiles; t++) {
+        const int c = tile_class(L, t);
+        if (c == TILE_COVERED)
+            covered.push_back(t);
+        else if (c == TILE_CLEAR)
+            clear.push_back(t);
+    }
+}
+
+}
diff --git a/raytracercpp_amd/renderer.py b/raytracercpp_amd/renderer.py
--- a/raytracercpp_amd/renderer.py
+++ b/raytracercpp_amd/renderer.py
@@ -460,6 +460,15 @@
         sets = np.zeros((int(info[1]), int(info[0]), 4), np.uint32)
         self._call("rt_tile_starts", int(src), ptr(sets, _u32p), sets.size, ptr(info, _i32p))
         return sets, bool(info[2])
+
+    def tile_lists(self, src=0):
+        info = np.zeros(5, np.int32)
+        self._call("rt_tile_lists", int(src), None, 0, ptr(info, _i32p))
+        tiles = np.zeros(max(1, int(info[2]) + int(info[3])), np.int32)
+        self._call("rt_tile_lists", int(src), ptr(tiles, _i32p), tiles.size, ptr(info, _i32p))
+        nc, nk = int(info[2]), int(info[3])
+        return tiles[:nc].copy(), tiles[nc:nc + nk].copy(), {"on": bool(info[4]), "tiles_x": int(info[0]),
+                                                             "tiles_y": int(info[1])}
 
     def load_scene(self, sc: SceneData, st: RenderSettings):
         self.set_render_settings(st)
```

New measurement: 10890 Mrays/s, median of 6. 1.05x the previous value.
